# mryab/learning-at-home

Hardware: NVIDIA H100
Metric: DMoE training samples/sec (whole job, device-timed, max over ranks) (higher is better)
Workload: dtype bf16

## Files before the change

learning-at-home_b200/csrc/adam.cu:

```cuda
#include "sm90.cuh"

namespace lah {

struct AdamArgs {
    float* p; float* g; float* m; float* v; float* vmax; bf16* p_bf16;
    int num_segs; long long seg_start[13]; long long seg_n[12]; long long total;
    const int* step;
    const int* group_rows;
    int step_scalar;
    float lr, beta1, beta2, eps, weight_decay;
    int amsgrad, zero_mask;
    int world; long long peer_grad_off; char* peer_base[8]; float grad_scale;
    int G_active; const int* shadow_of; long long shadow_g_off; int me;
    int num_ranges; long long r_start[6]; long long r_cum[7];
    int dead_mask;
    const int* poison;
    float decay;
    const float* lr_dev;
};

template <bool DECOUPLED, bool DEV_LR>
__global__ void __launch_bounds__(256) adam_kernel(AdamArgs a) {
    if (a.poison && (*a.poison & 1)) return;
    float dev_lr = 0.f, dev_decay = 1.f;
    if constexpr (DEV_LR) {
        dev_lr = a.lr_dev[0];
        if constexpr (DECOUPLED) dev_decay = a.lr_dev[1];
    }
    const long long stride = static_cast<long long>(gridDim.x) * blockDim.x * 4;
    const long long span = a.num_ranges ? a.r_cum[a.num_ranges] : a.total;
    for (long long j = (static_cast<long long>(blockIdx.x) * blockDim.x + threadIdx.x) * 4; j < span; j += stride) {
        long long i = j;
        if (a.num_ranges) {
            int r = 0;
#pragma unroll
            for (int t = 1; t < 6; ++t)
                if (t < a.num_ranges && j >= a.r_cum[t]) r = t;
            i = a.r_start[r] + (j - a.r_cum[r]);
        }
        int sg = 0;
#pragma unroll
        for (int t = 1; t < 12; ++t)
            if (t < a.num_segs && i >= a.seg_start[t]) sg = t;
        const int g = static_cast<int>((i - a.seg_start[sg]) / a.seg_n[sg]);
        if (g >= a.G_active) continue;
        if (a.group_rows && a.group_rows[g] <= 0) continue;
        const int step = a.step ? a.step[g] : a.step_scalar;
        const float bc1 = 1.f - powf(a.beta1, static_cast<float>(step));
        const float bc2 = 1.f - powf(a.beta2, static_cast<float>(step));
        const float step_size = (DEV_LR ? dev_lr : a.lr) / bc1;
        const float inv_sqrt_bc2 = rsqrtf(bc2);
        float4 gr;
        if (a.peer_grad_off >= 0) {
            gr = make_float4(0.f, 0.f, 0.f, 0.f);
            for (int r = 0; r < a.world; ++r) {
                if ((a.dead_mask >> r) & 1) continue;
                const float4 t = *reinterpret_cast<const float4*>(
                    reinterpret_cast<const float*>(a.peer_base[r] + a.peer_grad_off) + i);
                gr.x += t.x; gr.y += t.y; gr.z += t.z; gr.w += t.w;
            }
            gr.x *= a.grad_scale; gr.y *= a.grad_scale; gr.z *= a.grad_scale; gr.w *= a.grad_scale;
        } else if (a.shadow_of && a.shadow_of[2 * g] >= 0) {
            const int slot = a.shadow_of[2 * g], mask = a.shadow_of[2 * g + 1];
            gr = ((mask >> a.me) & 1) ? *reinterpret_cast<const float4*>(a.g + i) : make_float4(0.f, 0.f, 0.f, 0.f);
            const long long pi = i + (a.G_active + slot - g) * a.seg_n[sg];
            for (int r = 0; r < a.world; ++r) {
                if (r == a.me || !((mask >> r) & 1)) continue;
                const float4 t = *reinterpret_cast<const float4*>(
                    reinterpret_cast<const float*>(a.peer_base[r] + a.shadow_g_off) + pi);
                gr.x += t.x; gr.y += t.y; gr.z += t.z; gr.w += t.w;
            }
        } else {
            gr = *reinterpret_cast<const float4*>(a.g + i);
        }
        float4 p = *reinterpret_cast<const float4*>(a.p + i);
        float4 m = *reinterpret_cast<const float4*>(a.m + i);
        float4 v = *reinterpret_cast<const float4*>(a.v + i);
        float4 vm = a.amsgrad ? *reinterpret_cast<const float4*>(a.vmax + i) : make_float4(0.f, 0.f, 0.f, 0.f);
        float* pp = &p.x; float* mp = &m.x; float* vp = &v.x; float* vmp = &vm.x; float* gp = &gr.x;
#pragma unroll
        for (int t = 0; t < 4; ++t) {
            float grad = gp[t];
            if constexpr (DECOUPLED) pp[t] = __fmul_rn(pp[t], DEV_LR ? dev_decay : a.decay);
            else if (a.weight_decay != 0.f) grad += a.weight_decay * pp[t];
            mp[t] = mp[t] + (1.f - a.beta1) * (grad - mp[t]);
            vp[t] = vp[t] * a.beta2 + (1.f - a.beta2) * grad * grad;
            float denom;
            if (a.amsgrad) {
                vmp[t] = fmaxf(vmp[t], vp[t]);
                denom = sqrtf(vmp[t]) * inv_sqrt_bc2 + a.eps;
            } else {
                denom = sqrtf(vp[t]) * inv_sqrt_bc2 + a.eps;
            }
            pp[t] -= step_size * (mp[t] / denom);
        }
        *reinterpret_cast<float4*>(a.p + i) = p;
        *reinterpret_cast<float4*>(a.m + i) = m;
        *reinterpret_cast<float4*>(a.v + i) = v;
        if (a.amsgrad) *reinterpret_cast<float4*>(a.vmax + i) = vm;
        if (a.p_bf16) {
            uint2 q;
            q.x = pack_bf16x2(p.x, p.y);
            q.y = pack_bf16x2(p.z, p.w);
            *reinterpret_cast<uint2*>(a.p_bf16 + i) = q;
        }
        if (((a.zero_mask >> sg) & 1) && a.peer_grad_off < 0)
            *reinterpret_cast<float4*>(a.g + i) = make_float4(0.f, 0.f, 0.f, 0.f);
    }
}

__global__ void bump_steps_kernel(int* step, const int* group_rows, int G) {
    const int g = blockIdx.x * blockDim.x + threadIdx.x;
    if (g < G && group_rows[g] > 0) step[g] += 1;
}

__global__ void cast_bf16_kernel(const float* __restrict__ src, bf16* __restrict__ dst, long long n) {
    const long long stride = static_cast<long long>(gridDim.x) * blockDim.x * 4;
    for (long long i = (static_cast<long long>(blockIdx.x) * blockDim.x + threadIdx.x) * 4; i < n; i += stride) {
        const float4 p = *reinterpret_cast<const float4*>(src + i);
        uint2 q;
        q.x = pack_bf16x2(p.x, p.y);
        q.y = pack_bf16x2(p.z, p.w);
        *reinterpret_cast<uint2*>(dst + i) = q;
    }
}

__global__ void split_encode_kernel(const float* __restrict__ p, bf16* __restrict__ hi, uint16_t* __restrict__ lo,
                                    float* __restrict__ v, long long n) {
    const long long stride = static_cast<long long>(gridDim.x) * blockDim.x * 4;
    for (long long i = (static_cast<long long>(blockIdx.x) * blockDim.x + threadIdx.x) * 4; i < n; i += stride) {
        const float4 w = *reinterpret_cast<const float4*>(p + i);
        float4 s = *reinterpret_cast<const float4*>(v + i);
        uint2 h, l;
        h.x = pack_bf16x2(w.x, w.y);
        h.y = pack_bf16x2(w.z, w.w);
        l.x = (__float_as_uint(w.x) & 0xffffu) | (__float_as_uint(w.y) << 16);
        l.y = (__float_as_uint(w.z) & 0xffffu) | (__float_as_uint(w.w) << 16);
        s.x = with_tie_bit(without_tie_bit(s.x), split_tie_up(w.x));
        s.y = with_tie_bit(without_tie_bit(s.y), split_tie_up(w.y));
        s.z = with_tie_bit(without_tie_bit(s.z), split_tie_up(w.z));
        s.w = with_tie_bit(without_tie_bit(s.w), split_tie_up(w.w));
        *reinterpret_cast<uint2*>(hi + i) = h;
        *reinterpret_cast<uint2*>(lo + i) = l;
        *reinterpret_cast<float4*>(v + i) = s;
    }
}

__global__ void split_decode_kernel(const bf16* __restrict__ hi, const uint16_t* __restrict__ lo,
                                    const float* __restrict__ v, float* __restrict__ p, long long n) {
    const long long stride = static_cast<long long>(gridDim.x) * blockDim.x * 4;
    for (long long i = (static_cast<long long>(blockIdx.x) * blockDim.x + threadIdx.x) * 4; i < n; i += stride) {
        const uint2 h = *reinterpret_cast<const uint2*>(hi + i);
        const uint2 l = *reinterpret_cast<const uint2*>(lo + i);
        const float4 s = *reinterpret_cast<const float4*>(v + i);
        float4 w;
        w.x = split_decode(h.x & 0xffffu, l.x & 0xffffu, __float_as_uint(s.x) >> 31);
        w.y = split_decode(h.x >> 16, l.x >> 16, __float_as_uint(s.y) >> 31);
        w.z = split_decode(h.y & 0xffffu, l.y & 0xffffu, __float_as_uint(s.z) >> 31);
        w.w = split_decode(h.y >> 16, l.y >> 16, __float_as_uint(s.w) >> 31);
        *reinterpret_cast<float4*>(p + i) = w;
    }
}

}

using namespace lah;

extern "C" const int* lah_get_poison_word();

extern "C" {

int lah_adam_step(float* p, float* g, float* m, float* v, float* vmax, void* p_bf16, int num_segs, const long long* seg_n,
                  int G, const int* step, const int* group_rows, int step_scalar, float lr, const float* lr_dev, float beta1,
                  float beta2, float eps, float weight_decay, int amsgrad, int zero_mask, int world, long long peer_grad_off,
                  const unsigned long long* peer_bases, float grad_scale, int G_active, const int* shadow_of,
                  long long shadow_g_off, int me, int seg_mask, int dead_mask, float decay, int decoupled, cudaStream_t st) {
    if (num_segs < 1 || num_segs > 12) return -2;
    if (decoupled && weight_decay != 0.f) return -2;
    AdamArgs a;
    a.num_segs = num_segs;
    long long off = 0;
    for (int s = 0; s < 12; ++s) {
        a.seg_start[s] = off;
        a.seg_n[s] = s < num_segs ? seg_n[s] : 1;
        if (s < num_segs) {
            if (seg_n[s] % 4) return -2;
            off += seg_n[s] * G;
        }
    }
    a.seg_start[12] = off;
    a.p = p; a.g = g; a.m = m; a.v = v; a.vmax = vmax; a.p_bf16 = (bf16*)p_bf16;
    a.total = off; a.step = step; a.group_rows = group_rows; a.step_scalar = step_scalar; a.lr = lr;
    a.beta1 = beta1; a.beta2 = beta2; a.eps = eps; a.weight_decay = weight_decay; a.amsgrad = amsgrad;
    a.zero_mask = zero_mask; a.world = world; a.peer_grad_off = peer_grad_off; a.grad_scale = grad_scale;
    a.G_active = G_active > 0 ? G_active : G; a.shadow_of = shadow_of; a.shadow_g_off = shadow_g_off; a.me = me;
    for (int i = 0; i < 8; ++i) a.peer_base[i] = (peer_bases && i < world) ? (char*)peer_bases[i] : nullptr;
    a.poison = lah_get_poison_word();
    a.dead_mask = dead_mask;
    a.decay = decay;
    a.lr_dev = lr_dev;
    a.num_ranges = 0;
    a.r_cum[0] = 0;
    if (seg_mask) {
        for (int s = 0; s < num_segs; ++s) {
            if (!((seg_mask >> s) & 1)) continue;
            const long long len = seg_n[s] * G;
            if (a.num_ranges && a.r_start[a.num_ranges - 1] + (a.r_cum[a.num_ranges] - a.r_cum[a.num_ranges - 1]) == a.seg_start[s]) {
                a.r_cum[a.num_ranges] += len;
            } else {
                if (a.num_ranges == 6) return -2;
                a.r_start[a.num_ranges] = a.seg_start[s];
                a.r_cum[a.num_ranges + 1] = a.r_cum[a.num_ranges] + len;
                ++a.num_ranges;
            }
        }
        if (!a.num_ranges) return 0;
    }
    const long long span = a.num_ranges ? a.r_cum[a.num_ranges] : a.total;
    if (span <= 0) return 0;
    long long blocks = (span / 4 + 255) / 256;
    if (blocks > 132 * 16) blocks = 132 * 16;
    if (lr_dev) {
        if (decoupled)
            adam_kernel<true, true><<<(int)blocks, 256, 0, st>>>(a);
        else
            adam_kernel<false, true><<<(int)blocks, 256, 0, st>>>(a);
    } else if (decoupled) {
        adam_kernel<true, false><<<(int)blocks, 256, 0, st>>>(a);
    } else {
        adam_kernel<false, false><<<(int)blocks, 256, 0, st>>>(a);
    }
    return -(int)cudaGetLastError();
}

int lah_bump_steps(int* step, const int* group_rows, int G, cudaStream_t st) {
    bump_steps_kernel<<<(G + 255) / 256, 256, 0, st>>>(step, group_rows, G);
    return -(int)cudaGetLastError();
}

int lah_cast_bf16(const float* src, void* dst, long long n, cudaStream_t st) {
    if (n % 4) return -2;
    if (n <= 0) return 0;
    long long blocks = (n / 4 + 255) / 256;
    if (blocks > 132 * 16) blocks = 132 * 16;
    cast_bf16_kernel<<<(int)blocks, 256, 0, st>>>(src, (bf16*)dst, n);
    return -(int)cudaGetLastError();
}

int lah_split_master(float* p, void* hi, void* lo, float* v, long long n, int encode, cudaStream_t st) {
    if (n % 4) return -2;
    if (n <= 0) return 0;
    long long blocks = (n / 4 + 255) / 256;
    if (blocks > 132 * 16) blocks = 132 * 16;
    if (encode)
        split_encode_kernel<<<(int)blocks, 256, 0, st>>>(p, (bf16*)hi, (uint16_t*)lo, v, n);
    else
        split_decode_kernel<<<(int)blocks, 256, 0, st>>>((const bf16*)hi, (const uint16_t*)lo, v, p, n);
    return -(int)cudaGetLastError();
}

}
```

learning-at-home_b200/csrc/layernorm.cu:

```cuda
#include "sm90.cuh"
#include <cuda_fp8.h>
#include <stdlib.h>

#include <array>
#include <utility>

namespace lah {

constexpr float LN_EPS = 1e-5f;

constexpr int LN_MAX_C = 4096;

template <int C>
struct LnFwdCfg {
    static constexpr int NV = (C + 255) / 256;
    static constexpr bool TUNED = C >= 256 && (C & (C - 1)) == 0;
    static constexpr int R = TUNED ? ((NV * 4 <= 16) ? 4 : ((NV * 2 <= 16) ? 2 : 1)) : (NV <= 2 ? 4 : (NV <= 6 ? 2 : 1));
    static constexpr int MIN_BLOCKS = (TUNED || NV <= 12) ? 2 : 1;
};

static int ln_rows_per_warp(int dflt) {
    static int forced = -1;
    if (forced < 0) {
        const char* e = getenv("LAH_LN_ROWS");
        forced = e ? atoi(e) : 0;
    }
    return forced == 1 ? 1 : dflt;
}

template <int C, bool QUANT, int R>
__global__ void __launch_bounds__(256, LnFwdCfg<C>::MIN_BLOCKS) ln_relu_fwd_kernel(
    const bf16* __restrict__ h, bf16* __restrict__ a, float* __restrict__ mean_out, float* __restrict__ rstd_out,
    const float* __restrict__ gamma, const float* __restrict__ beta, const int* __restrict__ tile_group, int rows,
    int relu, uint8_t* __restrict__ aq, uint8_t* __restrict__ sf, int tile_shift) {
    constexpr int NV = LnFwdCfg<C>::NV;
    constexpr bool HALF = C % 256 != 0;
    static_assert(C % 128 == 0 && C <= LN_MAX_C && !(QUANT && HALF), "unsupported LayerNorm width");
    const int warp = threadIdx.x >> 5, lane = threadIdx.x & 31;
    const int row0 = (blockIdx.x * 8 + warp) * R;
    if (row0 >= rows) return;
    const int g = tile_group ? __ldg(tile_group + (row0 >> tile_shift)) : 0;
    if (g < 0) return;
    int4 q[R][NV];
#pragma unroll
    for (int r = 0; r < R; ++r) {
        const int4* hp = reinterpret_cast<const int4*>(h + static_cast<long long>(min(row0 + r, rows - 1)) * C);
#pragma unroll
        for (int j = 0; j < NV; ++j) {
            if constexpr (HALF) {
                if (j == NV - 1 && lane >= 16) {
                    q[r][j] = make_int4(0, 0, 0, 0);
                    continue;
                }
            }
            q[r][j] = ld_nc_v4(hp + j * 32 + lane);
        }
    }
    float mean[R], rstd[R];
#pragma unroll
    for (int r = 0; r < R; ++r) {
        float s = 0.f, ss = 0.f;
#pragma unroll
        for (int j = 0; j < NV; ++j) {
            const uint32_t w[4] = {(uint32_t)q[r][j].x, (uint32_t)q[r][j].y, (uint32_t)q[r][j].z, (uint32_t)q[r][j].w};
#pragma unroll
            for (int t = 0; t < 4; ++t) {
                const float2 f = unpack_bf16x2(w[t]);
                s += f.x + f.y;
                ss += f.x * f.x + f.y * f.y;
            }
        }
        s = warp_sum(s);
        ss = warp_sum(ss);
        mean[r] = s * (1.f / C);
        rstd[r] = rsqrtf(fmaxf(ss * (1.f / C) - mean[r] * mean[r], 0.f) + LN_EPS);
        if (lane == 0 && mean_out && row0 + r < rows) {
            mean_out[row0 + r] = mean[r];
            rstd_out[row0 + r] = rstd[r];
        }
    }
    const float* gp = gamma + static_cast<long long>(g) * C;
    const float* bp = beta + static_cast<long long>(g) * C;
#pragma unroll
    for (int j = 0; j < NV; ++j) {
        if constexpr (HALF) {
            if (j == NV - 1 && lane >= 16) break;
        }
        const int col = (j * 32 + lane) * 8;
        const int4 g0 = ld_nc_v4(reinterpret_cast<const int4*>(gp + col));
        const int4 g1 = ld_nc_v4(reinterpret_cast<const int4*>(gp + col + 4));
        const int4 b0 = ld_nc_v4(reinterpret_cast<const int4*>(bp + col));
        const int4 b1 = ld_nc_v4(reinterpret_cast<const int4*>(bp + col + 4));
        const float gg[8] = {__int_as_float(g0.x), __int_as_float(g0.y), __int_as_float(g0.z), __int_as_float(g0.w),
                             __int_as_float(g1.x), __int_as_float(g1.y), __int_as_float(g1.z), __int_as_float(g1.w)};
        const float bb[8] = {__int_as_float(b0.x), __int_as_float(b0.y), __int_as_float(b0.z), __int_as_float(b0.w),
                             __int_as_float(b1.x), __int_as_float(b1.y), __int_as_float(b1.z), __int_as_float(b1.w)};
#pragma unroll
        for (int r = 0; r < R; ++r) {
            const int row = row0 + r;
            if (row >= rows) continue;
            const uint32_t w[4] = {(uint32_t)q[r][j].x, (uint32_t)q[r][j].y, (uint32_t)q[r][j].z, (uint32_t)q[r][j].w};
            float y[8];
#pragma unroll
            for (int t = 0; t < 4; ++t) {
                const float2 f = unpack_bf16x2(w[t]);
                y[2 * t] = (f.x - mean[r]) * rstd[r] * gg[2 * t] + bb[2 * t];
                y[2 * t + 1] = (f.y - mean[r]) * rstd[r] * gg[2 * t + 1] + bb[2 * t + 1];
            }
            if (relu) {
#pragma unroll
                for (int t = 0; t < 8; ++t) y[t] = fmaxf(y[t], 0.f);
            }
            if (!QUANT || a) {
                int4 o;
                o.x = pack_bf16x2(y[0], y[1]);
                o.y = pack_bf16x2(y[2], y[3]);
                o.z = pack_bf16x2(y[4], y[5]);
                o.w = pack_bf16x2(y[6], y[7]);
                st_v4(reinterpret_cast<int4*>(a + static_cast<long long>(row) * C) + j * 32 + lane, o);
            }
            if (QUANT) {
                float amax = 0.f;
#pragma unroll
                for (int t = 0; t < 8; ++t) amax = fmaxf(amax, fabsf(y[t]));
                amax = fmaxf(amax, __shfl_xor_sync(0xffffffffu, amax, 1));
                amax = fmaxf(amax, __shfl_xor_sync(0xffffffffu, amax, 2));
                const uint32_t bits = __float_as_uint(amax * (1.f / 448.f));
                uint32_t e = ((bits >> 23) & 0xFFu) + ((bits & 0x7FFFFFu) ? 1u : 0u);
                e = min(max(e, 1u), 253u);
                const float inv = __uint_as_float((254u - e) << 23);
                uint2 o8;
                o8.x = static_cast<uint32_t>(__nv_cvt_float2_to_fp8x2(make_float2(y[0] * inv, y[1] * inv), __NV_SATFINITE, __NV_E4M3)) |
                       (static_cast<uint32_t>(__nv_cvt_float2_to_fp8x2(make_float2(y[2] * inv, y[3] * inv), __NV_SATFINITE, __NV_E4M3)) << 16);
                o8.y = static_cast<uint32_t>(__nv_cvt_float2_to_fp8x2(make_float2(y[4] * inv, y[5] * inv), __NV_SATFINITE, __NV_E4M3)) |
                       (static_cast<uint32_t>(__nv_cvt_float2_to_fp8x2(make_float2(y[6] * inv, y[7] * inv), __NV_SATFINITE, __NV_E4M3)) << 16);
                asm volatile("st.global.v2.u32 [%0], {%1, %2};" ::"l"(reinterpret_cast<uint2*>(aq + static_cast<long long>(row) * C) + j * 32 + lane),
                             "r"(o8.x), "r"(o8.y)
                             : "memory");
                if ((lane & 3) == 0) {
                    const int kb32 = j * 8 + (lane >> 2);
                    const int ra = row & 127;
                    const long long chunk = static_cast<long long>(row >> 7) * (C / 128) + (kb32 >> 2);
                    sf[chunk * 512 + ((ra & 31) * 4 + (ra >> 5)) * 4 + (kb32 & 3)] = static_cast<uint8_t>(e);
                }
            }
        }
    }
}

template <int C>
struct LnBwdCfg {
    static constexpr int THREADS = (C / 8 + 31) / 32 * 32;
    static constexpr int MIN_BLOCKS = (C <= 2048) ? 2 : 1;
    static constexpr int RB = ((THREADS / 32 * MIN_BLOCKS + 3) / 4 >= 4 && C != 2048) ? 2 : 4;
};

template <int C, bool RES>
__global__ void __launch_bounds__(LnBwdCfg<C>::THREADS, LnBwdCfg<C>::MIN_BLOCKS) ln_relu_bwd_kernel(const bf16* __restrict__ da, const bf16* __restrict__ h,
                                                            const float* __restrict__ mean_in,
                                                            const float* __restrict__ rstd_in,
                                                            const float* __restrict__ gamma,
                                                            const float* __restrict__ beta, bf16* __restrict__ dh,
                                                            float* __restrict__ part,
                                                            const int* __restrict__ tile_group, int rows, int relu, int tile_rows,
                                                            const bf16* __restrict__ dres) {
    constexpr int THREADS = LnBwdCfg<C>::THREADS;
    constexpr int WARPS = THREADS / 32;
    constexpr bool IDLE = THREADS * 8 != C;
    static_assert(C % 128 == 0 && C <= LN_MAX_C, "unsupported LayerNorm width");
    constexpr int RB = LnBwdCfg<C>::RB;
    __shared__ float red[WARPS][2 * RB];
    __shared__ float tot[2 * RB];
    const int tile = blockIdx.x;
    const int g = tile_group ? __ldg(tile_group + tile) : 0;
    if (g < 0) return;
    const int tid = threadIdx.x, warp = tid >> 5, lane = tid & 31;
    const int col = tid * 8;
    const bool live = !IDLE || col < C;
    float gam[8], bet[8];
    if (!live) {
#pragma unroll
        for (int t = 0; t < 8; ++t) gam[t] = bet[t] = 0.f;
    } else {
        const float* gp = gamma + static_cast<long long>(g) * C + col;
        const float* bp = beta + static_cast<long long>(g) * C + col;
        const float4 g0 = __ldg(reinterpret_cast<const float4*>(gp)), g1 = __ldg(reinterpret_cast<const float4*>(gp + 4));
        const float4 b0 = __ldg(reinterpret_cast<const float4*>(bp)), b1 = __ldg(reinterpret_cast<const float4*>(bp + 4));
        gam[0] = g0.x; gam[1] = g0.y; gam[2] = g0.z; gam[3] = g0.w; gam[4] = g1.x; gam[5] = g1.y; gam[6] = g1.z; gam[7] = g1.w;
        bet[0] = b0.x; bet[1] = b0.y; bet[2] = b0.z; bet[3] = b0.w; bet[4] = b1.x; bet[5] = b1.y; bet[6] = b1.z; bet[7] = b1.w;
    }
    float acc_dg[8], acc_db[8], acc_dbias[8];
#pragma unroll
    for (int t = 0; t < 8; ++t) acc_dg[t] = acc_db[t] = acc_dbias[t] = 0.f;

    const int row0 = tile * tile_rows;
    const int row_end = min(rows, row0 + tile_rows);
    int4 nqa[RB], nqh[RB];
    float nmu[RB], nrs[RB];
    auto issue_loads = [&](int rb) {
#pragma unroll
        for (int r = 0; r < RB; ++r) {
            const int row = rb + r;
            const int rr = row < row_end ? row : row0;
            const long long off = static_cast<long long>(rr) * C + col;
            if (live) {
                nqa[r] = ld_nc_v4(reinterpret_cast<const int4*>(da + off));
                nqh[r] = ld_nc_v4(reinterpret_cast<const int4*>(h + off));
            } else {
                nqa[r] = nqh[r] = make_int4(0, 0, 0, 0);
            }
            nmu[r] = __ldg(mean_in + rr);
            nrs[r] = __ldg(rstd_in + rr);
        }
    };
    issue_loads(row0);
    for (int rb = row0; rb < row_end; rb += RB) {
        float rs[RB];
        float part[2 * RB];
        int4 qa_c[RB], qh_c[RB];
        float mu_c[RB];
#pragma unroll
        for (int r = 0; r < RB; ++r) {
            qa_c[r] = nqa[r];
            qh_c[r] = nqh[r];
            mu_c[r] = nmu[r];
            rs[r] = nrs[r];
        }
        if (rb + RB < row_end) issue_loads(rb + RB);
        auto slice = [&](int r, bool ok, float (&gvv)[8], float (&xhh)[8]) {
            const uint32_t wa[4] = {(uint32_t)qa_c[r].x, (uint32_t)qa_c[r].y, (uint32_t)qa_c[r].z, (uint32_t)qa_c[r].w};
            const uint32_t wh[4] = {(uint32_t)qh_c[r].x, (uint32_t)qh_c[r].y, (uint32_t)qh_c[r].z, (uint32_t)qh_c[r].w};
#pragma unroll
            for (int t = 0; t < 4; ++t) {
                const float2 fa = unpack_bf16x2(wa[t]);
                const float2 fh = unpack_bf16x2(wh[t]);
                const float x0 = (fh.x - mu_c[r]) * rs[r], x1 = (fh.y - mu_c[r]) * rs[r];
                const float y0 = x0 * gam[2 * t] + bet[2 * t], y1 = x1 * gam[2 * t + 1] + bet[2 * t + 1];
                gvv[2 * t] = (ok && (!relu || y0 > 0.f)) ? fa.x : 0.f;
                gvv[2 * t + 1] = (ok && (!relu || y1 > 0.f)) ? fa.y : 0.f;
                xhh[2 * t] = x0;
                xhh[2 * t + 1] = x1;
            }
        };
#pragma unroll
        for (int r = 0; r < RB; ++r) {
            float gvv[8], xhh[8];
            slice(r, rb + r < row_end, gvv, xhh);
            float s1 = 0.f, s2 = 0.f;
// ... 203 lines not shown
            }
            nrs[r] = __ldg(rstd_in + rr);
        }
    };
    issue_loads(row0);
    for (int rb = row0; rb < row_end; rb += RB) {
        int4 qd[RB], qx[RB];
        float rs[RB], sum[RB];
#pragma unroll
        for (int r = 0; r < RB; ++r) {
            qd[r] = nqd[r];
            qx[r] = nqx[r];
            rs[r] = nrs[r];
        }
        if (rb + RB < row_end) issue_loads(rb + RB);
        auto unpack8 = [](const int4& q, float (&f)[8]) {
            const uint32_t w[4] = {(uint32_t)q.x, (uint32_t)q.y, (uint32_t)q.z, (uint32_t)q.w};
#pragma unroll
            for (int t = 0; t < 4; ++t) {
                const float2 v = unpack_bf16x2(w[t]);
                f[2 * t] = v.x;
                f[2 * t + 1] = v.y;
            }
        };
#pragma unroll
        for (int r = 0; r < RB; ++r) {
            float d[8], xv[8], s = 0.f;
            unpack8(qd[r], d);
            unpack8(qx[r], xv);
#pragma unroll
            for (int t = 0; t < 8; ++t) s += d[t] * gam[t] * xv[t];
            sum[r] = rb + r < row_end ? s : 0.f;
        }
#pragma unroll
        for (int r = 0; r < RB; ++r) sum[r] = warp_sum(sum[r]);
        if (lane == 0) {
#pragma unroll
            for (int r = 0; r < RB; ++r) red[warp][r] = sum[r];
        }
        __syncthreads();
        if (tid < RB) {
            float s = 0.f;
#pragma unroll
            for (int w = 0; w < WARPS; ++w) s += red[w][tid];
            tot[tid] = s * (1.f / C);
        }
        __syncthreads();
#pragma unroll
        for (int r = 0; r < RB; ++r) {
            const int row = rb + r;
            if (row >= row_end || !live) continue;
            float d[8], xv[8], o[8];
            unpack8(qd[r], d);
            unpack8(qx[r], xv);
            const float m = tot[r] * rs[r] * rs[r];
            if (RES) {
                float res[8];
                unpack8(ld_nc_v4(reinterpret_cast<const int4*>(dres + static_cast<long long>(row) * C + col)), res);
#pragma unroll
                for (int t = 0; t < 8; ++t) o[t] = rs[r] * (d[t] * gam[t] - xv[t] * m) + res[t];
            } else {
#pragma unroll
                for (int t = 0; t < 8; ++t) o[t] = rs[r] * (d[t] * gam[t] - xv[t] * m);
            }
#pragma unroll
            for (int t = 0; t < 8; ++t) acc_dg[t] += d[t] * (xv[t] * rs[r]);
            int4 q;
            q.x = pack_bf16x2(o[0], o[1]);
            q.y = pack_bf16x2(o[2], o[3]);
            q.z = pack_bf16x2(o[4], o[5]);
            q.w = pack_bf16x2(o[6], o[7]);
            *reinterpret_cast<int4*>(dx + static_cast<long long>(row) * C + col) = q;
        }
    }
    if (!live) return;
    float* pg = part + static_cast<long long>(tile) * C + col;
#pragma unroll
    for (int t = 0; t < 8; ++t) pg[t] = acc_dg[t];
}

__global__ void __launch_bounds__(512) grouped_colsum_kernel(const bf16* __restrict__ x, long long ldx,
                                                             float* __restrict__ part, int C,
                                                             const int* __restrict__ tile_group, int rows, int tile_rows) {
    __shared__ float2 sm[4][128];
    const int tile = blockIdx.x;
    const int g = tile_group ? __ldg(tile_group + tile) : 0;
    if (g < 0) return;
    const int cp = threadIdx.x & 127;
    const int phase = threadIdx.x >> 7;
    const int col = blockIdx.y * 256 + cp * 2;
    if (col >= C) return;
    const int row0 = tile * tile_rows, row_end = min(rows, row0 + tile_rows);
    float2 acc = make_float2(0.f, 0.f);
    for (int r = row0 + phase; r < row_end; r += 4) {
        const uint32_t u = __ldg(reinterpret_cast<const uint32_t*>(x + static_cast<long long>(r) * ldx + col));
        const float2 f = unpack_bf16x2(u);
        acc.x += f.x;
        acc.y += f.y;
    }
    sm[phase][cp] = acc;
    __syncthreads();
    if (phase == 0) {
        float2 s = sm[0][cp];
#pragma unroll
        for (int p = 1; p < 4; ++p) {
            s.x += sm[p][cp].x;
            s.y += sm[p][cp].y;
        }
        *reinterpret_cast<float2*>(part + static_cast<long long>(tile) * C + col) = s;
    }
}

__global__ void __launch_bounds__(256) group_tile_sum_kernel(const float* __restrict__ part, int num_tiles, int V, int C,
                                                             const int* __restrict__ tile_group, float* out0, float* out1,
                                                             float* out2) {
    const int i = blockIdx.x * blockDim.x + threadIdx.x;
    if (i >= V * C) return;
    const int v = i / C, c = i - v * C;
    float* out = v == 0 ? out0 : (v == 1 ? out1 : out2);
    int cur = -1;
    float acc = 0.f;
    for (int t = 0; t < num_tiles; ++t) {
        const int g = tile_group ? __ldg(tile_group + t) : 0;
        if (g < 0) continue;
        if (g != cur) {
            if (cur >= 0) out[static_cast<long long>(cur) * C + c] += acc;
            cur = g;
            acc = 0.f;
        }
        acc += __ldg(part + (static_cast<long long>(t) * V + v) * C + c);
    }
    if (cur >= 0) out[static_cast<long long>(cur) * C + c] += acc;
}

using LnFwdLaunch = void (*)(const void*, void*, float*, float*, const float*, const float*, const int*, int, int, int,
                             cudaStream_t);
using LnBwdLaunch = void (*)(const void*, const void*, const float*, const float*, const float*, const float*, void*,
                             float*, float*, float*, float*, const int*, int, int, int, const void*, cudaStream_t);

template <int C>
void ln_fwd_launch(const void* h, void* a, float* mean, float* rstd, const float* gamma, const float* beta,
                   const int* tile_group, int rows, int relu, int tile_shift, cudaStream_t st) {
    constexpr int RR = LnFwdCfg<C>::R;
    if constexpr (LnFwdCfg<C>::TUNED) {
        if (ln_rows_per_warp(RR) == 1) {
            ln_relu_fwd_kernel<C, false, 1><<<(rows + 7) / 8, 256, 0, st>>>(
                (const bf16*)h, (bf16*)a, mean, rstd, gamma, beta, tile_group, rows, relu, nullptr, nullptr, tile_shift);
            return;
        }
    }
    ln_relu_fwd_kernel<C, false, RR><<<(rows + 8 * RR - 1) / (8 * RR), 256, 0, st>>>(
        (const bf16*)h, (bf16*)a, mean, rstd, gamma, beta, tile_group, rows, relu, nullptr, nullptr, tile_shift);
}

template <int C>
void ln_bwd_launch(const void* da, const void* h, const float* mean, const float* rstd, const float* gamma,
                   const float* beta, void* dh, float* dgamma, float* dbeta, float* dbias, float* part,
                   const int* tile_group, int rows, int relu, int tile_rows, const void* dres, cudaStream_t st) {
    const int grid = (rows + tile_rows - 1) / tile_rows;
    constexpr int T = LnBwdCfg<C>::THREADS;
    if (dres)
        ln_relu_bwd_kernel<C, true><<<grid, T, 0, st>>>((const bf16*)da, (const bf16*)h, mean, rstd, gamma, beta,
                                                        (bf16*)dh, part, tile_group, rows, relu, tile_rows,
                                                        (const bf16*)dres);
    else
        ln_relu_bwd_kernel<C, false><<<grid, T, 0, st>>>((const bf16*)da, (const bf16*)h, mean, rstd, gamma, beta,
                                                         (bf16*)dh, part, tile_group, rows, relu, tile_rows, nullptr);
    group_tile_sum_kernel<<<(3 * C + 255) / 256, 256, 0, st>>>(part, grid, 3, C, tile_group, dgamma, dbeta, dbias);
}

template <int... I>
constexpr auto ln_fwd_table(std::integer_sequence<int, I...>) {
    return std::array<LnFwdLaunch, sizeof...(I)>{ln_fwd_launch<(I + 1) * 128>...};
}
template <int... I>
constexpr auto ln_bwd_table(std::integer_sequence<int, I...>) {
    return std::array<LnBwdLaunch, sizeof...(I)>{ln_bwd_launch<(I + 1) * 128>...};
}
constexpr auto kLnFwd = ln_fwd_table(std::make_integer_sequence<int, LN_MAX_C / 128>{});
constexpr auto kLnBwd = ln_bwd_table(std::make_integer_sequence<int, LN_MAX_C / 128>{});

using RmsFwdLaunch = void (*)(const void*, void*, float*, const float*, int, float, const int*, int, cudaStream_t);
using RmsBwdLaunch = void (*)(const void*, const void*, const float*, const float*, void*, float*, float*, int, int,
                              const void*, const int*, cudaStream_t);

template <int C>
void rms_fwd_launch(const void* x, void* n, float* rstd, const float* gamma, int rows, float eps, const int* tile_group,
                    int tile_shift, cudaStream_t st) {
    constexpr int RR = RmsFwdCfg<C>::R;
    const int grid = (rows + 8 * RR - 1) / (8 * RR);
    if (tile_group)
        rms_norm_fwd_kernel<C, RR, true><<<grid, 256, 0, st>>>((const bf16*)x, (bf16*)n, rstd, gamma, rows, eps,
                                                               tile_group, tile_shift);
    else
        rms_norm_fwd_kernel<C, RR, false><<<grid, 256, 0, st>>>((const bf16*)x, (bf16*)n, rstd, gamma, rows, eps,
                                                                nullptr, 0);
}

template <int C, bool GROUPED>
void rms_bwd_kernel_launch(int grid, const void* dn, const void* x, const float* rstd, const float* gamma, void* dx,
                           float* part, int rows, int tile_rows, const void* dres, const int* tile_group,
                           cudaStream_t st) {
    constexpr int T = LnBwdCfg<C>::THREADS;
    if (dres)
        rms_norm_bwd_kernel<C, true, GROUPED><<<grid, T, 0, st>>>((const bf16*)dn, (const bf16*)x, rstd, gamma,
                                                                  (bf16*)dx, part, rows, tile_rows, (const bf16*)dres,
                                                                  tile_group);
    else
        rms_norm_bwd_kernel<C, false, GROUPED><<<grid, T, 0, st>>>((const bf16*)dn, (const bf16*)x, rstd, gamma,
                                                                   (bf16*)dx, part, rows, tile_rows, nullptr,
                                                                   tile_group);
}

template <int C>
void rms_bwd_launch(const void* dn, const void* x, const float* rstd, const float* gamma, void* dx, float* dgamma,
                    float* part, int rows, int tile_rows, const void* dres, const int* tile_group, cudaStream_t st) {
    const int grid = (rows + tile_rows - 1) / tile_rows;
    if (tile_group)
        rms_bwd_kernel_launch<C, true>(grid, dn, x, rstd, gamma, dx, part, rows, tile_rows, dres, tile_group, st);
    else
        rms_bwd_kernel_launch<C, false>(grid, dn, x, rstd, gamma, dx, part, rows, tile_rows, dres, nullptr, st);
    group_tile_sum_kernel<<<(C + 255) / 256, 256, 0, st>>>(part, grid, 1, C, tile_group, dgamma, nullptr, nullptr);
}

template <int... I>
constexpr auto rms_fwd_table(std::integer_sequence<int, I...>) {
    return std::array<RmsFwdLaunch, sizeof...(I)>{rms_fwd_launch<(I + 1) * 128>...};
}
template <int... I>
constexpr auto rms_bwd_table(std::integer_sequence<int, I...>) {
    return std::array<RmsBwdLaunch, sizeof...(I)>{rms_bwd_launch<(I + 1) * 128>...};
}
constexpr auto kRmsFwd = rms_fwd_table(std::make_integer_sequence<int, LN_MAX_C / 128>{});
constexpr auto kRmsBwd = rms_bwd_table(std::make_integer_sequence<int, LN_MAX_C / 128>{});

static bool ln_width_ok(int C) { return C > 0 && C % 128 == 0 && C <= LN_MAX_C; }

}

using namespace lah;

extern "C" {

static int shift_of(int tile_rows) {
    int s = 0;
    while ((1 << s) < tile_rows) ++s;
    return ((1 << s) == tile_rows && tile_rows >= 8) ? s : -1;
}

int lah_ln_relu_fwd(const void* h, void* a, float* mean, float* rstd, const float* gamma, const float* beta,
                    const int* tile_group, int rows, int C, int relu, int tile_rows, cudaStream_t st) {
    if (rows <= 0) return 0;
    const int tile_shift = shift_of(tile_rows);
    if (tile_shift < 0 || !ln_width_ok(C)) return -2;
    kLnFwd[C / 128 - 1](h, a, mean, rstd, gamma, beta, tile_group, rows, relu, tile_shift, st);
    return -(int)cudaGetLastError();
}

int lah_ln_relu_fwd_q(const void* h, void* a, float* mean, float* rstd, const float* gamma, const float* beta,
                      const int* tile_group, int rows, int C, int relu, void* aq, void* sf, cudaStream_t st) {
    if (rows <= 0) return 0;
#define LAH_LN_FWD(CC)                                                                                          \
    if (C == CC) {                                                                                              \
        constexpr int RR = LnFwdCfg<CC>::R;                                                                     \
        if (ln_rows_per_warp(RR) == 1)                                                                          \
            ln_relu_fwd_kernel<CC, true, 1><<<(rows + 7) / 8, 256, 0, st>>>(                                  \
                (const bf16*)h, (bf16*)a, mean, rstd, gamma, beta, tile_group, rows, relu, (uint8_t*)aq, (uint8_t*)sf, 7);   \
        else                                                                                                    \
            ln_relu_fwd_kernel<CC, true, RR><<<(rows + 8 * RR - 1) / (8 * RR), 256, 0, st>>>(                 \
                (const bf16*)h, (bf16*)a, mean, rstd, gamma, beta, tile_group, rows, relu, (uint8_t*)aq, (uint8_t*)sf, 7);   \
        return -(int)cudaGetLastError();                                                                        \
    }
    LAH_LN_FWD(256) LAH_LN_FWD(512) LAH_LN_FWD(1024) LAH_LN_FWD(2048) LAH_LN_FWD(4096)
#undef LAH_LN_FWD
    return -2;
}

int lah_ln_relu_bwd(const void* da, const void* h, const float* mean, const float* rstd, const float* gamma,
                    const float* beta, void* dh, float* dgamma, float* dbeta, float* dbias, float* part,
                    const int* tile_group, int rows, int C, int relu, int tile_rows, const void* dres, cudaStream_t st) {
    if (rows <= 0) return 0;
    if (shift_of(tile_rows) < 0 || !ln_width_ok(C)) return -2;
    kLnBwd[C / 128 - 1](da, h, mean, rstd, gamma, beta, dh, dgamma, dbeta, dbias, part, tile_group, rows, relu,
                        tile_rows, dres, st);
    return -(int)cudaGetLastError();
}

int lah_rms_norm_fwd(const void* x, void* n, float* rstd, const float* gamma, int rows, int C, float eps,
                     const int* tile_group, int tile_rows, cudaStream_t st) {
    if (rows <= 0) return 0;
    const int tile_shift = tile_group ? shift_of(tile_rows) : 0;
    if (!ln_width_ok(C) || !(eps > 0.f) || tile_shift < 0) return -2;
    kRmsFwd[C / 128 - 1](x, n, rstd, gamma, rows, eps, tile_group, tile_shift, st);
    return -(int)cudaGetLastError();
}

int lah_rms_norm_bwd(const void* dn, const void* x, const float* rstd, const float* gamma, void* dx, float* dgamma,
                     float* part, int rows, int C, int tile_rows, const void* dres, const int* tile_group,
                     cudaStream_t st) {
    if (rows <= 0) return 0;
    if (shift_of(tile_rows) < 0 || !ln_width_ok(C)) return -2;
    kRmsBwd[C / 128 - 1](dn, x, rstd, gamma, dx, dgamma, part, rows, tile_rows, dres, tile_group, st);
    return -(int)cudaGetLastError();
}

int lah_grouped_colsum(const void* x, long long ldx, float* out, float* part, int C, const int* tile_group, int rows,
                       int tile_rows, cudaStream_t st) {
    if (rows <= 0) return 0;
    if (C % 128 || shift_of(tile_rows) < 0) return -2;
    const int tiles = (rows + tile_rows - 1) / tile_rows;
    dim3 grid(tiles, (C + 255) / 256);
    grouped_colsum_kernel<<<grid, 512, 0, st>>>((const bf16*)x, ldx, part, C, tile_group, rows, tile_rows);
    group_tile_sum_kernel<<<(C + 255) / 256, 256, 0, st>>>(part, tiles, 1, C, tile_group, out, nullptr, nullptr);
    return -(int)cudaGetLastError();
}

}
```

learning-at-home_b200/csrc/moe.cu:

```cuda
#include <cfloat>

#include "sm90.cuh"

namespace lah {

constexpr int MAX_WORLD = 8;
constexpr int MAX_GRID_DIMS = 4;
constexpr int MAX_K = 8;
constexpr long long SPIN_TIMEOUT_CYCLES = 20000000000ll;

struct Peers {
    char* base[MAX_WORLD];
    int world;
    int me;
    unsigned long long* wait_ns;
    int* step_ctr;
    int spin_timeout_ms;
    char* mc_base;
};

__device__ __forceinline__ void multimem_st_release_u32(void* mc_addr, int v) {
    asm volatile("multimem.st.release.sys.global.u32 [%0], %1;" ::"l"(mc_addr), "r"(v) : "memory");
}
__device__ __forceinline__ void multimem_st_u32(void* mc_addr, int v) {
    asm volatile("multimem.st.relaxed.sys.global.u32 [%0], %1;" ::"l"(mc_addr), "r"(v) : "memory");
}

__device__ __forceinline__ void signal_all_ranks(const Peers& peers, long long flags_off, int slot, int epoch, int tid) {
    if (peers.mc_base) {
        if (tid == 0) {
            __threadfence_system();
            multimem_st_release_u32(peers.mc_base + flags_off + (static_cast<long long>(slot) * MAX_WORLD + peers.me) * 4, epoch);
        }
    } else if (tid < peers.world) {
        __threadfence_system();
        st_release_sys(reinterpret_cast<int*>(peers.base[tid] + flags_off) + slot * MAX_WORLD + peers.me, epoch);
    }
}

__device__ __forceinline__ int epoch_of(const Peers& peers, int rel) {
    return rel + (peers.step_ctr ? *reinterpret_cast<volatile const int*>(peers.step_ctr) : 0);
}

struct GridSpec {
    int ndim;
    int size[MAX_GRID_DIMS];
    int offset[MAX_GRID_DIMS];
    int total;
    int num_experts;
};

enum Status { STATUS_TIMEOUT = 1, STATUS_OVERFLOW = 2 };

__device__ __forceinline__ float hash_uniform(unsigned long long x) {
    x += 0x9E3779B97F4A7C15ull;
    x = (x ^ (x >> 30)) * 0xBF58476D1CE4E5B9ull;
    x = (x ^ (x >> 27)) * 0x94D049BB133111EBull;
    x = x ^ (x >> 31);
    return static_cast<float>(x >> 40) * (1.0f / 16777216.0f);
}

__device__ __forceinline__ bool spin_until_ge(const int* flag, int epoch, int* status, int timeout_ms = 0, int rank = -1) {
    if (status && rank >= 0) {
        const volatile int* vs = status;
        if ((vs[1] >> rank) & 1) return false;
        if (vs[0] & STATUS_TIMEOUT) return false;
    }
    const long long t0 = clock64();
    const long long limit = timeout_ms > 0 ? static_cast<long long>(timeout_ms) * 2000000ll : SPIN_TIMEOUT_CYCLES;
    while (ld_acquire_sys(flag) < epoch) {
        if (clock64() - t0 > limit) {
            atomicOr(status, STATUS_TIMEOUT);
            return false;
        }
    }
    return true;
}

__device__ __forceinline__ void account_wait(const Peers& peers, unsigned long long t0, int world) {
    const unsigned long long dt64 = globaltimer_ns() - t0;
    const unsigned mask = (world >= 32) ? 0xffffffffu : ((1u << world) - 1u);
    const unsigned dt = __reduce_max_sync(mask, dt64 > 0xffffffffull ? 0xffffffffu : static_cast<unsigned>(dt64));
    if (peers.wait_ns && (threadIdx.x & 31) == 0) atomicAdd(peers.wait_ns, static_cast<unsigned long long>(dt));
}

// ... 122 lines not shown
    return a + (BIAS ? t.v2 : sigmoid_affinity(t.v2));
}

template <bool BIAS, bool SIGMOID>
__device__ __forceinline__ void group_scores(const float* lg, const GridSpec& gs, int n_group,
                                             const unsigned char* __restrict__ alive, float failure_rate,
                                             unsigned long long seed, long long tok, const float* __restrict__ bias,
                                             float* gscore, int* gvalid, int lane) {
    const int E = gs.num_experts, gsz = E / n_group;
    if (32 % gsz == 0) {
        for (int c0 = 0; c0 < E; c0 += 32) {
            const int c = c0 + lane;
            GroupTop2 t{-INFINITY, -INFINITY, 0};
            float key;
            if (c < E && group_candidate_key<BIAS, SIGMOID>(lg, gs, c, alive, failure_rate, seed, tok, bias, key))
                group_push<SIGMOID>(t, key);
            for (int o = gsz >> 1; o > 0; o >>= 1) group_merge<SIGMOID>(t, o);
            if (c < E && (lane & (gsz - 1)) == 0) {
                gscore[c / gsz] = group_score<BIAS, SIGMOID>(t);
                gvalid[c / gsz] = t.n > 0;
            }
        }
    } else {
        for (int g = 0; g < n_group; ++g) {
            GroupTop2 t{-INFINITY, -INFINITY, 0};
            for (int c = g * gsz + lane; c < (g + 1) * gsz; c += 32) {
                float key;
                if (group_candidate_key<BIAS, SIGMOID>(lg, gs, c, alive, failure_rate, seed, tok, bias, key))
                    group_push<SIGMOID>(t, key);
            }
#pragma unroll
            for (int o = 16; o > 0; o >>= 1) group_merge<SIGMOID>(t, o);
            if (lane == 0) {
                gscore[g] = group_score<BIAS, SIGMOID>(t);
                gvalid[g] = t.n > 0;
            }
        }
    }
    __syncwarp();
}

__device__ __forceinline__ void select_groups(const float* gscore, int* gvalid, int n_group, int topk_group, int lane) {
    const float a = lane < n_group ? gscore[lane] : -INFINITY;
    const float c = lane + 32 < n_group ? gscore[lane + 32] : -INFINITY;
    bool av = lane < n_group && gvalid[lane], cv = lane + 32 < n_group && gvalid[lane + 32];
    bool as = false, cs = false;
    for (int r = 0; r < topk_group; ++r) {
        float bv = -INFINITY;
        int bi = -1;
        if (av && (!cv || a >= c)) {
            bv = a;
            bi = lane;
        } else if (cv) {
            bv = c;
            bi = lane + 32;
        }
#pragma unroll
        for (int o = 16; o > 0; o >>= 1) {
            const float ov = __shfl_xor_sync(0xffffffffu, bv, o);
            const int oi = __shfl_xor_sync(0xffffffffu, bi, o);
            if ((oi >= 0) && (bi < 0 || ov > bv || (ov == bv && oi < bi))) {
                bv = ov;
                bi = oi;
            }
        }
        if (bi < 0) break;
        if (bi == lane) av = false, as = true;
        if (bi == lane + 32) cv = false, cs = true;
    }
    if (lane < n_group) gvalid[lane] = as;
    if (lane + 32 < n_group) gvalid[lane + 32] = cs;
    __syncwarp();
}

template <bool BIAS, bool SIGMOID, bool GROUPED, bool NORM>
__global__ void __launch_bounds__(256, GROUPED ? 1 : 0) gate_topk_kernel(const float* __restrict__ logits, int B, GridSpec gs, int k,
                                                        const unsigned char* __restrict__ alive, float failure_rate,
                                                        unsigned long long seed, long long token_offset,
                                                        int* __restrict__ idx_out, float* __restrict__ w_out,
                                                        int* __restrict__ pos_out, int* __restrict__ counts,
                                                        const int* __restrict__ step_ctr, const float* __restrict__ bias,
                                                        float scale, float* __restrict__ sig_out, int n_group,
                                                        int topk_group, float* __restrict__ lse_out) {
    constexpr bool LSE = !NORM && !SIGMOID;
    if (step_ctr) token_offset += *reinterpret_cast<const long long*>(step_ctr + 2);
    extern __shared__ float s_logits[];
    const int warp = threadIdx.x >> 5, lane = threadIdx.x & 31;
    const int b = blockIdx.x * 8 + warp;
    if (b >= B) return;
    float* lg = s_logits + warp * gs.total;
    for (int i = lane; i < gs.total; i += 32) lg[i] = logits[static_cast<long long>(b) * gs.total + i];
    __syncwarp();
    const int* gsel = nullptr;
    unsigned gdiv = 0;
    if constexpr (GROUPED) {
        float* gscore = s_logits + 8 * gs.total + warp * GROUP_WORDS;
        int* gvalid = reinterpret_cast<int*>(gscore + MAX_GROUPS);
        group_scores<BIAS, SIGMOID>(lg, gs, n_group, alive, failure_rate, seed, token_offset + b, bias, gscore, gvalid,
                                    lane);
        select_groups(gscore, gvalid, n_group, topk_group, lane);
        gsel = gvalid;
        gdiv = 0x7fffffffu / static_cast<unsigned>(gs.num_experts / n_group) + 1u;
    }

    float best_v[MAX_K];
    float best_u[MAX_K];
    int best_i[MAX_K];
#pragma unroll
    for (int j = 0; j < MAX_K; ++j) {
        best_v[j] = -INFINITY;
        best_u[j] = -INFINITY;
        best_i[j] = -1;
    }
    float run_m = -INFINITY, run_l = 0.f;
    for (int c = lane; c < gs.num_experts; c += 32) {
        float s = 0.f;
        if constexpr (LSE) {
            if (alive && !alive[c]) continue;
            s = pk_score(lg, gs, c);
            lse_fold(run_m, run_l, s);
        }
        if constexpr (GROUPED)
            if (!gsel[__umulhi(static_cast<unsigned>(c) << 1, gdiv)]) continue;
        if (!LSE && alive && !alive[c]) continue;
        if (failure_rate > 0.f) {
            const unsigned long long key = seed ^ (static_cast<unsigned long long>(token_offset + b) * 0x100000001B3ull +
                                                   static_cast<unsigned long long>(c));
            if (hash_uniform(key) < failure_rate) continue;
        }
        if constexpr (!LSE) {
            int rem = c;
#pragma unroll
            for (int d = MAX_GRID_DIMS - 1; d >= 0; --d) {
                if (d < gs.ndim) {
                    const int i = rem % gs.size[d];
                    rem /= gs.size[d];
                    s += lg[gs.offset[d] + i];
                }
            }
        }
        float key = s, aff = s;
        if constexpr (BIAS && SIGMOID) aff = sigmoid_affinity(s);
        if constexpr (BIAS) key = __fadd_rn(aff, __ldg(bias + c));
        if (key > best_v[MAX_K - 1] || best_i[MAX_K - 1] < 0) {
            float v = key, u = aff;
            int id = c;
            bool shifting = false;
#pragma unroll
            for (int j = 0; j < MAX_K; ++j) {
                const bool take = shifting || (best_i[j] < 0) || (v > best_v[j]);
                if (take) {
                    shifting = true;
                    const float tv = best_v[j];
                    const int ti = best_i[j];
                    best_v[j] = v;
                    best_i[j] = id;
                    v = tv;
                    id = ti;
                    if constexpr (BIAS) {
                        const float tu = best_u[j];
                        best_u[j] = u;
                        u = tu;
                    }
                }
            }
        }
// ... 29 lines not shown
                    bi = oi;
                    if constexpr (BIAS) bu = ou;
                }
            }
            sel_v[j] = BIAS ? bu : bv;
            sel_i[j] = bi;
            if (bi >= 0 && bi == id) ++head;
        }
    }
    if constexpr (SIGMOID) {
        float sg[MAX_K];
        float S = 0.f;
#pragma unroll
        for (int j = 0; j < MAX_K; ++j) {
            sg[j] = 0.f;
            if (sel_i[j] >= 0) sg[j] = BIAS ? sel_v[j] : sigmoid_affinity(sel_v[j]);
            S += sg[j];
        }
        const float norm = !NORM ? scale : S > 0.f ? __fdividef(scale, S) : 0.f;
        if (lane < k) {
            int id = -1;
            float v = 0.f;
#pragma unroll
            for (int j = 0; j < MAX_K; ++j)
                if (j == lane) {
                    id = sel_i[j];
                    v = sg[j];
                }
            const long long o = static_cast<long long>(b) * k + lane;
            idx_out[o] = id;
            w_out[o] = v * norm;
            sig_out[o] = v;
            if (id < 0) pos_out[o] = 0;
        }
        return;
    }
    if constexpr (LSE) {
#pragma unroll
        for (int o = 16; o > 0; o >>= 1) lse_merge(run_m, run_l, o);
        const float z = run_m > -INFINITY ? run_m + __logf(run_l) : 0.f;
        if (lane == 0) lse_out[b] = z;
        if (lane < k) {
            int id = -1;
            float v = 0.f;
#pragma unroll
            for (int j = 0; j < MAX_K; ++j)
                if (j == lane) {
                    id = sel_i[j];
                    v = sel_v[j];
                }
            const long long o = static_cast<long long>(b) * k + lane;
            idx_out[o] = id;
            w_out[o] = id >= 0 ? scale * __expf(v - z) : 0.f;
            if (id < 0) pos_out[o] = 0;
        }
        return;
    }
    float mx = -INFINITY;
#pragma unroll
    for (int j = 0; j < MAX_K; ++j)
        if (sel_i[j] >= 0) mx = fmaxf(mx, sel_v[j]);
    float denom = 0.f;
#pragma unroll
    for (int j = 0; j < MAX_K; ++j)
        if (sel_i[j] >= 0) denom += __expf(sel_v[j] - mx);
    if (lane < k) {
        int id = -1;
        float v = 0.f;
#pragma unroll
        for (int j = 0; j < MAX_K; ++j)
            if (j == lane) {
                id = sel_i[j];
                v = sel_v[j];
            }
        const long long o = static_cast<long long>(b) * k + lane;
        idx_out[o] = id;
        w_out[o] = id >= 0 ? __expf(v - mx) / denom : 0.f;
        if (id < 0) pos_out[o] = 0;
    }
}

__global__ void __launch_bounds__(1024) rank_slots_kernel(const int* __restrict__ idx, int n, int* __restrict__ pos,
                                                          int* __restrict__ counts) {
    __shared__ int warp_off[32];
    __shared__ int s_total;
    const int e = blockIdx.x, tid = threadIdx.x, lane = tid & 31, warp = tid >> 5;
    int base = 0;
    for (int start = 0; start < n; start += 1024) {
        const int i = start + tid;
        const bool hit = i < n && __ldg(idx + i) == e;
        const unsigned m = __ballot_sync(0xffffffffu, hit);
        if (lane == 0) warp_off[warp] = __popc(m);
        __syncthreads();
        if (warp == 0) {
            const int v = warp_off[lane];
            int incl = v;
#pragma unroll
            for (int d = 1; d < 32; d <<= 1) {
                const int y = __shfl_up_sync(0xffffffffu, incl, d);
                if (lane >= d) incl += y;
            }
            warp_off[lane] = incl - v;
            if (lane == 31) s_total = incl;
        }
        __syncthreads();
        if (hit) pos[i] = base + warp_off[warp] + __popc(m & ((1u << lane) - 1u));
        base += s_total;
        __syncthreads();
    }
    if (tid == 0 && base) counts[e] += base;
}

struct LayoutArgs {
    long long cnt_all_off;
    long long flags_off;
    int slot;
    int epoch;
    int E, E_loc;
    int max_rows;
    int max_tiles;
    int align;
    int tile_rows;
    int* counts;
    int* dst_row;
    int* group_off;
    int* group_rows;
    int* tile_group;
    int* total_rows;
    int* status;
    int S_max;
    float shadow_tol;
    int min_shadow_rows;
    int* route_owner;
    int* step_rows;
    int* shadow_info;
    int* owned_shadow;
};

constexpr int LAYOUT_MAX_E = 4096;

__global__ void __launch_bounds__(1024) layout_exchange_kernel(Peers peers, LayoutArgs a) {
    __shared__ int warp_tot[32];
    __shared__ int owner_base_s[MAX_WORLD + 1];
    __shared__ int s_tot[LAYOUT_MAX_E];
    __shared__ short s_slot[LAYOUT_MAX_E];
    __shared__ long long s_load[MAX_WORLD];
    __shared__ int s_shadow[MAX_WORLD * 2];
    __shared__ int s_pick[2];
    __shared__ int s_red_v[32], s_red_i[32];
    const int tid = threadIdx.x, lane = tid & 31, warp = tid >> 5;
    const int me = peers.me, world = peers.world;
    a.epoch = epoch_of(peers, a.epoch);
    if (peers.mc_base) {
        int* dst = reinterpret_cast<int*>(peers.mc_base + a.cnt_all_off) + static_cast<long long>(me) * a.E;
        for (int e = tid; e < a.E; e += blockDim.x) multimem_st_u32(dst + e, a.counts[e]);
    } else {
        for (int r = 0; r < world; ++r) {
            int* dst = reinterpret_cast<int*>(peers.base[r] + a.cnt_all_off) + static_cast<long long>(me) * a.E;
            for (int e = tid; e < a.E; e += blockDim.x) dst[e] = a.counts[e];
        }
    }
    __threadfence_system();
    __syncthreads();
    signal_all_ranks(peers, a.flags_off, a.slot, a.epoch, tid);
    if (tid < world) {
        const int* fw = reinterpret_cast<const int*>(peers.base[me] + a.flags_off) + a.slot * MAX_WORLD + tid;
        const unsigned long long t0 = globaltimer_ns();
        spin_until_ge(fw, a.epoch, a.status, peers.spin_timeout_ms, tid);
        account_wait(peers, t0, world);
    }
    __syncthreads();
    {
        const int dead = reinterpret_cast<volatile int*>(a.status)[1];
        if (dead) {
            int* mine = reinterpret_cast<int*>(peers.base[me] + a.cnt_all_off);
            for (int r = 0; r < world; ++r)
                if ((dead >> r) & 1)
                    for (int e = tid; e < a.E; e += blockDim.x) mine[static_cast<long long>(r) * a.E + e] = 0;
        }
    }
    for (int t = tid; t < a.max_tiles; t += blockDim.x) a.tile_group[t] = -1;
    if (tid < MAX_WORLD) s_load[tid] = 0;
    if (tid < MAX_WORLD * 2) s_shadow[tid] = -1;
    __syncthreads();
    const int* cnt_all = reinterpret_cast<const int*>(peers.base[me] + a.cnt_all_off);
    for (int e = tid; e < a.E; e += blockDim.x) {
        int tot = 0;
        for (int s = 0; s < world; ++s) tot += cnt_all[static_cast<long long>(s) * a.E + e];
        s_tot[e] = tot;
        s_slot[e] = -1;
        if (tot) atomicAdd(reinterpret_cast<unsigned long long*>(&s_load[e / a.E_loc]), static_cast<unsigned long long>(tot));
    }
    __syncthreads();
    int num_shadow = 0;
    for (int it = 0; it < a.S_max && world > 1; ++it) {
        if (tid == 0) {
            long long total = 0, mx = -1;
            int rmax = 0;
            for (int r = 0; r < world; ++r) {
                total += s_load[r];
                if (s_load[r] > mx) {
                    mx = s_load[r];
                    rmax = r;
                }
            }
            const bool balanced = static_cast<float>(mx) * world <= a.shadow_tol * static_cast<float>(total);
            s_pick[0] = balanced ? -1 : rmax;
        }
        __syncthreads();
        const int rmax = s_pick[0];
        if (rmax < 0) break;
        int bv = -1, bi = -1;
        for (int le = tid; le < a.E_loc; le += blockDim.x) {
            const int e = rmax * a.E_loc + le;
            if (s_slot[e] < 0 && s_tot[e] > bv) {
                bv = s_tot[e];
                bi = e;
            }
        }
#pragma unroll
        for (int o = 16; o > 0; o >>= 1) {
            const int ov = __shfl_xor_sync(0xffffffffu, bv, o);
            const int oi = __shfl_xor_sync(0xffffffffu, bi, o);
            if (ov > bv || (ov == bv && oi >= 0 && (bi < 0 || oi < bi))) {
// ... 81 lines not shown
            a.group_rows[G_own + s] = rows;
            for (int t = cur / a.tile_rows; t < (cur + padded) / a.tile_rows && t < a.max_tiles; ++t) a.tile_group[t] = G_own + s;
            int mask = 0;
            if (e >= 0)
                for (int r = 0; r < world; ++r) mask |= (cnt_all[static_cast<long long>(r) * a.E + e] > 0) << r;
            a.shadow_info[4 * s + 0] = e;
            a.shadow_info[4 * s + 1] = e >= 0 ? e / a.E_loc : -1;
            a.shadow_info[4 * s + 2] = rows;
            a.shadow_info[4 * s + 3] = mask;
            cur += padded;
        }
        a.group_off[G_own + a.S_max] = cur;
        *a.total_rows = cur;
    }
    if (tid < world) {
        int total = owner_base_s[tid + 1] - owner_base_s[tid];
        for (int s = 0; s < a.S_max; ++s) {
            const int e = s_shadow[s];
            if (e >= 0 && e / a.E_loc != tid)
                total += (cnt_all[static_cast<long long>(tid) * a.E + e] + a.align - 1) / a.align * a.align;
        }
        if (total > a.max_rows) atomicOr(a.status, STATUS_OVERFLOW);
    }
    __syncthreads();
    for (int e = tid; e < a.E; e += blockDim.x) {
        const int owner = e / a.E_loc;
        const int rel = a.dst_row[e] - owner_base_s[owner];
        const int before = a.counts[e];
        const int slot = s_slot[e];
        a.counts[e] = 0;
        if (owner == me) {
            const int le = e - me * a.E_loc;
            a.group_off[le] = rel;
            const int padded = (a.group_rows[le] + a.align - 1) / a.align * a.align;
            for (int t = rel / a.tile_rows; t < (rel + padded) / a.tile_rows && t < a.max_tiles; ++t) a.tile_group[t] = le;
            if (a.step_rows) a.step_rows[le] = s_tot[e];
            if (a.owned_shadow) {
                int mask = 0;
                if (slot >= 0)
                    for (int r = 0; r < world; ++r) mask |= (cnt_all[static_cast<long long>(r) * a.E + e] > 0) << r;
                a.owned_shadow[2 * le] = slot;
                a.owned_shadow[2 * le + 1] = mask;
            }
        }
        int dst, route;
        if (slot < 0) {
            dst = rel + before;
            route = owner;
        } else if (owner == me) {
            dst = rel;
            route = me;
        } else {
            dst = a.group_off[G_own + slot];
            route = me;
        }
        a.dst_row[e] = dst;
        if (a.route_owner) a.route_owner[e] = route;
    }
}

struct ScatterArgs {
    const bf16* src;
    const float* scale;
    const int* idx;
    const int* pos;
    const int* dst_row;
    int* pair_row;
    long long dst_off;
    long long flags_off;
    int slot, epoch;
    int num_pairs, k, H, E_loc, max_rows;
    const int* group_off;
    const int* group_rows;
    int pair_blocks;
    int align;
    const int* route_owner;
    int num_groups;
    int* done_counter;
    int* status;
};

template <int VEC_PER_LANE>
__global__ void __launch_bounds__(256) scatter_rows_kernel(Peers peers, ScatterArgs a) {
    const int warp = threadIdx.x >> 5, lane = threadIdx.x & 31;
    if (static_cast<int>(blockIdx.x) < a.pair_blocks) {
        const int p = blockIdx.x * 8 + warp;
        if (p < a.num_pairs) {
            const int e = a.idx[p];
            int row = -1;
            if (e >= 0) {
                row = (a.pair_row && !a.dst_row) ? a.pair_row[p] : a.dst_row[e] + a.pos[p];
                if (row >= a.max_rows) {
                    if (lane == 0) atomicOr(a.status, STATUS_OVERFLOW);
                    row = -1;
                }
            }
            if (a.pair_row && a.dst_row && lane == 0) a.pair_row[p] = row;
            if (row >= 0) {
                const int owner = a.route_owner ? a.route_owner[e] : e / a.E_loc;
                const int b = p / a.k;
                const int4* sp = reinterpret_cast<const int4*>(a.src + static_cast<long long>(b) * a.H);
                int4* dp = reinterpret_cast<int4*>(peers.base[owner] + a.dst_off) +
                           static_cast<long long>(row) * (a.H / 8);
                int4 v[VEC_PER_LANE];
#pragma unroll
                for (int j = 0; j < VEC_PER_LANE; ++j) v[j] = ld_nc_v4(sp + j * 32 + lane);
                if (a.scale) {
                    const float s = a.scale[p];
#pragma unroll
                    for (int j = 0; j < VEC_PER_LANE; ++j) {
                        uint32_t* u = reinterpret_cast<uint32_t*>(&v[j]);
#pragma unroll
                        for (int t = 0; t < 4; ++t) {
                            const float2 f = unpack_bf16x2(u[t]);
                            u[t] = pack_bf16x2(f.x * s, f.y * s);
                        }
                    }
                }
#pragma unroll
                for (int j = 0; j < VEC_PER_LANE; ++j) st_v4(dp + j * 32 + lane, v[j]);
            }
        }
    } else {
        const int nb = gridDim.x - a.pair_blocks;
        int4* base = reinterpret_cast<int4*>(peers.base[peers.me] + a.dst_off);
        const int4 z = make_int4(0, 0, 0, 0);
        for (int le = blockIdx.x - a.pair_blocks; le < a.num_groups; le += nb) {
            const int r0 = a.group_off[le] + a.group_rows[le];
            const int r1 = min(a.max_rows, a.group_off[le] + (a.group_rows[le] + a.align - 1) / a.align * a.align);
            for (int r = r0 + warp; r < r1; r += 8) {
                int4* dp = base + static_cast<long long>(r) * (a.H / 8);
#pragma unroll
                for (int j = 0; j < VEC_PER_LANE; ++j) dp[j * 32 + lane] = z;
            }
        }
    }
    __syncthreads();
    if (threadIdx.x == 0) {
        __threadfence_system();
        const int prev = atomicAdd(a.done_counter, 1);
        if (prev == static_cast<int>(gridDim.x) - 1) {
            *a.done_counter = 0;
            __threadfence_system();
            const int epoch = epoch_of(peers, a.epoch);
            if (peers.mc_base) {
                multimem_st_release_u32(peers.mc_base + a.flags_off + (static_cast<long long>(a.slot) * MAX_WORLD + peers.me) * 4, epoch);
            } else {
                for (int r = 0; r < peers.world; ++r) {
                    int* f = reinterpret_cast<int*>(peers.base[r] + a.flags_off) + a.slot * MAX_WORLD + peers.me;
                    st_release_sys(f, epoch);
                }
            }
        }
    }
}

__global__ void signal_wait_kernel(Peers peers, long long flags_off, int slot, int epoch, int do_signal, int do_wait,
                                   int* status) {
    const int lane = threadIdx.x;
    epoch = epoch_of(peers, epoch);
    if (do_signal) signal_all_ranks(peers, flags_off, slot, epoch, lane);
    if (do_wait && lane < peers.world) {
        const int* f = reinterpret_cast<const int*>(peers.base[peers.me] + flags_off) + slot * MAX_WORLD + lane;
        const unsigned long long t0 = globaltimer_ns();
        spin_until_ge(f, epoch, status, peers.spin_timeout_ms, lane);
        account_wait(peers, t0, peers.world);
    }
}

__global__ void __launch_bounds__(256) nvls_allreduce_kernel(Peers peers, long long off, long long n, float scale) {
    const long long per = ((n / 4 + peers.world - 1) / peers.world) * 4;
    const long long lo = per * peers.me, hi = min(n, lo + per);
    float* mc = reinterpret_cast<float*>(peers.mc_base + off);
    for (long long i = lo + (static_cast<long long>(blockIdx.x) * blockDim.x + threadIdx.x) * 4; i < hi;
         i += static_cast<long long>(gridDim.x) * blockDim.x * 4) {
        float4 r;
        asm volatile("multimem.ld_reduce.relaxed.sys.global.add.v4.f32 {%0, %1, %2, %3}, [%4];"
                     : "=f"(r.x), "=f"(r.y), "=f"(r.z), "=f"(r.w)
                     : "l"(mc + i)
                     : "memory");
        r.x *= scale; r.y *= scale; r.z *= scale; r.w *= scale;
        asm volatile("multimem.st.relaxed.sys.global.v4.f32 [%0], {%1, %2, %3, %4};" ::"l"(mc + i), "f"(r.x), "f"(r.y),
                     "f"(r.z), "f"(r.w)
                     : "memory");
    }
}

__global__ void heartbeat_kernel(Peers peers, long long hb_off, int first, int count, long long now_ms) {
    const int i = blockIdx.x * blockDim.x + threadIdx.x;
    if (i >= count) return;
    if (peers.mc_base) {
        asm volatile("multimem.st.relaxed.sys.global.u64 [%0], %1;" ::"l"(reinterpret_cast<long long*>(peers.mc_base + hb_off) + first + i),
                     "l"(now_ms)
                     : "memory");
    } else {
        for (int r = 0; r < peers.world; ++r) reinterpret_cast<long long*>(peers.base[r] + hb_off)[first + i] = now_ms;
    }
}

__global__ void alive_from_heartbeats_kernel(const long long* hb, unsigned char* alive, int E, long long now_ms, long long max_age_ms) {
    const int e = blockIdx.x * blockDim.x + threadIdx.x;
    if (e < E) alive[e] = (hb[e] > 0 && now_ms - hb[e] <= max_age_ms) ? 1 : 0;
}

__global__ void step_begin_kernel(int* step_ctr, int epoch_delta, long long token_delta) {
    step_ctr[0] += epoch_delta;
    *reinterpret_cast<long long*>(step_ctr + 2) += token_delta;
}

struct CombineArgs {
    long long src_off;
    const int* idx;
    const int* pair_row;
    const float* w;
    bf16* out;
    int B, k, H, E_loc;
    long long flags_off;
    int slot, epoch, do_signal, do_wait;
    int* status;
    const int* route_owner;
};

template <int VEC_PER_LANE, bool ADD>
__global__ void __launch_bounds__(256) combine_rows_kernel(Peers peers, CombineArgs a, const bf16* __restrict__ addend) {
    const int warp = threadIdx.x >> 5, lane = threadIdx.x & 31;
    if (a.do_signal || a.do_wait) a.epoch = epoch_of(peers, a.epoch);
    if (a.do_signal && blockIdx.x == 0 && threadIdx.x < 32) {
        signal_all_ranks(peers, a.flags_off, a.slot, a.epoch, threadIdx.x);
    }
    if (a.do_wait) {
        if (threadIdx.x < peers.world) {
            const int* f = reinterpret_cast<const int*>(peers.base[peers.me] + a.flags_off) + a.slot * MAX_WORLD + threadIdx.x;
            const unsigned long long t0 = globaltimer_ns();
            spin_until_ge(f, a.epoch, a.status, peers.spin_timeout_ms, threadIdx.x);
            if (blockIdx.x == 0) account_wait(peers, t0, peers.world);
        }
        __syncthreads();
    }
    const int b = blockIdx.x * 8 + warp;
    if (b >= a.B) return;
    float acc[VEC_PER_LANE * 8];
    if constexpr (ADD) {
        const int4* ap = reinterpret_cast<const int4*>(addend + static_cast<long long>(b) * a.H);
#pragma unroll
        for (int v = 0; v < VEC_PER_LANE; ++v) {
            const int4 q = __ldg(ap + v * 32 + lane);
            const uint32_t u[4] = {(uint32_t)q.x, (uint32_t)q.y, (uint32_t)q.z, (uint32_t)q.w};
#pragma unroll
            for (int t = 0; t < 4; ++t) {
                const float2 f = unpack_bf16x2(u[t]);
                acc[v * 8 + 2 * t] = f.x;
                acc[v * 8 + 2 * t + 1] = f.y;
            }
        }
    } else {
#pragma unroll
        for (int i = 0; i < VEC_PER_LANE * 8; ++i) acc[i] = 0.f;
    }
    for (int j = 0; j < a.k; ++j) {
        const long long p = static_cast<long long>(b) * a.k + j;
        const int e = a.idx[p];
        const int row = a.pair_row[p];
        if (e < 0 || row < 0) continue;
        const float w = a.w ? a.w[p] : 1.f;
        const int4* sp = reinterpret_cast<const int4*>(peers.base[a.route_owner ? a.route_owner[e] : e / a.E_loc] + a.src_off) +
                         static_cast<long long>(row) * (a.H / 8);
#pragma unroll
        for (int v = 0; v < VEC_PER_LANE; ++v) {
            const int4 q = ld_v4(sp + v * 32 + lane);
            const uint32_t u[4] = {(uint32_t)q.x, (uint32_t)q.y, (uint32_t)q.z, (uint32_t)q.w};
#pragma unroll
            for (int t = 0; t < 4; ++t) {
                const float2 f = unpack_bf16x2(u[t]);
                acc[v * 8 + 2 * t] += w * f.x;
                acc[v * 8 + 2 * t + 1] += w * f.y;
            }
        }
    }
    int4* op = reinterpret_cast<int4*>(a.out + static_cast<long long>(b) * a.H);
#pragma unroll
    for (int v = 0; v < VEC_PER_LANE; ++v) {
        int4 q;
        q.x = pack_bf16x2(acc[v * 8 + 0], acc[v * 8 + 1]);
        q.y = pack_bf16x2(acc[v * 8 + 2], acc[v * 8 + 3]);
        q.z = pack_bf16x2(acc[v * 8 + 4], acc[v * 8 + 5]);
        q.w = pack_bf16x2(acc[v * 8 + 6], acc[v * 8 + 7]);
        op[v * 32 + lane] = q;
    }
}

struct GateBwdArgs {
    long long yo_off;
    const bf16* grad;
    const int* idx;
    const int* pair_row;
    const float* w;
    float* dlogits;
    int B, k, H, E_loc;
    const int* route_owner;
};

template <int VEC_PER_LANE, bool SIGMOID, bool NORM>
__global__ void __launch_bounds__(256) gate_bwd_kernel(Peers peers, GateBwdArgs a, GridSpec gs,
                                                       const float* __restrict__ sig, float scale,
                                                       const float* __restrict__ logits, const float* __restrict__ lse,
                                                       const unsigned char* __restrict__ alive) {
    constexpr bool DENSE = !NORM && !SIGMOID;
    const int warp = threadIdx.x >> 5, lane = threadIdx.x & 31;
    const int b = blockIdx.x * 8 + warp;
    if (b >= a.B) return;
    float g[VEC_PER_LANE * 8];
    const int4* gp = reinterpret_cast<const int4*>(a.grad + static_cast<long long>(b) * a.H);
#pragma unroll
    for (int v = 0; v < VEC_PER_LANE; ++v) {
        const int4 q = ld_nc_v4(gp + v * 32 + lane);
        const uint32_t u[4] = {(uint32_t)q.x, (uint32_t)q.y, (uint32_t)q.z, (uint32_t)q.w};
#pragma unroll
        for (int t = 0; t < 4; ++t) {
            const float2 f = unpack_bf16x2(u[t]);
            g[v * 8 + 2 * t] = f.x;
            g[v * 8 + 2 * t + 1] = f.y;
        }
    }
    float dw[MAX_K], wj[MAX_K], sj[MAX_K];
    int ej[MAX_K];
    float dot_sum = 0.f;
#pragma unroll
    for (int j = 0; j < MAX_K; ++j) {
        dw[j] = 0.f;
        wj[j] = 0.f;
        if constexpr (SIGMOID) sj[j] = 0.f;
        ej[j] = -1;
        if (j < a.k) {
            const long long p = static_cast<long long>(b) * a.k + j;
            const int e = a.idx[p];
            const int row = a.pair_row[p];
            if (e >= 0) {
                wj[j] = a.w[p];
                ej[j] = e;
                if constexpr (SIGMOID) sj[j] = sig[p];
            }
            if (e >= 0 && row >= 0) {
                const int4* sp = reinterpret_cast<const int4*>(peers.base[a.route_owner ? a.route_owner[e] : e / a.E_loc] + a.yo_off) +
                                 static_cast<long long>(row) * (a.H / 8);
                float d = 0.f;
#pragma unroll
                for (int v = 0; v < VEC_PER_LANE; ++v) {
                    const int4 q = ld_v4(sp + v * 32 + lane);
                    const uint32_t u[4] = {(uint32_t)q.x, (uint32_t)q.y, (uint32_t)q.z, (uint32_t)q.w};
#pragma unroll
                    for (int t = 0; t < 4; ++t) {
                        const float2 f = unpack_bf16x2(u[t]);
                        d += g[v * 8 + 2 * t] * f.x + g[v * 8 + 2 * t + 1] * f.y;
                    }
                }
                d = warp_sum(d);
                dw[j] = d;
                dot_sum += wj[j] * d;
            }
        }
    }
    float* dl = a.dlogits + static_cast<long long>(b) * gs.total;
    for (int i = lane; i < gs.total; i += 32) dl[i] = 0.f;
    __syncwarp();
    if (lane == 0) {
        float inv_s = 0.f;
        if constexpr (SIGMOID && NORM) {
            float S = 0.f;
#pragma unroll
            for (int j = 0; j < MAX_K; ++j) S += sj[j];
            inv_s = S > 0.f ? __fdividef(1.f, S) : 0.f;
        }
#pragma unroll
        for (int j = 0; j < MAX_K; ++j) {
            if (ej[j] < 0) continue;
            float d;
            if constexpr (SIGMOID && NORM) d = sj[j] * (1.f - sj[j]) * (scale * dw[j] - dot_sum) * inv_s;
            else if constexpr (SIGMOID) d = scale * sj[j] * (1.f - sj[j]) * dw[j];
            else if constexpr (NORM) d = wj[j] * (dw[j] - dot_sum);
            else d = wj[j] * dw[j];
            int rem = ej[j];
            for (int dd = gs.ndim - 1; dd >= 0; --dd) {
                const int i = rem % gs.size[dd];
                rem /= gs.size[dd];
                dl[gs.offset[dd] + i] += d;
            }
        }
    }
    if constexpr (DENSE) {
// ... 220 lines not shown
    }
    __syncthreads();
    if (threadIdx.x == 0) {
        float ta = 0.f, tq = 0.f;
#pragma unroll
        for (int w = 0; w < RL_WARPS; ++w) {
            ta += s_warp[w][0];
            tq += s_warp[w][1];
        }
        loss[0] = f[gs.num_experts] * ta / static_cast<float>(B);
        loss[1] = tq / static_cast<float>(B);
        *ticket = 0;
    }
}

template <bool SIGMOID>
__global__ void __launch_bounds__(RL_WARPS * 32) router_loss_bwd_kernel(const float* __restrict__ logits, int B, GridSpec gs,
                                                                        const unsigned char* __restrict__ alive,
                                                                        const float* __restrict__ f,
                                                                        const float* __restrict__ z,
                                                                        const float* __restrict__ Fb, float aux_coef,
                                                                        float z_coef, float* __restrict__ dlogits) {
    extern __shared__ float s_buf[];
    const int warp = threadIdx.x >> 5, lane = threadIdx.x & 31;
    const int b = blockIdx.x * RL_WARPS + warp;
    if (b >= B) return;
    float* lg = s_buf + warp * router_bwd_warp_floats(gs);
    float* g = lg + gs.total;
    float* dl = dlogits + static_cast<long long>(b) * gs.total;
    for (int i = lane; i < gs.total; i += 32) lg[i] = logits[static_cast<long long>(b) * gs.total + i];
    __syncwarp();
    const float zb = z[b];
    const float invB = 1.f / static_cast<float>(B);
    const float base_aux = aux_coef * f[gs.num_experts];
    const float c0 = SIGMOID ? -base_aux * Fb[b] : 2.f * z_coef * zb - base_aux * Fb[b];
    const float inv_s = SIGMOID && zb > 0.f ? invB / zb : 0.f;
    for (int c = lane; c < gs.num_experts; c += 32) {
        float v = 0.f;
        if constexpr (SIGMOID) {
            if (!alive || alive[c]) {
                const float sg = sigmoid_affinity(pk_score(lg, gs, c));
                v = sg * (1.f - sg) * (base_aux * f[c] + c0) * inv_s;
            }
        } else if (!alive || alive[c]) {
            v = __expf(pk_score(lg, gs, c) - zb) * (base_aux * f[c] + c0) * invB;
        }
        if (gs.ndim == 1)
            dl[c] += v;
        else
            g[c + (c >> 5)] = v;
    }
    if (gs.ndim == 1) return;
    __syncwarp();
    for (int o = lane; o < gs.total; o += 32) {
        int d = 0;
        while (d + 1 < gs.ndim && o >= gs.offset[d + 1]) ++d;
        const int i = o - gs.offset[d];
        int stride = 1;
        for (int dd = gs.ndim - 1; dd > d; --dd) stride *= gs.size[dd];
        const int block = stride * gs.size[d];
        float acc = 0.f;
        for (int outer = 0; outer < gs.num_experts; outer += block)
            for (int inner = 0; inner < stride; ++inner) {
                const int e = outer + i * stride + inner;
                acc += g[e + (e >> 5)];
            }
        dl[o] += acc;
    }
}

static Peers g_peers = {};
static bool g_peers_set = false;

template <bool BIAS, bool SIGMOID, bool GROUPED, bool NORM>
static int launch_gate_topk(const float* logits, int B, const GridSpec& gs, int k, const unsigned char* alive,
                            float failure_rate, unsigned long long seed, long long token_offset, int* idx, float* w,
                            int* pos, int* counts, const float* bias, float scale, float* sig, int n_group,
                            int topk_group, float* lse, cudaStream_t st) {
    const int group_floats = GROUPED ? GROUP_WORDS : 0;
    if (int e = set_max_dynamic_smem<gate_topk_kernel<BIAS, SIGMOID, GROUPED, NORM>>(8 * sizeof(float) *
                                                                                     (LAYOUT_MAX_E + group_floats)))
        return e;
    if (B <= 0) return 0;
    gate_topk_kernel<BIAS, SIGMOID, GROUPED, NORM><<<(B + 7) / 8, 256, 8 * (gs.total + group_floats) * sizeof(float),
                                                     st>>>(
        logits, B, gs, k, alive, failure_rate, seed, token_offset, idx, w, pos, counts, g_peers.step_ctr, bias, scale, sig,
        n_group, topk_group, lse);
    return 0;
}

constexpr int GATE_BWD_DENSE_MAX_FLOATS = LAYOUT_MAX_E / 2 + 2 + LAYOUT_MAX_E + LAYOUT_MAX_E / 32 + 1;

template <int V, bool SIGMOID, bool NORM>
static int launch_gate_bwd(const GateBwdArgs& a, const GridSpec& gs, const float* sig, float scale, const float* logits,
                           const float* lse, const unsigned char* alive, cudaStream_t st) {
    int smem = 0;
    if constexpr (!SIGMOID && !NORM) {
        if (int e = set_max_dynamic_smem<gate_bwd_kernel<V, SIGMOID, NORM>>(8 * sizeof(float) *
                                                                             GATE_BWD_DENSE_MAX_FLOATS))
            return e;
        if (gs.ndim > 1) smem = 8 * router_bwd_warp_floats(gs) * sizeof(float);
    }
    gate_bwd_kernel<V, SIGMOID, NORM><<<(a.B + 7) / 8, 256, smem, st>>>(g_peers, a, gs, sig, scale, logits, lse, alive);
    return 0;
}

template <bool SIGMOID>
static int launch_router_loss_bwd(const float* logits, int B, const GridSpec& gs, const unsigned char* alive,
                                  const float* f, const float* z, const float* Fb, float aux_coef, float z_coef,
                                  float* dlogits, cudaStream_t st) {
    if (int e = set_max_dynamic_smem<router_loss_bwd_kernel<SIGMOID>>(RL_WARPS * sizeof(float) *
                                                                       (2 * LAYOUT_MAX_E + LAYOUT_MAX_E / 32 + 1)))
        return e;
    if (B == 0) return 0;
    router_loss_bwd_kernel<SIGMOID><<<(B + RL_WARPS - 1) / RL_WARPS, RL_WARPS * 32,
                                      RL_WARPS * router_bwd_warp_floats(gs) * sizeof(float), st>>>(
        logits, B, gs, alive, f, z, Fb, aux_coef, z_coef, dlogits);
    return 0;
}

}

using namespace lah;

extern "C" {

int lah_set_peers(const unsigned long long* bases, int world, int me) {
    if (world < 1 || world > MAX_WORLD || me < 0 || me >= world) return -2;
    for (int i = 0; i < MAX_WORLD; ++i) g_peers.base[i] = i < world ? reinterpret_cast<char*>(bases[i]) : nullptr;
    g_peers.world = world;
    g_peers.me = me;
    g_peers.wait_ns = nullptr;
    g_peers.step_ctr = nullptr;
    g_peers.spin_timeout_ms = 0;
    g_peers.mc_base = nullptr;
    g_peers_set = true;
    return 0;
}

int lah_set_multicast(unsigned long long mc_base) {
    g_peers.mc_base = reinterpret_cast<char*>(mc_base);
    return 0;
}
unsigned long long lah_get_multicast() { return reinterpret_cast<unsigned long long>(g_peers.mc_base); }

int lah_set_step_counters(int* step_ctr) {
    g_peers.step_ctr = step_ctr;
    return 0;
}
const int* lah_get_epoch_base() { return g_peers.step_ctr; }

int lah_set_spin_timeout_ms(int ms) {
    g_peers.spin_timeout_ms = ms;
    return 0;
}

int lah_nvls_allreduce(long long off, long long n, float scale, cudaStream_t st) {
    if (!g_peers_set || !g_peers.mc_base) return -10;
    if (n % 4 || off % 16) return -2;
    long long blocks = (n / 4 / g_peers.world + 255) / 256;
    if (blocks < 1) blocks = 1;
    if (blocks > 132 * 4) blocks = 132 * 4;
    nvls_allreduce_kernel<<<(int)blocks, 256, 0, st>>>(g_peers, off, n, scale);
    return -(int)cudaGetLastError();
}

int lah_heartbeat(long long hb_off, int first, int count, long long now_ms, cudaStream_t st) {
    if (!g_peers_set) return -10;
    if (count <= 0) return 0;
    heartbeat_kernel<<<(count + 127) / 128, 128, 0, st>>>(g_peers, hb_off, first, count, now_ms);
    return -(int)cudaGetLastError();
}

int lah_alive_from_heartbeats(const long long* hb, unsigned char* alive, int E, long long now_ms, long long max_age_ms,
                              cudaStream_t st) {
    if (E <= 0) return 0;
    alive_from_heartbeats_kernel<<<(E + 255) / 256, 256, 0, st>>>(hb, alive, E, now_ms, max_age_ms);
    return -(int)cudaGetLastError();
}

int lah_step_begin(int epoch_delta, long long token_delta, cudaStream_t st) {
    if (!g_peers.step_ctr) return -10;
    step_begin_kernel<<<1, 1, 0, st>>>(g_peers.step_ctr, epoch_delta, token_delta);
    return -(int)cudaGetLastError();
}

int lah_set_wait_counter(unsigned long long* counter) {
    g_peers.wait_ns = counter;
    return 0;
}

static int make_grid_spec(GridSpec* gs, const int* grid, int ndim) {
    if (ndim < 1 || ndim > MAX_GRID_DIMS) return -2;
    gs->ndim = ndim;
    gs->total = 0;
    gs->num_experts = 1;
    for (int d = 0; d < MAX_GRID_DIMS; ++d) {
        gs->size[d] = d < ndim ? grid[d] : 1;
        gs->offset[d] = gs->total;
        if (d < ndim) {
            gs->total += grid[d];
            gs->num_experts *= grid[d];
        }
    }
    return 0;
}

int lah_gate_topk(const float* logits, int B, const int* grid, int ndim, int k, const unsigned char* alive,
                  float failure_rate, unsigned long long seed, long long token_offset, int* idx, float* w, int* pos,
                  int* counts, const float* bias, int score_mode, float scale, float* sig, int n_group, int topk_group,
                  int norm, float* lse, cudaStream_t st) {
    GridSpec gs;
    if (make_grid_spec(&gs, grid, ndim)) return -2;
    if (k < 1 || k > MAX_K) return -3;
    if (gs.total > LAYOUT_MAX_E) return -2;
    if (bias && gs.num_experts > LAYOUT_MAX_E) return -2;
    if (norm != 0 && norm != 1) return -5;
    if (score_mode == 0 && norm && scale != 1.f) return -5;
    if (score_mode == 0 && !norm && (!(scale > 0.f && scale <= FLT_MAX) || (!lse && B > 0))) return -5;
    if (lse && (norm || score_mode != 0)) return -5;
    if (score_mode == 1 && (!(scale > 0.f && scale <= FLT_MAX) || (!sig && B > 0))) return -5;
    if (n_group < 1 || n_group > MAX_GROUPS || gs.num_experts % n_group) return -6;
    if (n_group > 1 && gs.num_experts > LAYOUT_MAX_E) return -6;
    if (topk_group < 1 || topk_group > n_group) return -6;
    const bool grouped = topk_group < n_group;
    int e;
#define LAH_GATE_TOPK(BIAS, SIGMOID, GROUPED, NORM)                                                                    \
    launch_gate_topk<BIAS, SIGMOID, GROUPED, NORM>(logits, B, gs, k, alive, failure_rate, seed, token_offset, idx, w,  \
                                                   pos, counts, BIAS ? bias : nullptr,                                 \
                                                   SIGMOID || !NORM ? scale : 1.f, SIGMOID ? sig : nullptr, n_group,   \
                                                   topk_group, NORM ? nullptr : lse, st)
#define LAH_GATE_TOPK_N(BIAS, SIGMOID, GROUPED) \
    (norm ? LAH_GATE_TOPK(BIAS, SIGMOID, GROUPED, true) : LAH_GATE_TOPK(BIAS, SIGMOID, GROUPED, false))
    if (score_mode == 0)
        e = grouped ? (bias ? LAH_GATE_TOPK_N(true, false, true) : LAH_GATE_TOPK_N(false, false, true))
                    : (bias ? LAH_GATE_TOPK_N(true, false, false) : LAH_GATE_TOPK_N(false, false, false));
    else if (score_mode == 1)
        e = grouped ? (bias ? LAH_GATE_TOPK_N(true, true, true) : LAH_GATE_TOPK_N(false, true, true))
                    : (bias ? LAH_GATE_TOPK_N(true, true, false) : LAH_GATE_TOPK_N(false, true, false));
    else
        return -4;
#undef LAH_GATE_TOPK_N
#undef LAH_GATE_TOPK
    if (e || B <= 0) return e;
    rank_slots_kernel<<<gs.num_experts, 1024, 0, st>>>(idx, B * k, pos, counts);
    return -(int)cudaGetLastError();
}

int lah_layout_exchange(long long cnt_all_off, long long flags_off, int slot, int epoch, int E, int E_loc, int max_rows,
                        int align, int tile_rows, int* counts, int* dst_row, int* group_off, int* group_rows, int* tile_group, int* total_rows,
                        int* status, int S_max, float shadow_tol, int min_shadow_rows, int* route_owner, int* step_rows,
                        int* shadow_info, int* owned_shadow, cudaStream_t st) {
    if (!g_peers_set) return -10;
    if (E > LAYOUT_MAX_E || S_max < 0 || S_max > 2 * MAX_WORLD) return -2;
    LayoutArgs a;
    a.cnt_all_off = cnt_all_off; a.flags_off = flags_off; a.slot = slot; a.epoch = epoch; a.E = E; a.E_loc = E_loc;
    if (tile_rows <= 0 || align % tile_rows) return -2;
    a.max_rows = max_rows; a.tile_rows = tile_rows; a.max_tiles = max_rows / tile_rows; a.align = align; a.counts = counts; a.dst_row = dst_row; a.group_off = group_off;
    a.group_rows = group_rows; a.tile_group = tile_group; a.total_rows = total_rows; a.status = status;
    a.S_max = S_max; a.shadow_tol = shadow_tol; a.min_shadow_rows = min_shadow_rows; a.route_owner = route_owner;
    a.step_rows = step_rows; a.shadow_info = shadow_info; a.owned_shadow = owned_shadow;
    layout_exchange_kernel<<<1, 1024, 0, st>>>(g_peers, a);
    return -(int)cudaGetLastError();
}

int lah_scatter_rows(const void* src, const float* scale, const int* idx, const int* pos, const int* dst_row,
                     int* pair_row, long long dst_off, long long flags_off, int slot, int epoch, int num_pairs, int k,
                     int H, int E_loc, int max_rows, int align, const int* group_off, const int* group_rows,
                     int* done_counter, int* status, const int* route_owner, int num_groups, cudaStream_t st) {
    if (!g_peers_set) return -10;
    ScatterArgs a;
    a.src = (const bf16*)src; a.scale = scale; a.idx = idx; a.pos = pos; a.dst_row = dst_row; a.pair_row = pair_row;
    a.dst_off = dst_off; a.flags_off = flags_off; a.slot = slot; a.epoch = epoch; a.num_pairs = num_pairs; a.k = k;
    a.H = H; a.E_loc = E_loc; a.max_rows = max_rows; a.group_off = group_off; a.group_rows = group_rows;
    a.pair_blocks = (num_pairs + 7) / 8; a.align = align; a.done_counter = done_counter; a.status = status;
    a.route_owner = route_owner; a.num_groups = num_groups > 0 ? num_groups : E_loc;
    const int pad_blocks = a.num_groups < 64 ? a.num_groups : 64;
    const int grid = a.pair_blocks + pad_blocks;
    if (H == 256) scatter_rows_kernel<1><<<grid, 256, 0, st>>>(g_peers, a);
    else if (H == 512) scatter_rows_kernel<2><<<grid, 256, 0, st>>>(g_peers, a);
    else if (H == 1024) scatter_rows_kernel<4><<<grid, 256, 0, st>>>(g_peers, a);
    else return -2;
    return -(int)cudaGetLastError();
}

int lah_signal_wait(long long flags_off, int slot, int epoch, int do_signal, int do_wait, int* status,
                    cudaStream_t st) {
    if (!g_peers_set) return -10;
    signal_wait_kernel<<<1, 32, 0, st>>>(g_peers, flags_off, slot, epoch, do_signal, do_wait, status);
    return -(int)cudaGetLastError();
}

int lah_combine_rows(long long src_off, const int* idx, const int* pair_row, const float* w, void* out, int B, int k,
                     int H, int E_loc, long long flags_off, int slot, int epoch, int do_signal, int do_wait, int* status,
                     const int* route_owner, const void* addend, cudaStream_t st) {
    if (!g_peers_set) return -10;
    if (B <= 0) return 0;
    CombineArgs a;
    a.src_off = src_off; a.idx = idx; a.pair_row = pair_row; a.w = w; a.out = (bf16*)out; a.B = B; a.k = k; a.H = H;
    a.E_loc = E_loc; a.flags_off = flags_off; a.slot = slot; a.epoch = epoch; a.do_signal = do_signal; a.do_wait = do_wait;
    a.status = status; a.route_owner = route_owner;
    const int grid = (B + 7) / 8;
    const bf16* add = (const bf16*)addend;
    if (add && (reinterpret_cast<uintptr_t>(add) % 16)) return -3;
#define LAH_COMBINE(V)                                                                   \
    if (add) combine_rows_kernel<V, true><<<grid, 256, 0, st>>>(g_peers, a, add);        \
    else combine_rows_kernel<V, false><<<grid, 256, 0, st>>>(g_peers, a, nullptr);
    if (H == 256) { LAH_COMBINE(1) }
    else if (H == 512) { LAH_COMBINE(2) }
    else if (H == 1024) { LAH_COMBINE(4) }
    else return -2;
#undef LAH_COMBINE
    return -(int)cudaGetLastError();
}

int lah_gate_bwd(long long yo_off, const void* grad, const int* idx, const int* pair_row, const float* w,
                 float* dlogits, int B, int k, int H, int E_loc, const int* grid_sizes, int ndim, const int* route_owner,
                 const float* sig, float scale, int norm, const float* lse, const float* logits,
                 const unsigned char* alive, cudaStream_t st) {
    if (!g_peers_set) return -10;
    const bool dense = !sig && norm == 0;
    if (norm != 0 && norm != 1) return -5;
    if (dense ? B > 0 && (!lse || !logits) : lse || logits || alive) return -5;
    if (B <= 0) return 0;
    GridSpec gs;
    if (make_grid_spec(&gs, grid_sizes, ndim)) return -2;
    if (k > MAX_K) return -3;
    if (sig || dense ? !(scale > 0.f && scale <= FLT_MAX) : scale != 1.f) return -5;
    if (dense && (gs.num_experts > LAYOUT_MAX_E || router_bwd_warp_floats(gs) > GATE_BWD_DENSE_MAX_FLOATS)) return -2;
    GateBwdArgs a;
    a.yo_off = yo_off; a.grad = (const bf16*)grad; a.idx = idx; a.pair_row = pair_row; a.w = w; a.dlogits = dlogits;
    a.B = B; a.k = k; a.H = H; a.E_loc = E_loc; a.route_owner = route_owner;
    int e;
#define LAH_GATE_BWD(V)                                                                                     \
    e = sig ? (norm ? launch_gate_bwd<V, true, true>(a, gs, sig, scale, nullptr, nullptr, nullptr, st)      \
                    : launch_gate_bwd<V, true, false>(a, gs, sig, scale, nullptr, nullptr, nullptr, st))    \
            : (norm ? launch_gate_bwd<V, false, true>(a, gs, nullptr, 1.f, nullptr, nullptr, nullptr, st)   \
                    : launch_gate_bwd<V, false, false>(a, gs, nullptr, scale, logits, lse, alive, st));
    if (H == 256) { LAH_GATE_BWD(1) }
    else if (H == 512) { LAH_GATE_BWD(2) }
    else if (H == 1024) { LAH_GATE_BWD(4) }
    else return -2;
#undef LAH_GATE_BWD
    if (e) return e;
    return -(int)cudaGetLastError();
}

static int router_grid_spec(GridSpec* gs, const int* grid, int ndim) {
    if (!grid || ndim < 1 || ndim > MAX_GRID_DIMS) return -2;
    long long total = 0, experts = 1;
    for (int d = 0; d < ndim; ++d) {
        if (grid[d] < 1) return -2;
        total += grid[d];
        experts *= grid[d];
        if (total > LAYOUT_MAX_E || experts > LAYOUT_MAX_E) return -2;
    }
    return make_grid_spec(gs, grid, ndim);
}

int lah_router_loss_fwd(const float* logits, int B, const int* grid, int ndim, const unsigned char* alive, const int* counts,
                        int count_rows, float* f, float* z, float* Fb, float* loss, float* partials, int* ticket,
                        int score_mode, cudaStream_t st) {
    GridSpec gs;
    if (router_grid_spec(&gs, grid, ndim)) return -2;
    if (B < 0 || count_rows < 1 || count_rows > MAX_WORLD) return -3;
    if (!counts || !f || !loss || (B > 0 && (!logits || !z || !Fb || !partials || !ticket))) return -4;
    if (score_mode != 0 && score_mode != 1) return -5;
    if (int e = score_mode ? set_max_dynamic_smem<router_loss_fwd_kernel<true>>(RL_WARPS * sizeof(float) * LAYOUT_MAX_E)
                           : set_max_dynamic_smem<router_loss_fwd_kernel<false>>(RL_WARPS * sizeof(float) * LAYOUT_MAX_E))
        return e;
    router_f_kernel<<<1, 1024, 0, st>>>(counts, count_rows, gs.num_experts, alive, f, B, loss);
    const int blocks = (B + RL_WARPS - 1) / RL_WARPS;
    const size_t smem = RL_WARPS * gs.total * sizeof(float);
    if (B > 0 && score_mode)
        router_loss_fwd_kernel<true><<<blocks, RL_WARPS * 32, smem, st>>>(logits, B, gs, alive, f, z, Fb, partials, ticket,
                                                                          loss);
    else if (B > 0)
        router_loss_fwd_kernel<false><<<blocks, RL_WARPS * 32, smem, st>>>(logits, B, gs, alive, f, z, Fb, partials, ticket,
                                                                           loss);
    return -(int)cudaGetLastError();
}

int lah_router_loss_bwd(const float* logits, int B, const int* grid, int ndim, const unsigned char* alive, const float* f,
                        const float* z, const float* Fb, float aux_coef, float z_coef, float* dlogits, int score_mode,
                        cudaStream_t st) {
    GridSpec gs;
    if (router_grid_spec(&gs, grid, ndim)) return -2;
    if (B < 0) return -3;
    if (B > 0 && (!logits || !f || !z || !Fb || !dlogits)) return -4;
    if (score_mode != 0 && (score_mode != 1 || z_coef != 0.f)) return -5;
    if (int e = score_mode ? launch_router_loss_bwd<true>(logits, B, gs, alive, f, z, Fb, aux_coef, z_coef, dlogits, st)
                           : launch_router_loss_bwd<false>(logits, B, gs, alive, f, z, Fb, aux_coef, z_coef, dlogits, st))
        return e;
    return B == 0 ? 0 : -(int)cudaGetLastError();
}

int lah_expert_bias_update(const int* counts, int count_rows, int E, const unsigned char* alive, float rate, float* bias,
                           cudaStream_t st) {
    if (E < 1 || E > LAYOUT_MAX_E) return -2;
    if (count_rows < 1 || count_rows > MAX_WORLD) return -3;
    if (!counts || !bias) return -4;
    if (!(rate >= 0.f && rate <= FLT_MAX)) return -5;
    expert_bias_update_kernel<<<1, 1024, 0, st>>>(counts, count_rows, E, alive, rate, bias);
    return -(int)cudaGetLastError();
}

static int make_seg_layout(SegLayout* L, int num_segs, const long long* seg_n, int slots) {
    if (num_segs < 1 || num_segs > 12) return -2;
    L->num_segs = num_segs;
    long long off = 0;
    for (int s = 0; s < 12; ++s) {
        L->seg_start[s] = off;
        L->seg_n[s] = s < num_segs ? seg_n[s] : 8;
        if (s < num_segs) {
            if (seg_n[s] % 8) return -2;
            off += seg_n[s] * slots;
        }
    }
    L->seg_start[12] = off;
    return 0;
}

int lah_pull_shadow(const int* shadow_info, int S_max, int E_loc, long long p_off, long long pbf16_off, int num_segs,
                    const long long* seg_n, int small_mask, cudaStream_t st) {
    if (!g_peers_set) return -10;
    if (S_max <= 0) return 0;
    PullArgs a;
    a.shadow_info = shadow_info; a.E_loc = E_loc; a.p_off = p_off; a.pbf16_off = pbf16_off; a.small_mask = small_mask;
    if (make_seg_layout(&a.L, num_segs, seg_n, E_loc + S_max)) return -2;
    pull_shadow_kernel<<<dim3(64, S_max), 256, 0, st>>>(g_peers, a);
    return -(int)cudaGetLastError();
}

int lah_zero_slots(float* g, int num_segs, const long long* seg_n, int slots, int first_slot, int num_slots, int seg_mask,
                   cudaStream_t st) {
    if (num_slots <= 0) return 0;
    SegLayout L;
    if (make_seg_layout(&L, num_segs, seg_n, slots)) return -2;
    zero_slots_kernel<<<dim3(8, num_segs), 256, 0, st>>>(g, L, first_slot, num_slots, seg_mask);
    return -(int)cudaGetLastError();
}

}
```

learning-at-home_b200/csrc/sm90.cuh:

```cuda
#pragma once

#include <cuda.h>
#include <cuda_runtime.h>
#include <cuda_bf16.h>
#include <stdint.h>

namespace lah {

typedef __nv_bfloat16 bf16;

__device__ __forceinline__ uint32_t smem_u32(const void* p) {
    return static_cast<uint32_t>(__cvta_generic_to_shared(p));
}

__device__ __forceinline__ uint32_t elect_one_sync() {
    uint32_t pred = 0;
    asm volatile(
        "{\n"
        ".reg .pred P1;\n"
        "elect.sync _|P1, 0xffffffff;\n"
        "selp.b32 %0, 1, 0, P1;\n"
        "}\n"
        : "=r"(pred));
    return pred;
}

__device__ __forceinline__ void mbar_init(uint64_t* bar, uint32_t count) {
    asm volatile("mbarrier.init.shared::cta.b64 [%0], %1;" ::"r"(smem_u32(bar)), "r"(count) : "memory");
}
__device__ __forceinline__ void fence_mbar_init() {
    asm volatile("fence.mbarrier_init.release.cluster;" ::: "memory");
}
__device__ __forceinline__ void fence_proxy_async_smem() {
    asm volatile("fence.proxy.async.shared::cta;" ::: "memory");
}
__device__ __forceinline__ void mbar_arrive_expect_tx(uint64_t* bar, uint32_t bytes) {
    asm volatile("mbarrier.arrive.expect_tx.shared::cta.b64 _, [%0], %1;" ::"r"(smem_u32(bar)), "r"(bytes)
                 : "memory");
}
__device__ __forceinline__ void mbar_arrive(uint64_t* bar) {
    asm volatile("mbarrier.arrive.shared::cta.b64 _, [%0];" ::"r"(smem_u32(bar)) : "memory");
}
__device__ __forceinline__ uint32_t mbar_try_wait(uint64_t* bar, uint32_t parity) {
    uint32_t ok;
    asm volatile(
        "{\n"
        ".reg .pred p;\n"
        "mbarrier.try_wait.parity.shared::cta.b64 p, [%1], %2;\n"
        "selp.b32 %0, 1, 0, p;\n"
        "}\n"
        : "=r"(ok)
        : "r"(smem_u32(bar)), "r"(parity)
        : "memory");
    return ok;
}
__device__ __forceinline__ void mbar_wait(uint64_t* bar, uint32_t parity) {
    while (!mbar_try_wait(bar, parity)) {
    }
}

__device__ __forceinline__ void tma_prefetch_desc(const CUtensorMap* tm) {
    asm volatile("prefetch.tensormap [%0];" ::"l"(reinterpret_cast<uint64_t>(tm)) : "memory");
}
__device__ __forceinline__ void tma_load_2d(void* smem_dst, const CUtensorMap* tm, uint64_t* bar, int c0, int c1) {
    asm volatile(
        "cp.async.bulk.tensor.2d.shared::cluster.global.mbarrier::complete_tx::bytes [%0], [%1, {%3, %4}], [%2];"
        ::"r"(smem_u32(smem_dst)), "l"(reinterpret_cast<uint64_t>(tm)), "r"(smem_u32(bar)), "r"(c0), "r"(c1)
        : "memory");
}
__device__ __forceinline__ void tma_load_3d(void* smem_dst, const CUtensorMap* tm, uint64_t* bar, int c0, int c1,
                                            int c2) {
    asm volatile(
        "cp.async.bulk.tensor.3d.shared::cluster.global.mbarrier::complete_tx::bytes [%0], [%1, {%3, %4, %5}], [%2];"
        ::"r"(smem_u32(smem_dst)), "l"(reinterpret_cast<uint64_t>(tm)), "r"(smem_u32(bar)), "r"(c0), "r"(c1), "r"(c2)
        : "memory");
}
__device__ __forceinline__ void tma_store_2d(const CUtensorMap* tm, const void* smem_src, int c0, int c1) {
    asm volatile("cp.async.bulk.tensor.2d.global.shared::cta.bulk_group [%0, {%2, %3}], [%1];" ::"l"(
                     reinterpret_cast<uint64_t>(tm)),
                 "r"(smem_u32(smem_src)), "r"(c0), "r"(c1)
                 : "memory");
}
__device__ __forceinline__ void tma_store_3d(const CUtensorMap* tm, const void* smem_src, int c0, int c1, int c2) {
    asm volatile("cp.async.bulk.tensor.3d.global.shared::cta.bulk_group [%0, {%2, %3, %4}], [%1];" ::"l"(
                     reinterpret_cast<uint64_t>(tm)),
                 "r"(smem_u32(smem_src)), "r"(c0), "r"(c1), "r"(c2)
                 : "memory");
}
// ... 117 lines not shown

__device__ __forceinline__ uint64_t make_smem_desc_sw64(uint32_t saddr, uint32_t lbo_bytes, uint32_t sbo_bytes) {
    uint64_t d = 0;
    d |= static_cast<uint64_t>((saddr & 0x3FFFFu) >> 4);
    d |= static_cast<uint64_t>((lbo_bytes >> 4) & 0x3FFFu) << 16;
    d |= static_cast<uint64_t>((sbo_bytes >> 4) & 0x3FFFu) << 32;
    d |= static_cast<uint64_t>(2) << 62;
    return d;
}

template <int COLS>
__device__ __forceinline__ uint64_t make_smem_desc_cols(uint32_t saddr, uint32_t lbo_bytes) {
    static_assert(COLS == 32 || COLS == 64, "atoms are 32 or 64 bf16 columns wide");
    if constexpr (COLS == 32) return make_smem_desc_sw64(saddr, lbo_bytes, 512);
    else return make_smem_desc_sw128(saddr, lbo_bytes, 1024);
}

__device__ __forceinline__ void named_bar_sync(int id, int threads) {
    asm volatile("bar.sync %0, %1;" ::"r"(id), "r"(threads) : "memory");
}

__device__ __forceinline__ void st_release_sys(int* p, int v) {
    asm volatile("st.release.sys.global.s32 [%0], %1;" ::"l"(p), "r"(v) : "memory");
}
__device__ __forceinline__ int ld_acquire_sys(const int* p) {
    int v;
    asm volatile("ld.acquire.sys.global.s32 %0, [%1];" : "=r"(v) : "l"(p) : "memory");
    return v;
}
__device__ __forceinline__ void red_add_release_sys(int* p, int v) {
    asm volatile("red.release.sys.global.add.s32 [%0], %1;" ::"l"(p), "r"(v) : "memory");
}
__device__ __forceinline__ int ld_acquire_gpu(const int* p) {
    int v;
    asm volatile("ld.acquire.gpu.global.s32 %0, [%1];" : "=r"(v) : "l"(p) : "memory");
    return v;
}
__device__ __forceinline__ int4 ld_nc_v4(const int4* p) {
    int4 r;
    asm volatile("ld.global.nc.L1::no_allocate.v4.s32 {%0, %1, %2, %3}, [%4];"
                 : "=r"(r.x), "=r"(r.y), "=r"(r.z), "=r"(r.w)
                 : "l"(p));
    return r;
}
__device__ __forceinline__ int4 ld_v4(const int4* p) {
    int4 r;
    asm volatile("ld.global.v4.s32 {%0, %1, %2, %3}, [%4];" : "=r"(r.x), "=r"(r.y), "=r"(r.z), "=r"(r.w) : "l"(p));
    return r;
}
__device__ __forceinline__ void st_v4(int4* p, const int4& v) {
    asm volatile("st.global.v4.s32 [%0], {%1, %2, %3, %4};" ::"l"(p), "r"(v.x), "r"(v.y), "r"(v.z), "r"(v.w)
                 : "memory");
}

__device__ __forceinline__ bool spin_flag_ge(const int* flag, int epoch) {
    const long long t0 = clock64();
    while (ld_acquire_sys(flag) < epoch) {
        if (clock64() - t0 > 20000000000ll) return false;
    }
    return true;
}
__device__ __forceinline__ bool spin_flag_ft(const int* flag, int epoch, int* status, int rank, int timeout_ms) {
    if (status) {
        const volatile int* vs = status;
        if ((vs[1] >> rank) & 1) return false;
        if (vs[0] & 1) return false;
    }
    const long long t0 = clock64();
    const long long limit = timeout_ms > 0 ? static_cast<long long>(timeout_ms) * 2000000ll : 20000000000ll;
    while (ld_acquire_sys(flag) < epoch) {
        if (clock64() - t0 > limit) {
            if (status) atomicOr(status, 1);
            return false;
        }
    }
    return true;
}
__device__ __forceinline__ unsigned long long globaltimer_ns() {
    unsigned long long t;
    asm volatile("mov.u64 %0, %%globaltimer;" : "=l"(t));
    return t;
}
__device__ __forceinline__ void fence_proxy_async_global() { asm volatile("fence.proxy.async.global;" ::: "memory"); }

__device__ __forceinline__ uint32_t pack_bf16x2(float lo, float hi) {
    __nv_bfloat162 v = __floats2bfloat162_rn(lo, hi);
    return *reinterpret_cast<uint32_t*>(&v);
}
__device__ __forceinline__ float2 unpack_bf16x2(uint32_t u) {
    __nv_bfloat162 v = *reinterpret_cast<__nv_bfloat162*>(&u);
    return __bfloat1622float2(v);
}
__device__ __forceinline__ float split_decode(uint32_t hi, uint32_t lo, bool tie_up) {
    const uint32_t up = (lo > 0x8000u || (lo == 0x8000u && tie_up)) ? 1u : 0u;
    return __uint_as_float(((hi - up) << 16) | lo);
}
__device__ __forceinline__ uint32_t split_tie_up(float p) {
    const uint32_t b = __float_as_uint(p);
    return ((b & 0xffffu) == 0x8000u && (b & 0x10000u)) ? 0x80000000u : 0u;
}
__device__ __forceinline__ float with_tie_bit(float v, uint32_t tie) { return __uint_as_float(__float_as_uint(v) | tie); }
__device__ __forceinline__ float without_tie_bit(float v) { return __uint_as_float(__float_as_uint(v) & 0x7fffffffu); }
__device__ __forceinline__ float warp_sum(float v) {
#pragma unroll
    for (int o = 16; o > 0; o >>= 1) v += __shfl_xor_sync(0xffffffffu, v, o);
    return v;
}
__device__ __forceinline__ float warp_max(float v) {
#pragma unroll
    for (int o = 16; o > 0; o >>= 1) v = fmaxf(v, __shfl_xor_sync(0xffffffffu, v, o));
    return v;
}

inline int make_tmap(CUtensorMap* tm, CUtensorMapDataType dtype, int rank, const void* ptr, const uint64_t* dims,
                     const uint64_t* strides_bytes, const uint32_t* box,
                     CUtensorMapSwizzle swizzle = CU_TENSOR_MAP_SWIZZLE_128B) {
    typedef CUresult (*EncodeTiled)(CUtensorMap*, CUtensorMapDataType, cuuint32_t, void*, const cuuint64_t*,
                                    const cuuint64_t*, const cuuint32_t*, const cuuint32_t*, CUtensorMapInterleave,
                                    CUtensorMapSwizzle, CUtensorMapL2promotion, CUtensorMapFloatOOBfill);
    static const EncodeTiled encode = [] {
        void* fn = nullptr;
        cudaDriverEntryPointQueryResult qres;
        if (cudaGetDriverEntryPoint("cuTensorMapEncodeTiled", &fn, cudaEnableDefault, &qres) != cudaSuccess) fn = nullptr;
        return reinterpret_cast<EncodeTiled>(fn);
    }();
    if (!encode) return -100;
    cuuint64_t gdims[3], gstr[2];
    cuuint32_t gbox[3], estr[3] = {1, 1, 1};
    for (int i = 0; i < rank; ++i) {
        gdims[i] = dims[i];
        gbox[i] = box[i];
    }
    for (int i = 0; i < rank - 1; ++i) gstr[i] = strides_bytes[i];
    const CUresult r = encode(tm, dtype, rank, const_cast<void*>(ptr), gdims, gstr, gbox, estr, CU_TENSOR_MAP_INTERLEAVE_NONE,
                              swizzle, CU_TENSOR_MAP_L2_PROMOTION_L2_256B, CU_TENSOR_MAP_FLOAT_OOB_FILL_NONE);
    return r == CUDA_SUCCESS ? 0 : -1000 - static_cast<int>(r);
}

inline int num_sms() {
    static const int sms = [] {
        int dev = 0, n = 0;
        cudaGetDevice(&dev);
        cudaDeviceGetAttribute(&n, cudaDevAttrMultiProcessorCount, dev);
        return n;
    }();
    return sms;
}

inline int persistent_grid(long long total_tiles, int max_ctas) {
    int grid = num_sms();
    if (max_ctas > 0 && max_ctas < grid) grid = max_ctas;
    if (total_tiles < grid) grid = static_cast<int>(total_tiles);
    return grid;
}

template <auto Kernel>
inline int set_max_dynamic_smem(int bytes) {
    static bool done = false;
    if (!done) {
        const cudaError_t e = cudaFuncSetAttribute(Kernel, cudaFuncAttributeMaxDynamicSharedMemorySize, bytes);
        if (e != cudaSuccess) return -static_cast<int>(e);
        done = true;
    }
    return 0;
}

}
```

learning-at-home_b200/csrc/small_m.cu:

```cuda
#include "sm90.cuh"
#include <climits>

namespace lah {
namespace smallm {

constexpr int BM = 128;
constexpr int BK = 64;
constexpr int MMA_K = 16;
constexpr int BN_MAX = 128;
constexpr int NUM_THREADS = 288;

namespace sab {

constexpr int STAGES = 6;
constexpr int A_BYTES = BM * BK * 2;
constexpr int B_BYTES = BN_MAX * BK * 2;
constexpr int STAGE_BYTES = A_BYTES + B_BYTES;
constexpr int BAR_OFFSET = STAGES * STAGE_BYTES;
constexpr int QD = 4;
constexpr int MAX_G = 1023;
constexpr int CUM_OFFSET = BAR_OFFSET + (2 * STAGES + 2 * QD) * 8 + QD * 4 + 16;
constexpr int SMEM_TOTAL = CUM_OFFSET + (MAX_G + 1) * 4 + 1024;
static_assert(SMEM_TOTAL <= 232448, "shared memory budget");

struct Params {
    int G, M_out, K;
    const int* group_off;
    const int* group_rows;
    bf16* out;
    long long ldo;
    const float* bias;
    const bf16* residual;
    long long ldr;
    const int* wait_flags;
    int wait_count, wait_epoch;
    const int* epoch_base;
    int* status;
    int* tile_counter;
};

__device__ __forceinline__ int box_rows_of(int nn) { return nn <= 16 ? 16 : (nn <= 32 ? 32 : (nn <= 64 ? 64 : 128)); }

__device__ __forceinline__ int find_group(const int* cum, int G, int gc) {
    int lo = 0, hi = G - 1;
    while (lo < hi) {
        const int mid = (lo + hi + 1) >> 1;
        if (cum[mid] <= gc) lo = mid; else hi = mid - 1;
    }
    return lo;
}

template <int NB, bool A_MN>
__device__ __forceinline__ void sab_tile(const Params& p, uint8_t* smem, uint64_t* full_bar, uint64_t* empty_bar, int& stage,
                                         uint32_t& phase, int num_kb, int wg, int warp, int lane, int g, int ms, int row0,
                                         int nn) {
    float acc[NB / 2];
    constexpr uint32_t A_KSTEP = A_MN ? MMA_K * 128 : MMA_K * 2;
    int prev_stage = -1;
    for (int kb = 0; kb < num_kb; ++kb) {
        mbar_wait(&full_bar[stage], phase);
        const uint32_t sa = smem_u32(smem + stage * STAGE_BYTES) + wg * (A_MN ? BK * 128 : 64 * 128);
        const uint32_t sb = smem_u32(smem + stage * STAGE_BYTES + A_BYTES);
        wgmma_fence();
#pragma unroll
        for (int k = 0; k < BK / MMA_K; ++k) {
            const uint64_t da = make_smem_desc_sw128(sa + k * A_KSTEP, BK * 128, 1024);
            const uint64_t db = make_smem_desc_sw128(sb + k * (MMA_K * 2), 0, 1024);
            const uint32_t accum = (kb > 0 || k > 0) ? 1u : 0u;
            if constexpr (NB == 16) wgmma_bf16_n16<A_MN, 0>(acc, da, db, accum);
            if constexpr (NB == 32) wgmma_bf16_n32<A_MN, 0>(acc, da, db, accum);
            if constexpr (NB == 64) wgmma_bf16_n64<A_MN, 0>(acc, da, db, accum);
            if constexpr (NB == 128) wgmma_bf16_n128<A_MN, 0>(acc, da, db, accum);
        }
        wgmma_commit();
        wgmma_wait<1>();
        if (prev_stage >= 0) {
            __syncwarp();
            if (lane == 0) mbar_arrive(&empty_bar[prev_stage]);
        }
        prev_stage = stage;
        if (++stage == STAGES) {
            stage = 0;
            phase ^= 1;
        }
    }
    wgmma_wait<0>();
    wgmma_fence_regs(acc);
    __syncwarp();
    if (lane == 0 && prev_stage >= 0) mbar_arrive(&empty_bar[prev_stage]);

    const int n16 = (nn + 15) & ~15;
#pragma unroll
    for (int h = 0; h < 2; ++h) {
        const int feat = ms * BM + wg * 64 + (warp & 3) * 16 + (lane >> 2) + 8 * h;
        const float bias = p.bias ? __ldg(p.bias + static_cast<long long>(g) * p.M_out + feat) : 0.f;
#pragma unroll
        for (int j = 0; j < NB / 8; ++j) {
#pragma unroll
            for (int e = 0; e < 2; ++e) {
                const int n = 8 * j + 2 * (lane & 3) + e;
                if (n < n16) {
                    const long long row = row0 + n;
                    float v = acc[4 * j + 2 * h + e] + bias;
                    if (p.residual) v += __bfloat162float(p.residual[row * p.ldr + feat]);
                    p.out[row * p.ldo + feat] = __float2bfloat16(v);
                }
            }
        }
    }
}

template <bool A_MN>
__global__ void __launch_bounds__(NUM_THREADS, 1)
swapab_kernel(const Params p, const __grid_constant__ CUtensorMap tmA, const __grid_constant__ CUtensorMap tmB16,
              const __grid_constant__ CUtensorMap tmB32, const __grid_constant__ CUtensorMap tmB64,
              const __grid_constant__ CUtensorMap tmB128) {
    extern __shared__ uint8_t smem_raw[];
    uint8_t* smem = reinterpret_cast<uint8_t*>((reinterpret_cast<uintptr_t>(smem_raw) + 1023) & ~uintptr_t(1023));
    uint64_t* full_bar = reinterpret_cast<uint64_t*>(smem + BAR_OFFSET);
    uint64_t* empty_bar = full_bar + STAGES;
    uint64_t* q_full = empty_bar + STAGES;
    uint64_t* q_empty = q_full + QD;
    volatile int* q_tile = reinterpret_cast<volatile int*>(q_empty + QD);
    int* cum = reinterpret_cast<int*>(smem + CUM_OFFSET);

    const int warp = threadIdx.x >> 5;
    const int lane = threadIdx.x & 31;

    if (warp == 0) {
        int carry = 0;
        for (int base = 0; base < p.G; base += 32) {
            const int g = base + lane;
            int x = g < p.G ? (__ldg(p.group_rows + g) + BN_MAX - 1) / BN_MAX : 0;
#pragma unroll
            for (int d = 1; d < 32; d <<= 1) {
                const int y = __shfl_up_sync(0xffffffffu, x, d);
                if (lane >= d) x += y;
            }
            if (g < p.G) cum[g + 1] = carry + x;
            carry += __shfl_sync(0xffffffffu, x, 31);
        }
        if (lane == 0) cum[0] = 0;
    }
    if (warp == 8 && lane == 0) {
        tma_prefetch_desc(&tmA);
        tma_prefetch_desc(&tmB16);
        tma_prefetch_desc(&tmB32);
        tma_prefetch_desc(&tmB64);
        tma_prefetch_desc(&tmB128);
        for (int i = 0; i < STAGES; ++i) {
            mbar_init(&full_bar[i], 1);
            mbar_init(&empty_bar[i], 8);
        }
        for (int i = 0; i < QD; ++i) {
            mbar_init(&q_full[i], 1);
            mbar_init(&q_empty[i], 8);
        }
        fence_mbar_init();
    }
    __syncthreads();

    const int m_slices = p.M_out / BM;
    const int total = cum[p.G] * m_slices;
    const int num_kb = p.K / BK;

    if (warp == 8) {
        if (lane != 0) return;
        if (p.wait_flags) {
            const int epoch = p.wait_epoch + (p.epoch_base ? *p.epoch_base : 0);
            const unsigned long long t_wait = globaltimer_ns();
            for (int sidx = 0; sidx < p.wait_count; ++sidx)
                spin_flag_ft(p.wait_flags + sidx, epoch, p.status, sidx, p.epoch_base ? p.epoch_base[1] : 0);
            if (blockIdx.x == 0) atomicAdd(reinterpret_cast<unsigned long long*>(p.status + 2), globaltimer_ns() - t_wait);
            fence_proxy_async_global();
        }
        int stage = 0, qi = 0;
        uint32_t phase = 0, qphase = 0;
        while (true) {
            const int tile = atomicAdd(p.tile_counter, 1);
            mbar_wait(&q_empty[qi], qphase ^ 1);
            q_tile[qi] = tile;
            mbar_arrive(&q_full[qi]);
            if (++qi == QD) {
                qi = 0;
                qphase ^= 1;
            }
            if (tile >= total) break;
            const int gc = tile / m_slices, ms = tile - gc * m_slices;
            const int g = find_group(cum, p.G, gc);
            const int n0 = (gc - cum[g]) * BN_MAX;
            const int rows = __ldg(p.group_rows + g);
            const int off = __ldg(p.group_off + g);
            const int box = box_rows_of(min(rows - n0, BN_MAX));
            const CUtensorMap* tmB = box == 16 ? &tmB16 : (box == 32 ? &tmB32 : (box == 64 ? &tmB64 : &tmB128));
            for (int kb = 0; kb < num_kb; ++kb) {
                mbar_wait(&empty_bar[stage], phase ^ 1);
                uint8_t* sa = smem + stage * STAGE_BYTES;
                uint8_t* sb = sa + A_BYTES;
                const int k = kb * BK;
                mbar_arrive_expect_tx(&full_bar[stage], A_BYTES + box * 128);
                if (!A_MN) {
                    tma_load_3d(sa, &tmA, &full_bar[stage], k, ms * BM, g);
                } else {
#pragma unroll
                    for (int i = 0; i < BM / 64; ++i)
                        tma_load_3d(sa + i * (BK * 128), &tmA, &full_bar[stage], ms * BM + i * 64, k, g);
                }
                tma_load_2d(sb, tmB, &full_bar[stage], k, off + n0);
                if (++stage == STAGES) {
                    stage = 0;
                    phase ^= 1;
                }
            }
        }
        return;
    }

    const int wg = warp >> 2;
    int stage = 0, qi = 0;
    uint32_t phase = 0, qphase = 0;
    while (true) {
        mbar_wait(&q_full[qi], qphase);
        const int tile = q_tile[qi];
        __syncwarp();
        if (lane == 0) mbar_arrive(&q_empty[qi]);
        if (++qi == QD) {
            qi = 0;
            qphase ^= 1;
        }
        if (tile >= total) break;
        const int gc = tile / m_slices, ms = tile - gc * m_slices;
        const int g = find_group(cum, p.G, gc);
        const int n0 = (gc - cum[g]) * BN_MAX;
        const int nn = min(__ldg(p.group_rows + g) - n0, BN_MAX);
        const int row0 = __ldg(p.group_off + g) + n0;
        switch (box_rows_of(nn)) {
            case 16: sab_tile<16, A_MN>(p, smem, full_bar, empty_bar, stage, phase, num_kb, wg, warp, lane, g, ms, row0, nn); break;
            case 32: sab_tile<32, A_MN>(p, smem, full_bar, empty_bar, stage, phase, num_kb, wg, warp, lane, g, ms, row0, nn); break;
            case 64: sab_tile<64, A_MN>(p, smem, full_bar, empty_bar, stage, phase, num_kb, wg, warp, lane, g, ms, row0, nn); break;
            default: sab_tile<128, A_MN>(p, smem, full_bar, empty_bar, stage, phase, num_kb, wg, warp, lane, g, ms, row0, nn); break;
        }
    }
}

}

namespace wa {

constexpr int WBK = 32;
constexpr int OP_STAGES = 2;
constexpr int OP_STAGE_BYTES = 2 * (WBK * BM * 2);
constexpr int OP_BYTES = OP_STAGES * OP_STAGE_BYTES;
constexpr int BAND_ROWS = 4;
constexpr int CHUNKS = 16 / BAND_ROWS;
constexpr int SUB_COLS = 32;
constexpr int SUB_BYTES = BM / CHUNKS * SUB_COLS * 4;
constexpr int ARR_BYTES = (BN_MAX / SUB_COLS) * SUB_BYTES;
constexpr int ST_STAGES = 3;
constexpr int ST_STAGE_BYTES = 4 * ARR_BYTES;
constexpr int ST_OFFSET = OP_BYTES;
constexpr int BAR_OFFSET = ST_OFFSET + ST_STAGES * ST_STAGE_BYTES;
constexpr int QD = 4;
constexpr int SMEM_TOTAL = BAR_OFFSET + (2 * OP_STAGES + 2 * ST_STAGES + 2 * QD) * 8 + QD * 4 + 16 + 1024;
static_assert(ST_STAGES <= CHUNKS, "the producer issues a tile's first ST_STAGES chunks before its remaining k-blocks");
static_assert(OP_STAGE_BYTES % 1024 == 0 && SUB_BYTES % 1024 == 0, "128-B swizzle atoms need 1 KB alignment");
static_assert(SMEM_TOTAL <= 232448, "shared memory budget");

struct Params {
    int G, N, K;
    const int* group_off;
    const int* group_rows;
    const int* skip;
    const int* step;
    float* p;
    float* m;
    float* v;
    float* vmax;
    bf16* p_bf16;
    float lr, beta1, beta2, eps;
    int amsgrad;
    float wd;
    int* tile_counter;
    const int* poison;
};
static_assert(sizeof(Params) == 128 && sizeof(Params) % alignof(CUtensorMap) == 0, "Params layout");

constexpr int WD_NONE = 0, WD_L2 = 1, WD_DECOUPLED = 2;

struct Tile {
    int g, mt, nt;
};

template <bool SPLIT>
struct StateMaps {
    CUtensorMap a[SPLIT ? 5 : 4];
};
constexpr int PLANE_COLS = 64;
constexpr int PLANE_BYTES = ARR_BYTES / 2;
static_assert(PLANE_BYTES == (BN_MAX / PLANE_COLS) * SUB_BYTES, "a plane box has the rows and bytes of an fp32 box");

template <bool SPLIT>
__device__ __forceinline__ void state_chunk_tma(const StateMaps<SPLIT>& tm, int n_arr, uint8_t* ss, uint64_t* bar, int col0,
                                                int srow, int c) {
    if constexpr (SPLIT) {
        for (int a = 0; a < 2; ++a)
#pragma unroll
            for (int q = 0; q < BN_MAX / PLANE_COLS; ++q) {
                uint8_t* s = ss + a * PLANE_BYTES + q * SUB_BYTES;
                if (bar) tma_load_3d(s, &tm.a[a], bar, col0 + q * PLANE_COLS, BAND_ROWS * c, srow / 16);
                else tma_store_3d(&tm.a[a], s, col0 + q * PLANE_COLS, BAND_ROWS * c, srow / 16);
            }
    }
    for (int a = SPLIT ? 1 : 0; a < n_arr; ++a)
#pragma unroll
        for (int q = 0; q < BN_MAX / SUB_COLS; ++q) {
            uint8_t* s = ss + a * ARR_BYTES + q * SUB_BYTES;
            const CUtensorMap* m = &tm.a[SPLIT ? a + 1 : a];
            if (bar) tma_load_3d(s, m, bar, col0 + q * SUB_COLS, BAND_ROWS * c, srow / 16);
            else tma_store_3d(m, s, col0 + q * SUB_COLS, BAND_ROWS * c, srow / 16);
        }
}

template <int WD, bool DEV_LR, bool SPLIT>
__global__ void __launch_bounds__(NUM_THREADS, 1)
wgrad_adam_kernel(const Params p, const __grid_constant__ CUtensorMap tmDY, const __grid_constant__ CUtensorMap tmX,
                  const __grid_constant__ StateMaps<SPLIT> tmS, const float* __restrict__ lr_dev) {
    extern __shared__ uint8_t smem_raw[];
    uint8_t* smem = reinterpret_cast<uint8_t*>((reinterpret_cast<uintptr_t>(smem_raw) + 1023) & ~uintptr_t(1023));
    uint8_t* st_smem = smem + ST_OFFSET;
    uint64_t* op_full = reinterpret_cast<uint64_t*>(smem + BAR_OFFSET);
    uint64_t* op_empty = op_full + OP_STAGES;
    uint64_t* st_full = op_empty + OP_STAGES;
    uint64_t* st_empty = st_full + ST_STAGES;
    uint64_t* q_full = st_empty + ST_STAGES;
    uint64_t* q_empty = q_full + QD;
    volatile int* q_tile = reinterpret_cast<volatile int*>(q_empty + QD);

    const int warp = threadIdx.x >> 5;
    const int lane = threadIdx.x & 31;
    if (p.poison && (*p.poison & 1)) return;
    const int n_arr = p.amsgrad ? 4 : 3;

    if (warp == 8 && lane == 0) {
        tma_prefetch_desc(&tmDY);
        tma_prefetch_desc(&tmX);
        for (int a = 0; a < n_arr + (SPLIT ? 1 : 0); ++a) tma_prefetch_desc(&tmS.a[a]);
        for (int i = 0; i < OP_STAGES; ++i) {
            mbar_init(&op_full[i], 1);
            mbar_init(&op_empty[i], 8);
        }
        for (int i = 0; i < ST_STAGES; ++i) {
            mbar_init(&st_full[i], 1);
            mbar_init(&st_empty[i], 1);
        }
        for (int i = 0; i < QD; ++i) {
            mbar_init(&q_full[i], 1);
            mbar_init(&q_empty[i], 8);
        }
        fence_mbar_init();
    }
    __syncthreads();

    const int n_tiles = p.K / BN_MAX;
    const int tiles_per_group = (p.N / BM) * n_tiles;
    const int total = p.G * tiles_per_group;
    auto decode = [&](int tile) {
        Tile t;
        t.g = tile / tiles_per_group;
        const int r = tile - t.g * tiles_per_group;
        t.mt = r / n_tiles;
        t.nt = r - t.mt * n_tiles;
        return t;
    };

    if (warp == 8) {
        if (lane != 0) return;
        uint32_t phase = 0, qphase = 0, sphase = 0;
        int qi = 0, stage = 0, sstage = 0;
        while (true) {
            int tile;
            while (true) {
                tile = atomicAdd(p.tile_counter, 1);
                if (tile >= total) break;
                const int g = tile / tiles_per_group;
                if (__ldg(p.group_rows + g) > 0 && !(p.skip && __ldg(p.skip + 2 * g) >= 0)) break;
                atomicMax(p.tile_counter, (g + 1) * tiles_per_group);
            }
            mbar_wait(&q_empty[qi], qphase ^ 1);
            q_tile[qi] = tile;
            mbar_arrive(&q_full[qi]);
            if (++qi == QD) {
                qi = 0;
                qphase ^= 1;
            }
            if (tile >= total) break;
            const Tile t = decode(tile);
            const int off = __ldg(p.group_off + t.g), rows = __ldg(p.group_rows + t.g);
            const int srow = t.g * p.N + t.mt * BM;
            auto load_chunk = [&](int c) {
                mbar_wait(&st_empty[sstage], sphase ^ 1);
                mbar_arrive_expect_tx(&st_full[sstage], n_arr * ARR_BYTES);
                state_chunk_tma(tmS, n_arr, st_smem + sstage * ST_STAGE_BYTES, &st_full[sstage], t.nt * BN_MAX, srow, c);
                if (++sstage == ST_STAGES) {
                    sstage = 0;
                    sphase ^= 1;
                }
            };
            for (int t0 = 0; t0 < rows; t0 += WBK) {
                mbar_wait(&op_empty[stage], phase ^ 1);
                mbar_arrive_expect_tx(&op_full[stage], OP_STAGE_BYTES);
                uint8_t* sa = smem + stage * OP_STAGE_BYTES;
                uint8_t* sb = sa + WBK * BM * 2;
#pragma unroll
                for (int i = 0; i < BM / 64; ++i)
                    tma_load_2d(sa + i * (WBK * 128), &tmDY, &op_full[stage], t.mt * BM + i * 64, off + t0);
#pragma unroll
                for (int i = 0; i < BN_MAX / 64; ++i)
                    tma_load_2d(sb + i * (WBK * 128), &tmX, &op_full[stage], t.nt * BN_MAX + i * 64, off + t0);
                if (++stage == OP_STAGES) {
                    stage = 0;
                    phase ^= 1;
                }
                if (t0 == 0)
                    for (int c = 0; c < ST_STAGES; ++c) load_chunk(c);
            }
            for (int c = ST_STAGES; c < CHUNKS; ++c) load_chunk(c);
        }
        return;
    }

    float lr = p.lr, wd = p.wd;
    if constexpr (DEV_LR) {
        lr = lr_dev[0];
        if constexpr (WD == WD_DECOUPLED) wd = lr_dev[1];
    }
    const int wg = warp >> 2;
    int qi = 0, stage = 0, sstage = 0;
    uint32_t phase = 0, qphase = 0, sphase = 0;
    float acc[BN_MAX / 2];
    float xg[BN_MAX / 8];
    const int lrow = wg * 64 + (warp & 3) * 16 + (lane >> 2);
    const int brow = (lane >> 2) & 3;
    const int R = warp * BAND_ROWS + brow;
    const int jflip = 2 * (brow & 1);
    while (true) {
        mbar_wait(&q_full[qi], qphase);
        const int tile = q_tile[qi];
        __syncwarp();
        if (lane == 0) mbar_arrive(&q_empty[qi]);
        if (++qi == QD) {
            qi = 0;
            qphase ^= 1;
        }
        if (tile >= total) break;
        const Tile t = decode(tile);
        const int rows = __ldg(p.group_rows + t.g);
        int prev_stage = -1;
        for (int t0 = 0; t0 < rows; t0 += WBK) {
            mbar_wait(&op_full[stage], phase);
            const uint32_t sa = smem_u32(smem + stage * OP_STAGE_BYTES) + wg * (WBK * 128);
            const uint32_t sb = smem_u32(smem + stage * OP_STAGE_BYTES + WBK * BM * 2);
            const int ksteps = min(WBK / MMA_K, (rows - t0 + MMA_K - 1) / MMA_K);
            wgmma_fence();
            for (int k = 0; k < ksteps; ++k) {
                const uint64_t da = make_smem_desc_sw128(sa + k * (MMA_K * 128), WBK * 128, 1024);
                const uint64_t db = make_smem_desc_sw128(sb + k * (MMA_K * 128), WBK * 128, 1024);
                wgmma_bf16_n128<1, 1>(acc, da, db, (t0 > 0 || k > 0) ? 1u : 0u);
            }
            wgmma_commit();
            wgmma_wait<1>();
            if (prev_stage >= 0) {
                __syncwarp();
                if (lane == 0) mbar_arrive(&op_empty[prev_stage]);
            }
            prev_stage = stage;
            if (++stage == OP_STAGES) {
                stage = 0;
                phase ^= 1;
// ... 80 lines not shown
                state_chunk_tma(tmS, n_arr, ss, nullptr, t.nt * BN_MAX, srow, c);
                tma_store_commit();
                tma_store_wait_read<0>();
                mbar_arrive(&st_empty[sstage]);
            }
            if (++sstage == ST_STAGES) {
                sstage = 0;
                sphase ^= 1;
            }
            if (c == 1) {
#pragma unroll
                for (int j = 0; j < BN_MAX / 8; ++j) {
                    acc[4 * j] = acc[4 * j + 2];
                    acc[4 * j + 1] = acc[4 * j + 3];
                }
            }
        }
    }
    if (threadIdx.x == 0) tma_store_wait<0>();
}

}
}
}

using namespace lah;
using namespace lah::smallm;

extern "C" const int* lah_get_epoch_base();

static int* tile_counter() {
    static int* ctr = nullptr;
    if (!ctr) {
        if (cudaMalloc(&ctr, 256) != cudaSuccess) return nullptr;
        cudaMemset(ctr, 0, 256);
    }
    return ctr;
}
static const int* g_poison = nullptr;

extern "C" {

int lah_set_poison_word(const int* status) {
    g_poison = status;
    return 0;
}
const int* lah_get_poison_word() { return g_poison; }

int lah_swapab_linear(const void* x, long long ldx, int x_rows, const void* W, int G, int M_out, int K, int a_mn,
                      void* out, long long ldo, const int* group_off, const int* group_rows, const float* bias,
                      const void* residual, long long ldr, const int* wait_flags, int wait_count, int wait_epoch,
                      int* status, int max_ctas, cudaStream_t st) {
    if ((K % BK) || (M_out % BM) || (ldx % 8) || G > sab::MAX_G) return -2;
    CUtensorMap tmA, tmB[4];
    if (!a_mn) {
        uint64_t dims[3] = {(uint64_t)K, (uint64_t)M_out, (uint64_t)G};
        uint64_t str[2] = {(uint64_t)K * 2, (uint64_t)M_out * K * 2};
        uint32_t box[3] = {BK, BM, 1};
        int r = make_tmap(&tmA, CU_TENSOR_MAP_DATA_TYPE_BFLOAT16, 3, W, dims, str, box);
        if (r) return r;
    } else {
        uint64_t dims[3] = {(uint64_t)M_out, (uint64_t)K, (uint64_t)G};
        uint64_t str[2] = {(uint64_t)M_out * 2, (uint64_t)M_out * K * 2};
        uint32_t box[3] = {64, BK, 1};
        int r = make_tmap(&tmA, CU_TENSOR_MAP_DATA_TYPE_BFLOAT16, 3, W, dims, str, box);
        if (r) return r;
    }
    const uint32_t boxes[4] = {16, 32, 64, 128};
    for (int i = 0; i < 4; ++i) {
        uint64_t dims[2] = {(uint64_t)K, (uint64_t)x_rows};
        uint64_t str[1] = {(uint64_t)ldx * 2};
        uint32_t box[2] = {BK, boxes[i]};
        int r = make_tmap(&tmB[i], CU_TENSOR_MAP_DATA_TYPE_BFLOAT16, 2, x, dims, str, box);
        if (r) return r;
    }
    sab::Params p;
    p.G = G; p.M_out = M_out; p.K = K; p.group_off = group_off; p.group_rows = group_rows; p.out = (bf16*)out; p.ldo = ldo;
    p.bias = bias; p.residual = (const bf16*)residual; p.ldr = ldr; p.wait_flags = wait_flags; p.wait_count = wait_count;
    p.wait_epoch = wait_epoch; p.epoch_base = lah_get_epoch_base(); p.status = status;
    p.tile_counter = tile_counter();
    if (!p.tile_counter) return -3;
    const long long total = 1ll * (M_out / BM) * (G + x_rows / BN_MAX);
    if (total <= 0 || G <= 0) return 0;
    if (cudaMemsetAsync(p.tile_counter, 0, sizeof(int), st) != cudaSuccess) return -4;
    const int ctas = persistent_grid(total, max_ctas);
    if (!a_mn) {
        if (int e = set_max_dynamic_smem<sab::swapab_kernel<false>>(sab::SMEM_TOTAL)) return e;
        sab::swapab_kernel<false><<<ctas, NUM_THREADS, sab::SMEM_TOTAL, st>>>(p, tmA, tmB[0], tmB[1], tmB[2], tmB[3]);
    } else {
        if (int e = set_max_dynamic_smem<sab::swapab_kernel<true>>(sab::SMEM_TOTAL)) return e;
        sab::swapab_kernel<true><<<ctas, NUM_THREADS, sab::SMEM_TOTAL, st>>>(p, tmA, tmB[0], tmB[1], tmB[2], tmB[3]);
    }
    return -(int)cudaGetLastError();
}

}

template <int WD, bool DEV_LR, bool SPLIT>
static int launch_wgrad_adam(const wa::Params& a, const CUtensorMap& tmDY, const CUtensorMap& tmX,
                             const wa::StateMaps<SPLIT>& tmS, const float* lr_dev, int ctas, cudaStream_t st) {
    if (int e = set_max_dynamic_smem<wa::wgrad_adam_kernel<WD, DEV_LR, SPLIT>>(wa::SMEM_TOTAL)) return e;
    wa::wgrad_adam_kernel<WD, DEV_LR, SPLIT><<<ctas, NUM_THREADS, wa::SMEM_TOTAL, st>>>(a, tmDY, tmX, tmS, lr_dev);
    return -(int)cudaGetLastError();
}

template <bool SPLIT>
static int wgrad_adam(const void* dy, long long lddy, const void* x, long long ldx, int total_rows, int G, int N, int K,
                      const int* group_off, const int* group_rows, const int* skip, const int* step, void* p, void* lo,
                      float* m, float* v, float* vmax, void* p_bf16, float lr, const float* lr_dev, float beta1, float beta2,
                      float eps, int amsgrad, float weight_decay, float decay, int decoupled, int max_ctas, cudaStream_t st) {
    if ((N % BM) || (K % BN_MAX) || (lddy % 8) || (ldx % 8) || 1ll * G * N > INT_MAX) return -2;
    if (decoupled && weight_decay != 0.f) return -2;
    if (amsgrad && !vmax) return -2;
    CUtensorMap tmDY, tmX;
    wa::StateMaps<SPLIT> tmS;
    {
        void* arrs[5] = {p, m, v, amsgrad ? vmax : (float*)m, nullptr};
        if (SPLIT) {
            arrs[1] = lo; arrs[2] = m; arrs[3] = v; arrs[4] = amsgrad ? vmax : m;
        }
        uint64_t dims[3] = {(uint64_t)K, 16, (uint64_t)G * N / 16};
        uint64_t str[2] = {(uint64_t)K * 4, (uint64_t)K * 64};
        uint32_t box[3] = {wa::SUB_COLS, wa::BAND_ROWS, BM / 16};
        for (int a = 0; a < (SPLIT ? 5 : 4); ++a) {
            int r;
            if (SPLIT && a < 2) {
                uint64_t pstr[2] = {(uint64_t)K * 2, (uint64_t)K * 32};
                uint32_t pbox[3] = {wa::PLANE_COLS, wa::BAND_ROWS, BM / 16};
                r = make_tmap(&tmS.a[a], CU_TENSOR_MAP_DATA_TYPE_BFLOAT16, 3, arrs[a], dims, pstr, pbox);
            } else {
                r = make_tmap(&tmS.a[a], CU_TENSOR_MAP_DATA_TYPE_FLOAT32, 3, arrs[a], dims, str, box);
            }
            if (r) return r;
        }
    }
    {
        uint64_t dims[2] = {(uint64_t)N, (uint64_t)total_rows};
        uint64_t str[1] = {(uint64_t)lddy * 2};
        uint32_t box[2] = {64, wa::WBK};
        int r = make_tmap(&tmDY, CU_TENSOR_MAP_DATA_TYPE_BFLOAT16, 2, dy, dims, str, box);
        if (r) return r;
    }
    {
        uint64_t dims[2] = {(uint64_t)K, (uint64_t)total_rows};
        uint64_t str[1] = {(uint64_t)ldx * 2};
        uint32_t box[2] = {64, wa::WBK};
        int r = make_tmap(&tmX, CU_TENSOR_MAP_DATA_TYPE_BFLOAT16, 2, x, dims, str, box);
        if (r) return r;
    }
    wa::Params a;
    a.G = G; a.N = N; a.K = K; a.group_off = group_off; a.group_rows = group_rows; a.skip = skip; a.step = step;
    a.p = SPLIT ? nullptr : (float*)p; a.m = m; a.v = v; a.vmax = vmax; a.p_bf16 = (bf16*)p_bf16; a.lr = lr; a.beta1 = beta1; a.beta2 = beta2; a.eps = eps; a.amsgrad = amsgrad;
    a.wd = decoupled ? decay : weight_decay;
    a.tile_counter = tile_counter() ? tile_counter() + 16 : nullptr;
    a.poison = g_poison;
    if (!a.tile_counter) return -3;
    const long long total = 1ll * G * (N / BM) * (K / BN_MAX);
    if (total <= 0) return 0;
    if (cudaMemsetAsync(a.tile_counter, 0, sizeof(int), st) != cudaSuccess) return -4;
    const int ctas = persistent_grid(total, max_ctas);
    if (lr_dev) {
        if (decoupled) return launch_wgrad_adam<wa::WD_DECOUPLED, true, SPLIT>(a, tmDY, tmX, tmS, lr_dev, ctas, st);
        if (weight_decay != 0.f) return launch_wgrad_adam<wa::WD_L2, true, SPLIT>(a, tmDY, tmX, tmS, lr_dev, ctas, st);
        return launch_wgrad_adam<wa::WD_NONE, true, SPLIT>(a, tmDY, tmX, tmS, lr_dev, ctas, st);
    }
    if (decoupled) return launch_wgrad_adam<wa::WD_DECOUPLED, false, SPLIT>(a, tmDY, tmX, tmS, nullptr, ctas, st);
    if (weight_decay != 0.f) return launch_wgrad_adam<wa::WD_L2, false, SPLIT>(a, tmDY, tmX, tmS, nullptr, ctas, st);
    return launch_wgrad_adam<wa::WD_NONE, false, SPLIT>(a, tmDY, tmX, tmS, nullptr, ctas, st);
}

extern "C" {

int lah_wgrad_adam(const void* dy, long long lddy, const void* x, long long ldx, int total_rows, int G, int N, int K,
                   const int* group_off, const int* group_rows, const int* skip, const int* step, float* p, float* m,
                   float* v, float* vmax, void* p_bf16, float lr, const float* lr_dev, float beta1, float beta2, float eps,
                   int amsgrad, float weight_decay, float decay, int decoupled, int max_ctas, cudaStream_t st) {
    return wgrad_adam<false>(dy, lddy, x, ldx, total_rows, G, N, K, group_off, group_rows, skip, step, p, nullptr, m, v,
                             vmax, p_bf16, lr, lr_dev, beta1, beta2, eps, amsgrad, weight_decay, decay, decoupled, max_ctas,
                             st);
}

int lah_wgrad_adam_split(const void* dy, long long lddy, const void* x, long long ldx, int total_rows, int G, int N, int K,
                         const int* group_off, const int* group_rows, const int* skip, const int* step, void* hi, void* lo,
                         float* m, float* v, float* vmax, float lr, const float* lr_dev, float beta1, float beta2, float eps,
                         int amsgrad, float weight_decay, float decay, int decoupled, int max_ctas, cudaStream_t st) {
    if (!hi || !lo) return -2;
    return wgrad_adam<true>(dy, lddy, x, ldx, total_rows, G, N, K, group_off, group_rows, skip, step, hi, lo, m, v, vmax,
                            nullptr, lr, lr_dev, beta1, beta2, eps, amsgrad, weight_decay, decay, decoupled, max_ctas, st);
}

}
```

learning-at-home_b200/ops/kernels.py:

```python
import ctypes
import math

import torch
import torch.nn.functional as F

from . import native
from .native import c_void_p, c_int, c_ll, c_float, ptr, stream_ptr

c_ull = ctypes.c_ulonglong
_configured = False

SLOT_COUNTS, SLOT_DISPATCH, SLOT_OUTPUT, SLOT_GRAD, SLOT_DINPUT, SLOT_TRAINER, SLOT_BARRIER, SLOT_SHADOW = range(8)
NUM_SLOTS = 8
MAX_WORLD = 8
STATUS_TIMEOUT, STATUS_OVERFLOW = 1, 2


def _lib():
    global _configured
    lib = native.cuda_lib()
    if _configured:
        return lib
    P, I, L, Fl = c_void_p, c_int, c_ll, c_float
    sigs = {
        "lah_ln_relu_fwd": [P, P, P, P, P, P, P, I, I, I, I, P],
        "lah_ln_relu_bwd": [P, P, P, P, P, P, P, P, P, P, P, P, I, I, I, I, P, P],
        "lah_grouped_colsum": [P, L, P, P, I, P, I, I, P],
        "lah_set_step_counters": [P],
        "lah_set_multicast": [c_ull],
        "lah_set_poison_word": [P],
        "lah_nvls_allreduce": [L, L, Fl, P],
        "lah_heartbeat": [L, I, I, L, P],
        "lah_alive_from_heartbeats": [P, P, I, L, L, P],
        "lah_set_spin_timeout_ms": [I],
        "lah_step_begin": [I, L, P],
        "lah_swapab_linear": [P, L, I, P, I, I, I, I, P, L, P, P, P, P, L, P, I, I, P, I, P],
        "lah_wgrad_adam": [P, L, P, L, I, I, I, I, P, P, P, P, P, P, P, P, P, Fl, P, Fl, Fl, Fl, I, Fl, Fl, I, I, P],
        "lah_wgrad_adam_split": [P, L, P, L, I, I, I, I, P, P, P, P, P, P, P, P, P, Fl, P, Fl, Fl, Fl, I, Fl, Fl, I, I, P],
        "lah_ln_relu_fwd_q": [P, P, P, P, P, P, P, I, I, I, P, P, P],
        "lah_set_peers": [P, I, I],
        "lah_set_wait_counter": [P],
        "lah_gate_topk": [P, I, P, I, I, P, Fl, c_ull, L, P, P, P, P, P, I, Fl, P, I, I, I, P, P],
        "lah_expert_bias_update": [P, I, I, P, Fl, P, P],
        "lah_layout_exchange": [L, L, I, I, I, I, I, I, I, P, P, P, P, P, P, P, I, Fl, I, P, P, P, P, P],
        "lah_scatter_rows": [P, P, P, P, P, P, L, L, I, I, I, I, I, I, I, I, P, P, P, P, P, I, P],
        "lah_pull_shadow": [P, I, I, L, L, I, P, I, P],
        "lah_zero_slots": [P, I, P, I, I, I, I, P],
        "lah_signal_wait": [L, I, I, I, I, P, P],
        "lah_combine_rows": [L, P, P, P, P, I, I, I, I, L, I, I, I, I, P, P, P, P],
        "lah_gate_bwd": [L, P, P, P, P, P, I, I, I, I, P, I, P, P, Fl, I, P, P, P, P],
        "lah_router_loss_fwd": [P, I, P, I, P, P, I, P, P, P, P, P, P, I, P],
        "lah_router_loss_bwd": [P, I, P, I, P, P, P, P, Fl, Fl, P, I, P],
        "lah_adam_step": [P, P, P, P, P, P, I, P, I, P, P, I, Fl, P, Fl, Fl, Fl, Fl, I, I, I, L, P, Fl, I, P, L, I, I, I, Fl,
                          I, P],
        "lah_bump_steps": [P, P, I, P],
        "lah_cast_bf16": [P, P, L, P],
        "lah_split_master": [P, P, P, P, L, I, P],
        "lah_attention_fwd": [P, P, P, L, I, I, I, c_ull, I, Fl, P, P],
        "lah_attention_bwd": [P, P, P, P, P, P, P, L, I, I, I, c_ull, I, Fl, P, P],
        "lah_attention_fwd_causal": [P, P, P, L, I, I, I, c_ull, I, Fl, P],
        "lah_attention_bwd_causal": [P, P, P, P, P, P, P, L, I, I, I, c_ull, I, Fl, P],
        "lah_pack_key_mask": [P, P, L, I, P],
        "lah_dropout_mask": [P, I, I, I, I, I, c_ull, I, P],
        "lah_dropout_ew": [I, P, P, P, L, I, c_ull, I, I, Fl, P],
        "lah_rms_norm_fwd": [P, P, P, P, I, I, Fl, P, I, P],
        "lah_rms_norm_bwd": [P, P, P, P, P, P, P, I, I, I, P, P, P],
        "lah_swiglu_fwd": [P, P, L, I, P],
        "lah_swiglu_bwd": [P, P, P, L, I, P],
        "lah_symm_alloc": [c_ull, ctypes.POINTER(c_void_p)],
        "lah_symm_free": [P],
        "lah_symm_get_handle": [P, ctypes.c_char_p],
        "lah_symm_open_handle": [ctypes.c_char_p, ctypes.POINTER(c_void_p)],
        "lah_symm_close_handle": [P],
        "lah_device_sync": [],
    }
    for name, argtypes in sigs.items():
        fn = getattr(lib, name)
        fn.restype = c_int
        fn.argtypes = argtypes
    _configured = True
    return lib


def _grid_array(grid_size):
    return (c_int * len(grid_size))(*[int(g) for g in grid_size])


def _check_ln_width(C, what, max_width=None):
    if max_width is None and not ln_width_ok(C):
        raise ValueError(f"{what}: width {C} is not a multiple of {LN_WIDTH_STEP} in [{LN_WIDTH_STEP}, {LN_MAX_WIDTH}]")
    if max_width is not None and (C <= 0 or C % LN_WIDTH_STEP):
        raise ValueError(f"{what}: width {C} is not a positive multiple of {LN_WIDTH_STEP}")


def ln_relu_fwd(h, gamma, beta, tile_group, *, out, mean, rstd, relu=True, quant=None, tile_rows=128):
    rows, C = h.shape
    _check_ln_width(C, "ln_relu_fwd")
    assert h.is_contiguous() and gamma.dtype == torch.float32 and (out is None or out.is_contiguous())
    if quant is not None:
        assert quant.K == C and quant.groups == 1 and quant.rows_per_group >= rows and quant.tile_rows == 128
        native.check(_lib().lah_ln_relu_fwd_q(ptr(h), ptr(out), ptr(mean), ptr(rstd), ptr(gamma), ptr(beta),
                                              ptr(tile_group), rows, C, int(relu), ptr(quant.q), ptr(quant.sf),
                                              stream_ptr()), "lah_ln_relu_fwd_q")
    else:
        native.check(_lib().lah_ln_relu_fwd(ptr(h), ptr(out), ptr(mean), ptr(rstd), ptr(gamma), ptr(beta),
                                            ptr(tile_group), rows, C, int(relu), int(tile_rows), stream_ptr()),
                     "lah_ln_relu_fwd")
    native.count_launch()
    return out


def ln_relu_bwd(da, h, mean, rstd, gamma, beta, tile_group, *, dh, dgamma, dbeta, dbias, relu=True, tile_rows=128,
                dres=None):
    rows, C = h.shape
    _check_ln_width(C, "ln_relu_bwd")
    assert da.is_contiguous() and h.is_contiguous() and dh.is_contiguous()
    assert dres is None or (dres.shape == h.shape and dres.dtype == torch.bfloat16 and dres.is_contiguous())
    part = torch.empty((rows + tile_rows - 1) // tile_rows, 3, C, device=h.device, dtype=torch.float32)
    native.check(_lib().lah_ln_relu_bwd(ptr(da), ptr(h), ptr(mean), ptr(rstd), ptr(gamma), ptr(beta), ptr(dh),
                                        ptr(dgamma), ptr(dbeta), ptr(dbias), ptr(part), ptr(tile_group), rows, C,
                                        int(relu), int(tile_rows), ptr(dres), stream_ptr()), "lah_ln_relu_bwd")
    native.count_launch(2)
    return dh


def _bf16_rows(t, what, shape):
    if t.dtype != torch.bfloat16 or not t.is_contiguous() or tuple(t.shape) != tuple(shape):
        raise ValueError(f"{what}: expected a contiguous bf16 tensor of shape {tuple(shape)}, got {t.dtype} "
                         f"{tuple(t.shape)}{'' if t.is_contiguous() else ' (not contiguous)'}")


def _f32_vec(t, what, n):
    if t.dtype != torch.float32 or not t.is_contiguous() or t.numel() != n:
        raise ValueError(f"{what}: expected a contiguous float32 tensor of {n} elements, got {t.dtype} {tuple(t.shape)}")


def _check_rms_groups(what, gamma, tile_group, tile_rows, rows, C):
    if tile_rows < 8 or tile_rows & (tile_rows - 1):
# ... 721 lines not shown
    arr = None
    if peer_bases is not None:
        arr = (c_ull * len(peer_bases))(*[int(b) for b in peer_bases])
    if isinstance(seg_sizes, int):
        seg_sizes = [seg_sizes]
    segs = (c_ll * len(seg_sizes))(*[int(s) for s in seg_sizes])
    if lr_dev is not None:
        _check_lr_dev(lr_dev)
    l2, decay = weight_decay_args(lr, weight_decay, decoupled)
    native.check(_lib().lah_adam_step(ptr(p), ptr(g), ptr(m), ptr(v), ptr(vmax), ptr(p_bf16), len(seg_sizes),
                                      ctypes.cast(segs, c_void_p), G, ptr(step), ptr(group_rows), int(step_scalar), lr,
                                      ptr(lr_dev), betas[0], betas[1], eps, l2, int(amsgrad), int(zero_mask), world,
                                      peer_grad_off, ctypes.cast(arr, c_void_p) if arr is not None else c_void_p(0),
                                      grad_scale, int(G_active), ptr(shadow_of), int(shadow_g_off), int(me), int(seg_mask),
                                      int(dead_mask), decay, int(bool(decoupled and weight_decay)), stream_ptr()),
                 "lah_adam_step")
    native.count_launch()


def swapab_linear(x, w, group_off, group_rows, *, out, bias=None, residual=None, w_is_kn=False, wait=None, max_ctas=0):
    assert x.dtype == torch.bfloat16 and w.dtype == torch.bfloat16 and out.dtype == torch.bfloat16 and w.is_contiguous()
    rows, K = x.shape
    G = w.shape[0]
    M_out = w.shape[2] if w_is_kn else w.shape[1]
    assert (w.shape[1] if w_is_kn else w.shape[2]) == K and x.stride(1) == 1 and out.stride(1) == 1
    wait_flags, wait_count, wait_epoch, wait_status = (wait[0], wait[0].numel(), wait[1], wait[2]) if wait else (None, 0, 0, None)
    native.check(_lib().lah_swapab_linear(ptr(x), x.stride(0), rows, ptr(w), G, M_out, K, int(w_is_kn), ptr(out),
                                          out.stride(0), ptr(group_off), ptr(group_rows), ptr(bias), ptr(residual),
                                          residual.stride(0) if residual is not None else 0, ptr(wait_flags), wait_count,
                                          wait_epoch, ptr(wait_status), int(max_ctas), stream_ptr()),
                 "lah_swapab_linear")
    native.count_launch()
    return out


def swapab_linear_ref(x, w, group_off, group_rows, *, bias=None, residual=None, w_is_kn=False):
    off, rows = group_off.tolist(), group_rows.tolist()
    M_out = w.shape[2] if w_is_kn else w.shape[1]
    out = torch.zeros(x.shape[0], M_out, dtype=torch.float32, device=x.device)
    for g, (o, r) in enumerate(zip(off, rows)):
        if r <= 0:
            continue
        wg = w[g].float()
        y = x[o:o + r].float() @ (wg if w_is_kn else wg.t())
        if bias is not None:
            y = y + bias.view(w.shape[0], M_out)[g]
        if residual is not None:
            y = y + residual[o:o + r].float()
        out[o:o + r] = y
    return out


def wgrad_adam(dy, x, group_off, group_rows, *, p, m, v, vmax, p_bf16, step, skip=None, lr=1e-3, betas=(0.9, 0.999),
               eps=1e-8, amsgrad=True, weight_decay=0.0, decoupled=False, max_ctas=0, lr_dev=None, p_lo=None):
    G, N, Kd = (p if p_lo is None else p_lo).shape
    assert dy.shape[1] == N and x.shape[1] == Kd and dy.shape[0] == x.shape[0]
    assert dy.dtype == torch.bfloat16 and x.dtype == torch.bfloat16
    if p_lo is None:
        assert p.is_contiguous() and p.dtype == torch.float32
    else:
        assert p is None and p_lo.dtype == torch.int16 and p_bf16.dtype == torch.bfloat16
        assert p_lo.is_contiguous() and p_bf16.is_contiguous() and p_bf16.shape[1:] == p_lo.shape[1:]
    if amsgrad and vmax is None:
        raise ValueError("wgrad_adam: amsgrad needs a vmax tensor (vmax=None only with amsgrad=False)")
    if lr_dev is not None:
        _check_lr_dev(lr_dev)
    l2, decay = weight_decay_args(lr, weight_decay, decoupled)
    common = (ptr(dy), dy.stride(0), ptr(x), x.stride(0), dy.shape[0], G, N, Kd, ptr(group_off), ptr(group_rows),
              ptr(skip), ptr(step))
    tail = (lr, ptr(lr_dev), betas[0], betas[1], eps, int(amsgrad), l2, decay, int(bool(decoupled and weight_decay)),
            int(max_ctas), stream_ptr())
    if p_lo is None:
        native.check(_lib().lah_wgrad_adam(*common, ptr(p), ptr(m), ptr(v), ptr(vmax), ptr(p_bf16), *tail),
                     "lah_wgrad_adam")
    else:
        native.check(_lib().lah_wgrad_adam_split(*common, ptr(p_bf16), ptr(p_lo), ptr(m), ptr(v), ptr(vmax), *tail),
                     "lah_wgrad_adam_split")
    native.count_launch()


def bump_steps(step, group_rows):
    native.check(_lib().lah_bump_steps(ptr(step), ptr(group_rows), step.numel(), stream_ptr()), "lah_bump_steps")
    native.count_launch()


def cast_bf16(src, dst):
    assert src.dtype == torch.float32 and dst.dtype == torch.bfloat16 and src.numel() == dst.numel()
    native.check(_lib().lah_cast_bf16(ptr(src), ptr(dst), src.numel(), stream_ptr()), "lah_cast_bf16")
    native.count_launch()


def _check_split(p, hi, lo, v):
    n = p.numel()
    assert p.dtype == torch.float32 and hi.dtype == torch.bfloat16 and lo.dtype == torch.int16 and v.dtype == torch.float32
    assert hi.numel() == n and lo.numel() == n and v.numel() == n
    assert all(t.is_contiguous() and t.is_cuda for t in (p, hi, lo, v))


def split_encode(p, hi, lo, v):
    _check_split(p, hi, lo, v)
    native.check(_lib().lah_split_master(ptr(p), ptr(hi), ptr(lo), ptr(v), p.numel(), 1, stream_ptr()), "lah_split_master")
    native.count_launch()


def split_decode(hi, lo, v, out):
    _check_split(out, hi, lo, v)
    native.check(_lib().lah_split_master(ptr(out), ptr(hi), ptr(lo), ptr(v), out.numel(), 0, stream_ptr()),
                 "lah_split_master")
    native.count_launch()


def product_key_scores(logits, grid_size):
    parts = torch.split(logits, list(grid_size), dim=-1)
    scores = parts[0]
    for part in parts[1:]:
        scores = (scores.unsqueeze(-1) + part.unsqueeze(-2)).flatten(-2)
    return scores


def sigmoid_weights_ref(sel, valid, scale=1.0):
    sg = torch.where(valid, torch.sigmoid(sel), torch.zeros_like(sel))
    S = sg.sum(-1, keepdim=True)
    return torch.where(S > 0, scale * sg / torch.where(S > 0, S, torch.ones_like(S)), torch.zeros_like(sg))


def softmax_lse_ref(scores, alive=None):
    live = torch.ones(scores.shape[-1], dtype=torch.bool, device=scores.device) if alive is None \
        else alive.bool().reshape(-1).to(scores.device)
    masked = scores.masked_fill(~live.view(1, -1), float("-inf"))
    ok = torch.isfinite(masked).any(-1, keepdim=True)
    z = torch.logsumexp(torch.where(ok, masked, torch.zeros_like(masked)), -1, keepdim=True)
    return torch.where(ok, z, torch.zeros_like(z)).squeeze(-1)


def softmax_weights_ref(scores, idx, alive=None, scale=1.0):
    z = softmax_lse_ref(scores, alive)
    sel = torch.gather(scores, 1, idx.clamp(min=0))
    valid = idx >= 0
    return torch.where(valid, scale * torch.exp(sel.masked_fill(~valid, 0.0) - z.unsqueeze(-1)), torch.zeros_like(sel))


def expert_group_scores_ref(scores, bias, n_group, score="softmax"):
    B, E = scores.shape
    gsz = E // n_group
    cand = torch.isfinite(scores)
    base = torch.sigmoid(scores) if score == "sigmoid" else scores
    key = base if bias is None else base + bias.to(device=scores.device, dtype=torch.float32).reshape(1, -1)
    key = key.masked_fill(~cand, float("-inf")).view(B, n_group, gsz)
    top = torch.sort(key, dim=-1, descending=True)[0]
    gscore = top[..., 0]
    if score == "sigmoid" and gsz > 1:
        gscore = torch.where(torch.isfinite(top[..., 1]), top[..., 0] + top[..., 1], top[..., 0])
    return gscore, cand.view(B, n_group, gsz).any(-1)


def expert_group_mask_ref(scores, bias, n_group, topk_group, score="softmax"):
    gscore, has = expert_group_scores_ref(scores, bias, n_group, score)
    order = torch.sort(gscore.masked_fill(~has, float("-inf")), dim=-1, descending=True, stable=True)[1]
    chosen = torch.zeros_like(has)
    chosen.scatter_(1, order[:, :topk_group], True)
    chosen &= has
    return chosen.repeat_interleave(scores.shape[1] // n_group, dim=1)


def gate_topk_ref(logits, grid_size, k, alive=None, fail_mask=None, bias=None, score="softmax", scale=1.0, n_group=1,
                  topk_group=1, norm=True):
# ... 155 lines not shown
```

learning-at-home_b200/parallel/engine.py:

```python
import math
from dataclasses import dataclass, field
from typing import Dict, List, Optional, Sequence, Tuple

import torch
import torch.nn as nn
import torch.nn.functional as F

from ..models.layers import FFN_SEG_KEYS as REF_KEYS, FFN_SEG_NAMES as SEG_NAMES, FFN_SMALL_SEG_MASK as SMALL_SEG_MASK
from ..models.layers import EXPERT_LAYOUTS, GATED_LAYOUT, GatedFeedforwardBlock, gated_inner_dim
from ..ops import fp8, gemm, kernels as K, native
from ..ops.expert_blocks import (RowPlan, ffn_backward, ffn_forward, ffn_forward_fp8, swiglu_mlp_backward,
                                 swiglu_mlp_forward)

GATED_EPS = 1e-6
SHARED_SWAPAB_ROWS = 512
SHARED_PAD = 128


@dataclass
class DMoEConfig:
    hidden: int = 512
    grid_size: Tuple[int, ...] = (8, 8)
    k: int = 4
    num_layers: int = 4
# ... 162 lines not shown
    if cfg.n_group > 1:
        raise ValueError(f"{arm} routes each token over all experts; set n_group=1 (FusedDMoE / DMoETrainer limit the "
                         "routing to the topk_group best expert groups)")


def max_groups_per_token(idx, k: int, num_experts: int, n_group: int) -> int:
    idx = idx.reshape(-1, k).long()
    if idx.numel() == 0:
        return 0
    g = torch.where(idx >= 0, idx // (num_experts // n_group), torch.full_like(idx, n_group))
    hit = torch.zeros(idx.shape[0], n_group + 1, dtype=torch.bool, device=idx.device).scatter_(1, g, True)
    return int(hit[:, :n_group].sum(1).max())


def refuse_shared_expert(cfg: DMoEConfig, arm: str):
    if cfg.shared_inner_dim > 0:
        raise ValueError(f"{arm} has no shared expert; set shared_inner_dim to 0 (FusedDMoE / DMoETrainer / "
                         "BaselineDMoE train it)")


def expert_uid(cfg: DMoEConfig, e: int) -> str:
    parts = []
    for size in reversed(cfg.grid_size):
        parts.append(str(e % size))
        e //= size
    return ".".join([cfg.uid_prefix] + parts[::-1])


class EngineContext:

    def __init__(self, cfg: DMoEConfig, group=None, device=None, heap_bytes: Optional[int] = None):
        from .symmetric import SymmetricHeap
        import torch.distributed as dist
        cfg.check_native_sizes()
        self.cfg = cfg
        self.device = device or torch.device("cuda", torch.cuda.current_device())
        distributed = dist.is_available() and dist.is_initialized()
        self.world = dist.get_world_size(group) if distributed else 1
        self.rank = dist.get_rank(group) if distributed else 0
        assert cfg.num_experts % self.world == 0, "experts must divide evenly over ranks"
        self.E = cfg.num_experts
        self.E_loc = self.E // self.world
        pairs = cfg.tokens_per_rank * cfg.k
        cap = pairs if self.world == 1 else int(math.ceil(pairs * cfg.capacity_factor))
        self.small = cfg.resolved_path(self.world) == "small"
        if self.small:
            self.align = self.tile_rows = 16
            self.S = 0
        else:
            self.align = 256 if all(n % 256 == 0 for n in cfg.gemm_widths()) else 128
            self.tile_rows = 128
            self.S = min(int(cfg.shadow_experts), 2 * K.MAX_WORLD) if self.world > 1 else 0
        self.G_tot = self.E_loc + self.S
        self.max_rows = ((cap + self.align - 1) // self.align + self.G_tot) * self.align
        self.max_rows = (self.max_rows + 127) // 128 * 128
        self.max_tiles = self.max_rows // self.tile_rows
        H = cfg.hidden
        sym_rows_bytes = self.max_rows * H * 2
        need = (3 * cfg.num_layers + 2) * (sym_rows_bytes + 4096) + K.MAX_WORLD * self.E * 4 + (32 << 20)
        if self.S:
            rec = sum(int(math.prod(shape)) for shape in cfg.seg_shapes().values())
            need += cfg.num_layers * (self.G_tot * rec * 10 + (1 << 20))
        if cfg.shared_inner_dim:
            need += cfg.num_layers * (H + 3 * H * cfg.shared_inner_dim + 256) * 4
        self.heap = SymmetricHeap(heap_bytes or need, group=group, device=self.device)
        self.flags, self.flags_off = self.heap.alloc((K.NUM_SLOTS, K.MAX_WORLD), torch.int32)
        self.cnt_all, self.cnt_all_off = self.heap.alloc((K.MAX_WORLD, self.E), torch.int32)
        i32 = dict(dtype=torch.int32, device=self.device)
        self.counts = torch.zeros(self.E, **i32)
        self.done_counter = torch.zeros(1, **i32)
        self._status_buf = torch.zeros(4, **i32)
        self.status = self._status_buf[:1]
        self.wait_ns = self._status_buf[2:4].view(torch.int64)
        K.set_wait_counter(self.wait_ns)
        self.step_ctr = torch.zeros(4, **i32)
        K.set_step_counters(self.step_ctr)
        K.set_spin_timeout_ms(cfg.peer_timeout_ms)
        self.step_ctr[1] = int(cfg.peer_timeout_ms)
        self.dead_mask = 0
        import os as _os
        octas = int(_os.environ.get("LAH_OPTIMIZER_CTAS", cfg.optimizer_ctas))
        sms = torch.cuda.get_device_properties(self.device).multi_processor_count
        if octas < 0:
            octas = sms * (17 if self.world == 1 else 18) // 28
        self.opt_ctas = octas if (self.small and 0 < octas < sms - 8) else 0
        self.chain_ctas = sms - self.opt_ctas if self.opt_ctas else 0
        self.opt_stream = torch.cuda.Stream(self.device) if self.opt_ctas else None
        self._opt_pending = False
        self.defer_join = False
        K.set_poison_word(self.status)
        self._lr_written = K.lr_block_values(cfg.lr, cfg.weight_decay, cfg.decoupled_weight_decay)
        self.lr_dev = torch.tensor(self._lr_written, dtype=torch.float32, device=self.device)
        assert 2 * cfg.num_layers + 4 < self.EPOCH_STRIDE
        self.alive = torch.ones(self.E, dtype=torch.uint8, device=self.device)
        self.hb, self.hb_off = self.heap.alloc((self.E,), torch.int64)
        self.hb.zero_()
        self._hb_stream = None
        self.epoch = 0
        self.token_counter = 0
        from .profiler import StageTimer
        self.timer = StageTimer(enabled=False)
        self.gyd, self.gyd_off = self.heap.alloc((self.max_rows, H), torch.bfloat16)
        self.dxd, self.dxd_off = self.heap.alloc((self.max_rows, H), torch.bfloat16)
        if cfg.router_losses:
            blocks = -(-cfg.tokens_per_rank // K.ROUTER_WARPS)
            self.router_partials = torch.zeros(2 * blocks, dtype=torch.float32, device=self.device)
            self.router_ticket = torch.zeros(1, dtype=torch.int32, device=self.device)
        bf = dict(dtype=torch.bfloat16, device=self.device)
        for name, width in cfg.layout.buffers(H, cfg.inner)["scratch"].items():
            setattr(self, name, torch.empty(self.max_rows, width, **bf))
        if cfg.shared_inner_dim:
            Is, R = cfg.shared_inner_dim, -(-cfg.tokens_per_rank // SHARED_PAD) * SHARED_PAD
            self.shared_da = torch.zeros(R, Is, **bf)
            self.shared_dh = torch.zeros(R, 2 * Is, **bf)
            self.shared_dn = torch.zeros(R, H, **bf)
            self.shared_dx = torch.zeros(R, H, **bf)
            tiles = torch.arange(1, R // SHARED_PAD + 1, dtype=torch.int32) * SHARED_PAD
            self.shared_go = torch.stack([torch.zeros_like(tiles), tiles], 1).to(self.device)
            self.shared_tg = torch.zeros(R // SHARED_PAD, dtype=torch.int32, device=self.device)
        self.heap.barrier()

    EPOCH_STRIDE = 64

    def adam_kwargs(self) -> Dict:
        return dict(self.cfg.adam_kwargs(), lr_dev=self.lr_dev)

    def refresh_lr(self):
        cfg = self.cfg
        vals = K.lr_block_values(cfg.lr, cfg.weight_decay, cfg.decoupled_weight_decay)
        if vals == self._lr_written or torch.cuda.is_current_stream_capturing():
            return
        self.lr_dev[0].fill_(vals[0])
        self.lr_dev[1].fill_(vals[1])
        self._lr_written = vals

    def close(self):
        K.set_wait_counter(None)
        K.set_step_counters(None)
        K.set_poison_word(None)
        self.heap.close()

    def heartbeat(self, experts=None, now: Optional[float] = None):
        import time
        first, count = experts if experts is not None else (self.rank * self.E_loc, self.E_loc)
        now_ms = int((time.time() if now is None else now) * 1000)
        if self._hb_stream is None:
            self._hb_stream = torch.cuda.Stream(self.device)
        with torch.cuda.stream(self._hb_stream):
            K.heartbeat(self.hb_off, first, count, now_ms)

    def refresh_alive(self, heartbeat_expiration: float = 120.0, now: Optional[float] = None):
        import time
        now_ms = int((time.time() if now is None else now) * 1000)
        if self._hb_stream is None:
            self._hb_stream = torch.cuda.Stream(self.device)
        with torch.cuda.stream(self._hb_stream):
            K.alive_from_heartbeats(self.hb, self.alive, now_ms, int(heartbeat_expiration * 1000))
            self._apply_dead_mask()

    def step_failed(self) -> bool:
        return bool(int(self.status.item()) & K.STATUS_TIMEOUT)

    def clear_failure(self):
        self._status_buf[0] = 0

    def detect_dead_ranks(self, max_age: float, now: Optional[float] = None):
        ages = self.heartbeat_ages(now).view(self.world, self.E_loc)
# ... 767 lines not shown
```

Measured before the change: 13740.

## Enable programmatic dependent launch across MoE, LayerNorm, Adam and wgrad kernels

Converts many kernel launches (gating, routing, scatter/combine, LayerNorm, Adam, swap-AB GEMM, fused wgrad-Adam) to launches with the programmatic-dependent-launch attribute, each guarded by griddep_wait/launch_dependents, so that one kernel's prologue can overlap the previous kernel's tail. The wgrad-Adam kernel now sets up barriers and issues L2 prefetch of optimizer state before the dependency wait. Tile counters are reset by the kernels themselves instead of by a separate memset. The optimizer CTA split ratio is retuned, and a graph-edge inspection helper is added. The main risks are ordering bugs if a kernel reads its predecessor's output before the wait, and counter-reset correctness.

```diff
diff --git a/learning-at-home_b200/csrc/adam.cu b/learning-at-home_b200/csrc/adam.cu
--- a/learning-at-home_b200/csrc/adam.cu
+++ b/learning-at-home_b200/csrc/adam.cu
@@ -21,6 +21,8 @@
 
 template <bool DECOUPLED, bool DEV_LR>
 __global__ void __launch_bounds__(256) adam_kernel(AdamArgs a) {
+    griddep_wait();
+    griddep_launch_dependents();
     if (a.poison && (*a.poison & 1)) return;
     float dev_lr = 0.f, dev_decay = 1.f;
     if constexpr (DEV_LR) {
@@ -110,6 +112,8 @@
 }
 
 __global__ void bump_steps_kernel(int* step, const int* group_rows, int G) {
+    griddep_wait();
+    griddep_launch_dependents();
     const int g = blockIdx.x * blockDim.x + threadIdx.x;
     if (g < G && group_rows[g] > 0) step[g] += 1;
 }
@@ -222,19 +226,19 @@
     if (blocks > 132 * 16) blocks = 132 * 16;
     if (lr_dev) {
         if (decoupled)
-            adam_kernel<true, true><<<(int)blocks, 256, 0, st>>>(a);
+            launch_pdl(adam_kernel<true, true>, (int)blocks, 256, 0, st, a);
         else
-            adam_kernel<false, true><<<(int)blocks, 256, 0, st>>>(a);
+            launch_pdl(adam_kernel<false, true>, (int)blocks, 256, 0, st, a);
     } else if (decoupled) {
-        adam_kernel<true, false><<<(int)blocks, 256, 0, st>>>(a);
+        launch_pdl(adam_kernel<true, false>, (int)blocks, 256, 0, st, a);
     } else {
-        adam_kernel<false, false><<<(int)blocks, 256, 0, st>>>(a);
+        launch_pdl(adam_kernel<false, false>, (int)blocks, 256, 0, st, a);
     }
     return -(int)cudaGetLastError();
 }
 
 int lah_bump_steps(int* step, const int* group_rows, int G, cudaStream_t st) {
-    bump_steps_kernel<<<(G + 255) / 256, 256, 0, st>>>(step, group_rows, G);
+    launch_pdl(bump_steps_kernel, (G + 255) / 256, 256, 0, st, step, group_rows, G);
     return -(int)cudaGetLastError();
 }
 
diff --git a/learning-at-home_b200/csrc/layernorm.cu b/learning-at-home_b200/csrc/layernorm.cu
--- a/learning-at-home_b200/csrc/layernorm.cu
+++ b/learning-at-home_b200/csrc/layernorm.cu
@@ -33,6 +33,8 @@
     const bf16* __restrict__ h, bf16* __restrict__ a, float* __restrict__ mean_out, float* __restrict__ rstd_out,
     const float* __restrict__ gamma, const float* __restrict__ beta, const int* __restrict__ tile_group, int rows,
     int relu, uint8_t* __restrict__ aq, uint8_t* __restrict__ sf, int tile_shift) {
+    griddep_wait();
+    griddep_launch_dependents();
     constexpr int NV = LnFwdCfg<C>::NV;
     constexpr bool HALF = C % 256 != 0;
     static_assert(C % 128 == 0 && C <= LN_MAX_C && !(QUANT && HALF), "unsupported LayerNorm width");
@@ -164,6 +166,8 @@
                                                             float* __restrict__ part,
                                                             const int* __restrict__ tile_group, int rows, int relu, int tile_rows,
                                                             const bf16* __restrict__ dres) {
+    griddep_wait();
+    griddep_launch_dependents();
     constexpr int THREADS = LnBwdCfg<C>::THREADS;
     constexpr int WARPS = THREADS / 32;
     constexpr bool IDLE = THREADS * 8 != C;
@@ -533,6 +537,8 @@
 __global__ void __launch_bounds__(512) grouped_colsum_kernel(const bf16* __restrict__ x, long long ldx,
                                                              float* __restrict__ part, int C,
                                                              const int* __restrict__ tile_group, int rows, int tile_rows) {
+    griddep_wait();
+    griddep_launch_dependents();
     __shared__ float2 sm[4][128];
     const int tile = blockIdx.x;
     const int g = tile_group ? __ldg(tile_group + tile) : 0;
@@ -565,6 +571,8 @@
 __global__ void __launch_bounds__(256) group_tile_sum_kernel(const float* __restrict__ part, int num_tiles, int V, int C,
                                                              const int* __restrict__ tile_group, float* out0, float* out1,
                                                              float* out2) {
+    griddep_wait();
+    griddep_launch_dependents();
     const int i = blockIdx.x * blockDim.x + threadIdx.x;
     if (i >= V * C) return;
     const int v = i / C, c = i - v * C;
@@ -595,12 +603,12 @@
     constexpr int RR = LnFwdCfg<C>::R;
     if constexpr (LnFwdCfg<C>::TUNED) {
         if (ln_rows_per_warp(RR) == 1) {
-            ln_relu_fwd_kernel<C, false, 1><<<(rows + 7) / 8, 256, 0, st>>>(
+            launch_pdl(ln_relu_fwd_kernel<C, false, 1>, (rows + 7) / 8, 256, 0, st,
                 (const bf16*)h, (bf16*)a, mean, rstd, gamma, beta, tile_group, rows, relu, nullptr, nullptr, tile_shift);
             return;
         }
     }
-    ln_relu_fwd_kernel<C, false, RR><<<(rows + 8 * RR - 1) / (8 * RR), 256, 0, st>>>(
+    launch_pdl(ln_relu_fwd_kernel<C, false, RR>, (rows + 8 * RR - 1) / (8 * RR), 256, 0, st,
         (const bf16*)h, (bf16*)a, mean, rstd, gamma, beta, tile_group, rows, relu, nullptr, nullptr, tile_shift);
 }
 
@@ -611,13 +619,13 @@
     const int grid = (rows + tile_rows - 1) / tile_rows;
     constexpr int T = LnBwdCfg<C>::THREADS;
     if (dres)
-        ln_relu_bwd_kernel<C, true><<<grid, T, 0, st>>>((const bf16*)da, (const bf16*)h, mean, rstd, gamma, beta,
+        launch_pdl(ln_relu_bwd_kernel<C, true>, grid, T, 0, st, (const bf16*)da, (const bf16*)h, mean, rstd, gamma, beta,
                                                         (bf16*)dh, part, tile_group, rows, relu, tile_rows,
                                                         (const bf16*)dres);
     else
-        ln_relu_bwd_kernel<C, false><<<grid, T, 0, st>>>((const bf16*)da, (const bf16*)h, mean, rstd, gamma, beta,
+        launch_pdl(ln_relu_bwd_kernel<C, false>, grid, T, 0, st, (const bf16*)da, (const bf16*)h, mean, rstd, gamma, beta,
                                                          (bf16*)dh, part, tile_group, rows, relu, tile_rows, nullptr);
-    group_tile_sum_kernel<<<(3 * C + 255) / 256, 256, 0, st>>>(part, grid, 3, C, tile_group, dgamma, dbeta, dbias);
+    launch_pdl(group_tile_sum_kernel, (3 * C + 255) / 256, 256, 0, st, part, grid, 3, C, tile_group, dgamma, dbeta, dbias);
 }
 
 template <int... I>
@@ -671,7 +679,7 @@
         rms_bwd_kernel_launch<C, true>(grid, dn, x, rstd, gamma, dx, part, rows, tile_rows, dres, tile_group, st);
     else
         rms_bwd_kernel_launch<C, false>(grid, dn, x, rstd, gamma, dx, part, rows, tile_rows, dres, nullptr, st);
-    group_tile_sum_kernel<<<(C + 255) / 256, 256, 0, st>>>(part, grid, 1, C, tile_group, dgamma, nullptr, nullptr);
+    launch_pdl(group_tile_sum_kernel, (C + 255) / 256, 256, 0, st, part, grid, 1, C, tile_group, dgamma, nullptr, nullptr);
 }
 
 template <int... I>
@@ -715,10 +723,10 @@
     if (C == CC) {                                                                                              \
         constexpr int RR = LnFwdCfg<CC>::R;                                                                     \
         if (ln_rows_per_warp(RR) == 1)                                                                          \
-            ln_relu_fwd_kernel<CC, true, 1><<<(rows + 7) / 8, 256, 0, st>>>(                                  \
+            launch_pdl(ln_relu_fwd_kernel<CC, true, 1>, (rows + 7) / 8, 256, 0, st,                                   \
                 (const bf16*)h, (bf16*)a, mean, rstd, gamma, beta, tile_group, rows, relu, (uint8_t*)aq, (uint8_t*)sf, 7);   \
         else                                                                                                    \
-            ln_relu_fwd_kernel<CC, true, RR><<<(rows + 8 * RR - 1) / (8 * RR), 256, 0, st>>>(                 \
+            launch_pdl(ln_relu_fwd_kernel<CC, true, RR>, (rows + 8 * RR - 1) / (8 * RR), 256, 0, st,                  \
                 (const bf16*)h, (bf16*)a, mean, rstd, gamma, beta, tile_group, rows, relu, (uint8_t*)aq, (uint8_t*)sf, 7);   \
         return -(int)cudaGetLastError();                                                                        \
     }
@@ -761,8 +769,8 @@
     if (C % 128 || shift_of(tile_rows) < 0) return -2;
     const int tiles = (rows + tile_rows - 1) / tile_rows;
     dim3 grid(tiles, (C + 255) / 256);
-    grouped_colsum_kernel<<<grid, 512, 0, st>>>((const bf16*)x, ldx, part, C, tile_group, rows, tile_rows);
-    group_tile_sum_kernel<<<(C + 255) / 256, 256, 0, st>>>(part, tiles, 1, C, tile_group, out, nullptr, nullptr);
+    launch_pdl(grouped_colsum_kernel, grid, 512, 0, st, (const bf16*)x, ldx, part, C, tile_group, rows, tile_rows);
+    launch_pdl(group_tile_sum_kernel, (C + 255) / 256, 256, 0, st, part, tiles, 1, C, tile_group, out, nullptr, nullptr);
     return -(int)cudaGetLastError();
 }
 
diff --git a/learning-at-home_b200/csrc/moe.cu b/learning-at-home_b200/csrc/moe.cu
--- a/learning-at-home_b200/csrc/moe.cu
+++ b/learning-at-home_b200/csrc/moe.cu
@@ -1,6 +1,9 @@
 #include <cfloat>
 
 #include "sm90.cuh"
+#include <cstring>
+#include <string>
+#include <vector>
 
 namespace lah {
 
@@ -289,6 +292,8 @@
                                                         const int* __restrict__ step_ctr, const float* __restrict__ bias,
                                                         float scale, float* __restrict__ sig_out, int n_group,
                                                         int topk_group, float* __restrict__ lse_out) {
+    griddep_wait();
+    griddep_launch_dependents();
     constexpr bool LSE = !NORM && !SIGMOID;
     if (step_ctr) token_offset += *reinterpret_cast<const long long*>(step_ctr + 2);
     extern __shared__ float s_logits[];
@@ -484,6 +489,8 @@
 
 __global__ void __launch_bounds__(1024) rank_slots_kernel(const int* __restrict__ idx, int n, int* __restrict__ pos,
                                                           int* __restrict__ counts) {
+    griddep_wait();
+    griddep_launch_dependents();
     __shared__ int warp_off[32];
     __shared__ int s_total;
     const int e = blockIdx.x, tid = threadIdx.x, lane = tid & 31, warp = tid >> 5;
@@ -542,6 +549,8 @@
 constexpr int LAYOUT_MAX_E = 4096;
 
 __global__ void __launch_bounds__(1024) layout_exchange_kernel(Peers peers, LayoutArgs a) {
+    griddep_wait();
+    griddep_launch_dependents();
     __shared__ int warp_tot[32];
     __shared__ int owner_base_s[MAX_WORLD + 1];
     __shared__ int s_tot[LAYOUT_MAX_E];
@@ -789,6 +798,8 @@
 
 template <int VEC_PER_LANE>
 __global__ void __launch_bounds__(256) scatter_rows_kernel(Peers peers, ScatterArgs a) {
+    griddep_wait();
+    griddep_launch_dependents();
     const int warp = threadIdx.x >> 5, lane = threadIdx.x & 31;
     if (static_cast<int>(blockIdx.x) < a.pair_blocks) {
         const int p = blockIdx.x * 8 + warp;
@@ -930,6 +941,8 @@
 
 template <int VEC_PER_LANE, bool ADD>
 __global__ void __launch_bounds__(256) combine_rows_kernel(Peers peers, CombineArgs a, const bf16* __restrict__ addend) {
+    griddep_wait();
+    griddep_launch_dependents();
     const int warp = threadIdx.x >> 5, lane = threadIdx.x & 31;
     if (a.do_signal || a.do_wait) a.epoch = epoch_of(peers, a.epoch);
     if (a.do_signal && blockIdx.x == 0 && threadIdx.x < 32) {
@@ -1012,6 +1025,8 @@
                                                        const float* __restrict__ sig, float scale,
                                                        const float* __restrict__ logits, const float* __restrict__ lse,
                                                        const unsigned char* __restrict__ alive) {
+    griddep_wait();
+    griddep_launch_dependents();
     constexpr bool DENSE = !NORM && !SIGMOID;
     const int warp = threadIdx.x >> 5, lane = threadIdx.x & 31;
     const int b = blockIdx.x * 8 + warp;
@@ -1398,11 +1413,9 @@
                                                                                      (LAYOUT_MAX_E + group_floats)))
         return e;
     if (B <= 0) return 0;
-    gate_topk_kernel<BIAS, SIGMOID, GROUPED, NORM><<<(B + 7) / 8, 256, 8 * (gs.total + group_floats) * sizeof(float),
-                                                     st>>>(
-        logits, B, gs, k, alive, failure_rate, seed, token_offset, idx, w, pos, counts, g_peers.step_ctr, bias, scale, sig,
-        n_group, topk_group, lse);
-    return 0;
+    return launch_pdl(gate_topk_kernel<BIAS, SIGMOID, GROUPED, NORM>, (B + 7) / 8, 256,
+                      8 * (gs.total + group_floats) * sizeof(float), st, logits, B, gs, k, alive, failure_rate, seed,
+                      token_offset, idx, w, pos, counts, g_peers.step_ctr, bias, scale, sig, n_group, topk_group, lse);
 }
 
 constexpr int GATE_BWD_DENSE_MAX_FLOATS = LAYOUT_MAX_E / 2 + 2 + LAYOUT_MAX_E + LAYOUT_MAX_E / 32 + 1;
@@ -1417,8 +1430,8 @@
             return e;
         if (gs.ndim > 1) smem = 8 * router_bwd_warp_floats(gs) * sizeof(float);
     }
-    gate_bwd_kernel<V, SIGMOID, NORM><<<(a.B + 7) / 8, 256, smem, st>>>(g_peers, a, gs, sig, scale, logits, lse, alive);
-    return 0;
+    return launch_pdl(gate_bwd_kernel<V, SIGMOID, NORM>, (a.B + 7) / 8, 256, smem, st, g_peers, a, gs, sig, scale, logits,
+                      lse, alive);
 }
 
 template <bool SIGMOID>
@@ -1559,7 +1572,7 @@
 #undef LAH_GATE_TOPK_N
 #undef LAH_GATE_TOPK
     if (e || B <= 0) return e;
-    rank_slots_kernel<<<gs.num_experts, 1024, 0, st>>>(idx, B * k, pos, counts);
+    launch_pdl(rank_slots_kernel, gs.num_experts, 1024, 0, st, idx, B * k, pos, counts);
     return -(int)cudaGetLastError();
 }
 
@@ -1576,7 +1589,7 @@
     a.group_rows = group_rows; a.tile_group = tile_group; a.total_rows = total_rows; a.status = status;
     a.S_max = S_max; a.shadow_tol = shadow_tol; a.min_shadow_rows = min_shadow_rows; a.route_owner = route_owner;
     a.step_rows = step_rows; a.shadow_info = shadow_info; a.owned_shadow = owned_shadow;
-    layout_exchange_kernel<<<1, 1024, 0, st>>>(g_peers, a);
+    launch_pdl(layout_exchange_kernel, 1, 1024, 0, st, g_peers, a);
     return -(int)cudaGetLastError();
 }
 
@@ -1593,9 +1606,9 @@
     a.route_owner = route_owner; a.num_groups = num_groups > 0 ? num_groups : E_loc;
     const int pad_blocks = a.num_groups < 64 ? a.num_groups : 64;
     const int grid = a.pair_blocks + pad_blocks;
-    if (H == 256) scatter_rows_kernel<1><<<grid, 256, 0, st>>>(g_peers, a);
-    else if (H == 512) scatter_rows_kernel<2><<<grid, 256, 0, st>>>(g_peers, a);
-    else if (H == 1024) scatter_rows_kernel<4><<<grid, 256, 0, st>>>(g_peers, a);
+    if (H == 256) launch_pdl(scatter_rows_kernel<1>, grid, 256, 0, st, g_peers, a);
+    else if (H == 512) launch_pdl(scatter_rows_kernel<2>, grid, 256, 0, st, g_peers, a);
+    else if (H == 1024) launch_pdl(scatter_rows_kernel<4>, grid, 256, 0, st, g_peers, a);
     else return -2;
     return -(int)cudaGetLastError();
 }
@@ -1620,8 +1633,8 @@
     const bf16* add = (const bf16*)addend;
     if (add && (reinterpret_cast<uintptr_t>(add) % 16)) return -3;
 #define LAH_COMBINE(V)                                                                   \
-    if (add) combine_rows_kernel<V, true><<<grid, 256, 0, st>>>(g_peers, a, add);        \
-    else combine_rows_kernel<V, false><<<grid, 256, 0, st>>>(g_peers, a, nullptr);
+    if (add) launch_pdl(combine_rows_kernel<V, true>, grid, 256, 0, st, g_peers, a, add);        \
+    else launch_pdl(combine_rows_kernel<V, false>, grid, 256, 0, st, g_peers, a, nullptr);
     if (H == 256) { LAH_COMBINE(1) }
     else if (H == 512) { LAH_COMBINE(2) }
     else if (H == 1024) { LAH_COMBINE(4) }
@@ -1748,6 +1761,42 @@
     return -(int)cudaGetLastError();
 }
 
+int lah_graph_programmatic_edges(void* graph, char* buf, int buflen, int* counts) {
+    cudaGraph_t g = static_cast<cudaGraph_t>(graph);
+    size_t n = 0;
+    if (cudaError_t e = cudaGraphGetEdges_v2(g, nullptr, nullptr, nullptr, &n)) return -static_cast<int>(e);
+    std::vector<cudaGraphNode_t> from(n), to(n);
+    std::vector<cudaGraphEdgeData> data(n);
+    if (n)
+        if (cudaError_t e = cudaGraphGetEdges_v2(g, from.data(), to.data(), data.data(), &n)) return -static_cast<int>(e);
+    auto name = [](cudaGraphNode_t node) -> std::string {
+        cudaGraphNodeType t;
+        cudaKernelNodeParams kp;
+        const char* nm = nullptr;
+        if (cudaGraphNodeGetType(node, &t) != cudaSuccess || t != cudaGraphNodeTypeKernel) return "?";
+        if (cudaGraphKernelNodeGetParams(node, &kp) != cudaSuccess || cudaFuncGetName(&nm, kp.func) != cudaSuccess || !nm) {
+            cudaGetLastError();
+            return "?";
+        }
+        return nm;
+    };
+    std::string lines;
+    int prog = 0;
+    for (size_t i = 0; i < n; ++i) {
+        if (data[i].type != cudaGraphDependencyTypeProgrammatic) continue;
+        ++prog;
+        if (buf) lines += name(from[i]) + "\t" + name(to[i]) + "\n";
+    }
+    counts[0] = static_cast<int>(n);
+    counts[1] = prog;
+    if (buf && buflen > 0) {
+        const size_t len = lines.size() < static_cast<size_t>(buflen - 1) ? lines.size() : static_cast<size_t>(buflen - 1);
+        memcpy(buf, lines.data(), len);
+        buf[len] = 0;
+    }
+    return 0;
+}
+
 int lah_zero_slots(float* g, int num_segs, const long long* seg_n, int slots, int first_slot, int num_slots, int seg_mask,
                    cudaStream_t st) {
     if (num_slots <= 0) return 0;
diff --git a/learning-at-home_b200/csrc/sm90.cuh b/learning-at-home_b200/csrc/sm90.cuh
--- a/learning-at-home_b200/csrc/sm90.cuh
+++ b/learning-at-home_b200/csrc/sm90.cuh
@@ -4,6 +4,7 @@
 #include <cuda_runtime.h>
 #include <cuda_bf16.h>
 #include <stdint.h>
+#include <utility>
 
 namespace lah {
 
@@ -287,6 +288,13 @@
     return t;
 }
 __device__ __forceinline__ void fence_proxy_async_global() { asm volatile("fence.proxy.async.global;" ::: "memory"); }
+
+__device__ __forceinline__ void griddep_wait() { asm volatile("griddepcontrol.wait;" ::: "memory"); }
+__device__ __forceinline__ void griddep_launch_dependents() { asm volatile("griddepcontrol.launch_dependents;" :::); }
+__device__ __forceinline__ void tma_prefetch_l2_3d(const CUtensorMap* tm, int c0, int c1, int c2) {
+    asm volatile("cp.async.bulk.prefetch.tensor.3d.L2.global [%0, {%1, %2, %3}];"
+                 ::"l"(reinterpret_cast<uint64_t>(tm)), "r"(c0), "r"(c1), "r"(c2) : "memory");
+}
 
 __device__ __forceinline__ uint32_t pack_bf16x2(float lo, float hi) {
     __nv_bfloat162 v = __floats2bfloat162_rn(lo, hi);
@@ -359,6 +367,21 @@
     return grid;
 }
 
+template <typename... KArgs, typename... Args>
+inline int launch_pdl(void (*kernel)(KArgs...), dim3 grid, dim3 block, size_t smem, cudaStream_t st, Args&&... args) {
+    cudaLaunchConfig_t cfg = {};
+    cfg.gridDim = grid;
+    cfg.blockDim = block;
+    cfg.dynamicSmemBytes = smem;
+    cfg.stream = st;
+    cudaLaunchAttribute attr[1];
+    attr[0].id = cudaLaunchAttributeProgrammaticStreamSerialization;
+    attr[0].val.programmaticStreamSerializationAllowed = 1;
+    cfg.attrs = attr;
+    cfg.numAttrs = 1;
+    return -static_cast<int>(cudaLaunchKernelEx(&cfg, kernel, std::forward<Args>(args)...));
+}
+
 template <auto Kernel>
 inline int set_max_dynamic_smem(int bytes) {
     static bool done = false;
diff --git a/learning-at-home_b200/csrc/small_m.cu b/learning-at-home_b200/csrc/small_m.cu
--- a/learning-at-home_b200/csrc/small_m.cu
+++ b/learning-at-home_b200/csrc/small_m.cu
@@ -9,6 +9,15 @@
 constexpr int MMA_K = 16;
 constexpr int BN_MAX = 128;
 constexpr int NUM_THREADS = 288;
+
+__device__ __forceinline__ void tile_counter_leave(int* ctr) {
+    __threadfence();
+    if (atomicAdd(ctr + 1, 1) == static_cast<int>(gridDim.x) - 1) {
+        __threadfence();
+        atomicExch(ctr, 0);
+        atomicExch(ctr + 1, 0);
+    }
+}
 
 namespace sab {
 
@@ -22,6 +31,7 @@
 constexpr int CUM_OFFSET = BAR_OFFSET + (2 * STAGES + 2 * QD) * 8 + QD * 4 + 16;
 constexpr int SMEM_TOTAL = CUM_OFFSET + (MAX_G + 1) * 4 + 1024;
 static_assert(SMEM_TOTAL <= 232448, "shared memory budget");
+constexpr int PREFETCH_KB = 8;
 
 struct Params {
     int G, M_out, K;
@@ -127,21 +137,6 @@
     const int warp = threadIdx.x >> 5;
     const int lane = threadIdx.x & 31;
 
-    if (warp == 0) {
-        int carry = 0;
-        for (int base = 0; base < p.G; base += 32) {
-            const int g = base + lane;
-            int x = g < p.G ? (__ldg(p.group_rows + g) + BN_MAX - 1) / BN_MAX : 0;
-#pragma unroll
-            for (int d = 1; d < 32; d <<= 1) {
-                const int y = __shfl_up_sync(0xffffffffu, x, d);
-                if (lane >= d) x += y;
-            }
-            if (g < p.G) cum[g + 1] = carry + x;
-            carry += __shfl_sync(0xffffffffu, x, 31);
-        }
-        if (lane == 0) cum[0] = 0;
-    }
     if (warp == 8 && lane == 0) {
         tma_prefetch_desc(&tmA);
         tma_prefetch_desc(&tmB16);
@@ -157,6 +152,33 @@
             mbar_init(&q_empty[i], 8);
         }
         fence_mbar_init();
+        const int m_slices = p.M_out / BM;
+        const int g = min(static_cast<int>(blockIdx.x) / m_slices, p.G - 1), ms = blockIdx.x % m_slices;
+        for (int kb = 0; kb < min(p.K / BK, PREFETCH_KB); ++kb) {
+            if (!A_MN) {
+                tma_prefetch_l2_3d(&tmA, kb * BK, ms * BM, g);
+            } else {
+#pragma unroll
+                for (int i = 0; i < BM / 64; ++i) tma_prefetch_l2_3d(&tmA, ms * BM + i * 64, kb * BK, g);
+            }
+        }
+    }
+    griddep_wait();
+
+    if (warp == 0) {
+        int carry = 0;
+        for (int base = 0; base < p.G; base += 32) {
+            const int g = base + lane;
+            int x = g < p.G ? (__ldg(p.group_rows + g) + BN_MAX - 1) / BN_MAX : 0;
+#pragma unroll
+            for (int d = 1; d < 32; d <<= 1) {
+                const int y = __shfl_up_sync(0xffffffffu, x, d);
+                if (lane >= d) x += y;
+            }
+            if (g < p.G) cum[g + 1] = carry + x;
+            carry += __shfl_sync(0xffffffffu, x, 31);
+        }
+        if (lane == 0) cum[0] = 0;
     }
     __syncthreads();
 
@@ -185,7 +207,11 @@
                 qi = 0;
                 qphase ^= 1;
             }
-            if (tile >= total) break;
+            if (tile >= total) {
+                tile_counter_leave(p.tile_counter);
+                griddep_launch_dependents();
+                break;
+            }
             const int gc = tile / m_slices, ms = tile - gc * m_slices;
             const int g = find_group(cum, p.G, gc);
             const int n0 = (gc - cum[g]) * BN_MAX;
@@ -301,13 +327,14 @@
 
 template <bool SPLIT>
 __device__ __forceinline__ void state_chunk_tma(const StateMaps<SPLIT>& tm, int n_arr, uint8_t* ss, uint64_t* bar, int col0,
-                                                int srow, int c) {
+                                                int srow, int c, bool l2_only = false) {
     if constexpr (SPLIT) {
         for (int a = 0; a < 2; ++a)
 #pragma unroll
             for (int q = 0; q < BN_MAX / PLANE_COLS; ++q) {
                 uint8_t* s = ss + a * PLANE_BYTES + q * SUB_BYTES;
-                if (bar) tma_load_3d(s, &tm.a[a], bar, col0 + q * PLANE_COLS, BAND_ROWS * c, srow / 16);
+                if (l2_only) tma_prefetch_l2_3d(&tm.a[a], col0 + q * PLANE_COLS, BAND_ROWS * c, srow / 16);
+                else if (bar) tma_load_3d(s, &tm.a[a], bar, col0 + q * PLANE_COLS, BAND_ROWS * c, srow / 16);
                 else tma_store_3d(&tm.a[a], s, col0 + q * PLANE_COLS, BAND_ROWS * c, srow / 16);
             }
     }
@@ -316,7 +343,8 @@
         for (int q = 0; q < BN_MAX / SUB_COLS; ++q) {
             uint8_t* s = ss + a * ARR_BYTES + q * SUB_BYTES;
             const CUtensorMap* m = &tm.a[SPLIT ? a + 1 : a];
-            if (bar) tma_load_3d(s, m, bar, col0 + q * SUB_COLS, BAND_ROWS * c, srow / 16);
+            if (l2_only) tma_prefetch_l2_3d(m, col0 + q * SUB_COLS, BAND_ROWS * c, srow / 16);
+            else if (bar) tma_load_3d(s, m, bar, col0 + q * SUB_COLS, BAND_ROWS * c, srow / 16);
             else tma_store_3d(m, s, col0 + q * SUB_COLS, BAND_ROWS * c, srow / 16);
         }
 }
@@ -335,32 +363,11 @@
     uint64_t* q_full = st_empty + ST_STAGES;
     uint64_t* q_empty = q_full + QD;
     volatile int* q_tile = reinterpret_cast<volatile int*>(q_empty + QD);
+    volatile int* poisoned = q_tile + QD;
 
     const int warp = threadIdx.x >> 5;
     const int lane = threadIdx.x & 31;
-    if (p.poison && (*p.poison & 1)) return;
     const int n_arr = p.amsgrad ? 4 : 3;
-
-    if (warp == 8 && lane == 0) {
-        tma_prefetch_desc(&tmDY);
-        tma_prefetch_desc(&tmX);
-        for (int a = 0; a < n_arr + (SPLIT ? 1 : 0); ++a) tma_prefetch_desc(&tmS.a[a]);
-        for (int i = 0; i < OP_STAGES; ++i) {
-            mbar_init(&op_full[i], 1);
-            mbar_init(&op_empty[i], 8);
-        }
-        for (int i = 0; i < ST_STAGES; ++i) {
-            mbar_init(&st_full[i], 1);
-            mbar_init(&st_empty[i], 1);
-        }
-        for (int i = 0; i < QD; ++i) {
-            mbar_init(&q_full[i], 1);
-            mbar_init(&q_empty[i], 8);
-        }
-        fence_mbar_init();
-    }
-    __syncthreads();
-
     const int n_tiles = p.K / BN_MAX;
     const int tiles_per_group = (p.N / BM) * n_tiles;
     const int total = p.G * tiles_per_group;
@@ -372,6 +379,37 @@
         t.nt = r - t.mt * n_tiles;
         return t;
     };
+
+    if (warp == 8 && lane == 0) {
+        tma_prefetch_desc(&tmDY);
+        tma_prefetch_desc(&tmX);
+        for (int a = 0; a < n_arr + (SPLIT ? 1 : 0); ++a) tma_prefetch_desc(&tmS.a[a]);
+        for (int i = 0; i < OP_STAGES; ++i) {
+            mbar_init(&op_full[i], 1);
+            mbar_init(&op_empty[i], 8);
+        }
+        for (int i = 0; i < ST_STAGES; ++i) {
+            mbar_init(&st_full[i], 1);
+            mbar_init(&st_empty[i], 1);
+        }
+        for (int i = 0; i < QD; ++i) {
+            mbar_init(&q_full[i], 1);
+            mbar_init(&q_empty[i], 8);
+        }
+        fence_mbar_init();
+        if (static_cast<int>(blockIdx.x) < total) {
+            const Tile t = decode(blockIdx.x);
+            for (int c = 0; c < ST_STAGES; ++c)
+                state_chunk_tma(tmS, n_arr, nullptr, nullptr, t.nt * BN_MAX, t.g * p.N + t.mt * BM, c, true);
+        }
+    }
+    griddep_wait();
+    if (threadIdx.x == 0) {
+        *poisoned = p.poison && (*p.poison & 1);
+        if (*poisoned) tile_counter_leave(p.tile_counter);
+    }
+    __syncthreads();
+    if (*poisoned) return;
 
     if (warp == 8) {
         if (lane != 0) return;
@@ -393,7 +431,11 @@
                 qi = 0;
                 qphase ^= 1;
             }
-            if (tile >= total) break;
+            if (tile >= total) {
+                tile_counter_leave(p.tile_counter);
+                griddep_launch_dependents();
+                break;
+            }
             const Tile t = decode(tile);
             const int off = __ldg(p.group_off + t.g), rows = __ldg(p.group_rows + t.g);
             const int srow = t.g * p.N + t.mt * BM;
@@ -640,16 +682,14 @@
     if (!p.tile_counter) return -3;
     const long long total = 1ll * (M_out / BM) * (G + x_rows / BN_MAX);
     if (total <= 0 || G <= 0) return 0;
-    if (cudaMemsetAsync(p.tile_counter, 0, sizeof(int), st) != cudaSuccess) return -4;
     const int ctas = persistent_grid(total, max_ctas);
     if (!a_mn) {
         if (int e = set_max_dynamic_smem<sab::swapab_kernel<false>>(sab::SMEM_TOTAL)) return e;
-        sab::swapab_kernel<false><<<ctas, NUM_THREADS, sab::SMEM_TOTAL, st>>>(p, tmA, tmB[0], tmB[1], tmB[2], tmB[3]);
-    } else {
-        if (int e = set_max_dynamic_smem<sab::swapab_kernel<true>>(sab::SMEM_TOTAL)) return e;
-        sab::swapab_kernel<true><<<ctas, NUM_THREADS, sab::SMEM_TOTAL, st>>>(p, tmA, tmB[0], tmB[1], tmB[2], tmB[3]);
-    }
-    return -(int)cudaGetLastError();
+        return launch_pdl(sab::swapab_kernel<false>, ctas, NUM_THREADS, sab::SMEM_TOTAL, st, p, tmA, tmB[0], tmB[1], tmB[2],
+                          tmB[3]);
+    }
+    if (int e = set_max_dynamic_smem<sab::swapab_kernel<true>>(sab::SMEM_TOTAL)) return e;
+    return launch_pdl(sab::swapab_kernel<true>, ctas, NUM_THREADS, sab::SMEM_TOTAL, st, p, tmA, tmB[0], tmB[1], tmB[2], tmB[3]);
 }
 
 }
@@ -658,8 +698,8 @@
 static int launch_wgrad_adam(const wa::Params& a, const CUtensorMap& tmDY, const CUtensorMap& tmX,
                              const wa::StateMaps<SPLIT>& tmS, const float* lr_dev, int ctas, cudaStream_t st) {
     if (int e = set_max_dynamic_smem<wa::wgrad_adam_kernel<WD, DEV_LR, SPLIT>>(wa::SMEM_TOTAL)) return e;
-    wa::wgrad_adam_kernel<WD, DEV_LR, SPLIT><<<ctas, NUM_THREADS, wa::SMEM_TOTAL, st>>>(a, tmDY, tmX, tmS, lr_dev);
-    return -(int)cudaGetLastError();
+    return launch_pdl(wa::wgrad_adam_kernel<WD, DEV_LR, SPLIT>, ctas, NUM_THREADS, wa::SMEM_TOTAL, st, a, tmDY, tmX, tmS,
+                      lr_dev);
 }
 
 template <bool SPLIT>
@@ -715,7 +755,6 @@
     if (!a.tile_counter) return -3;
     const long long total = 1ll * G * (N / BM) * (K / BN_MAX);
     if (total <= 0) return 0;
-    if (cudaMemsetAsync(a.tile_counter, 0, sizeof(int), st) != cudaSuccess) return -4;
     const int ctas = persistent_grid(total, max_ctas);
     if (lr_dev) {
         if (decoupled) return launch_wgrad_adam<wa::WD_DECOUPLED, true, SPLIT>(a, tmDY, tmX, tmS, lr_dev, ctas, st);
diff --git a/learning-at-home_b200/ops/kernels.py b/learning-at-home_b200/ops/kernels.py
--- a/learning-at-home_b200/ops/kernels.py
+++ b/learning-at-home_b200/ops/kernels.py
@@ -54,6 +54,7 @@
         "lah_adam_step": [P, P, P, P, P, P, I, P, I, P, P, I, Fl, P, Fl, Fl, Fl, Fl, I, I, I, L, P, Fl, I, P, L, I, I, I, Fl,
                           I, P],
         "lah_bump_steps": [P, P, I, P],
+        "lah_graph_programmatic_edges": [P, P, I, P],
         "lah_cast_bf16": [P, P, L, P],
         "lah_split_master": [P, P, P, P, L, I, P],
         "lah_attention_fwd": [P, P, P, L, I, I, I, c_ull, I, Fl, P, P],
@@ -941,6 +942,16 @@
 def bump_steps(step, group_rows):
     native.check(_lib().lah_bump_steps(ptr(step), ptr(group_rows), step.numel(), stream_ptr()), "lah_bump_steps")
     native.count_launch()
+
+
+def graph_programmatic_edges(graph):
+    buf = ctypes.create_string_buffer(1 << 20)
+    counts = (ctypes.c_int * 2)()
+    native.check(_lib().lah_graph_programmatic_edges(c_void_p(graph.raw_cuda_graph()), buf, len(buf), counts),
+                 "lah_graph_programmatic_edges")
+    edges = [tuple(line.split("\t")) for line in buf.value.decode().splitlines()]
+    assert len(edges) == counts[1], (len(edges), counts[1])
+    return counts[0], edges
 
 
 def cast_bf16(src, dst):
diff --git a/learning-at-home_b200/parallel/engine.py b/learning-at-home_b200/parallel/engine.py
--- a/learning-at-home_b200/parallel/engine.py
+++ b/learning-at-home_b200/parallel/engine.py
@@ -268,7 +268,7 @@
         octas = int(_os.environ.get("LAH_OPTIMIZER_CTAS", cfg.optimizer_ctas))
         sms = torch.cuda.get_device_properties(self.device).multi_processor_count
         if octas < 0:
-            octas = sms * (17 if self.world == 1 else 18) // 28
+            octas = sms * 8 // 11 if self.world == 1 else sms * 9 // 14
         self.opt_ctas = octas if (self.small and 0 < octas < sms - 8) else 0
         self.chain_ctas = sms - self.opt_ctas if self.opt_ctas else 0
         self.opt_stream = torch.cuda.Stream(self.device) if self.opt_ctas else None
```

Measured after the change: 14010, median of 6. 1.02x the previous value.
